# hku-mars/loam_livox

Hardware: NVIDIA H100
Metric: scans_per_sec (higher is better)
Workload: dtype f32 kNN / f64 solve

## Files before the change

include/loamlivox_b200.h:

```cpp
#ifndef LOAMLIVOX_B200_H
#define LOAMLIVOX_B200_H
#include <stddef.h>
#include <stdint.h>

#ifdef __cplusplus
extern "C" {
#endif

typedef struct { float x, y, z, intensity; } ll_point;
typedef struct { float x, y, z, _pad0, intensity, _pad1, _pad2, _pad3; } ll_pcl_xyzi;
enum { LL_FMT_XYZI16 = 0, LL_FMT_PCL32 = 1, LL_FMT_STRIDED = 2  };
enum { LL_HOST = 0, LL_DEVICE = 1 };

enum {
  LL_OK = 0,
  LL_ERR_INVALID = -1,
  LL_ERR_CUDA = -2,
  LL_ERR_CAPACITY = -3,
  LL_ERR_NO_BLOCKS = -4,
  LL_ERR_CAP_BINDS = -5
};

enum { LL_PT_NORMAL = 0, LL_PT_000 = 1, LL_PT_TOO_NEAR = 2, LL_PT_REFLECTIVITY_LOW = 4, LL_PT_REFLECTIVITY_HIGH = 8,
       LL_PT_CIRCLE_EDGE = 16, LL_PT_NAN = 32, LL_PT_SMALL_VIEW_ANGLE = 64 };
enum { LL_LABEL_INVALID = -1, LL_LABEL_UNLABELED = 0, LL_LABEL_CORNER = 1, LL_LABEL_SURFACE = 2, LL_LABEL_NEAR_NAN = 4,
       LL_LABEL_NEAR_ZERO = 8 };

typedef struct ll_ctx ll_ctx;
typedef struct ll_map ll_map;

typedef struct {
  float corner_curvature;
  float surface_curvature;
  float minimum_view_angle;
  float livox_min_dis;
  float livox_min_sigma;
  float max_fov_deg;
  float time_interval_pts;
  int   max_scan_points;
  int   max_features;
} ll_config;
void ll_config_default(ll_config* cfg);

int  ll_ctx_create(const ll_config* cfg, int device, ll_ctx** out);
void ll_ctx_destroy(ll_ctx* ctx);
int  ll_ctx_warmup(ll_ctx* ctx);
const char* ll_last_error(const ll_ctx* ctx);
void* ll_ctx_stream(ll_ctx* ctx);
int  ll_ctx_sync(ll_ctx* ctx);

int ll_extract(ll_ctx* ctx, const void* raw, size_t n, int fmt, int where, double stamp, int* n_scans);
int ll_extract_reset(ll_ctx* ctx);
int ll_piece_bounds(ll_ctx* ctx, int pieces, float* start, float* end);
int ll_get_features(ll_ctx* ctx, float minimum_blur, float maximum_blur, ll_point* corners, size_t* n_corners,
                    ll_point* surface, size_t* n_surface, ll_point* full, size_t* n_full);
int ll_extract_point_info(ll_ctx* ctx, int32_t* pt_type, int32_t* pt_label, float* curvature, float* view_angle,
                          float* depth_sq2, float* time_stamp, float* polar_dis_sq2, int32_t* polar_direction);
int ll_extract_split_idx(ll_ctx* ctx, int32_t* out, int cap, int* n_out);

int ll_voxel_downsample(ll_ctx* ctx, const void* in, size_t n, int fmt, int where, float leaf, ll_point* out, size_t* n_out);

int  ll_map_build(ll_ctx* ctx, const void* corner, size_t n_corner, const void* surf, size_t n_surf, int fmt, int where, ll_map** out);
int  ll_map_rebuild(ll_ctx* ctx, ll_map* map, const void* corner, size_t nc, const void* surf, size_t ns, int fmt, int where);
void ll_map_release(ll_map* map);
size_t ll_map_size(const ll_map* map, int which );
int  ll_map_build_sharded(ll_ctx* ctx, const void* corner, size_t n_corner, const void* surf, size_t n_surf, int fmt, int where,
                          int rank, int world, float cell_size, float halo_corner, float halo_surf, ll_map** out);
typedef struct { int rank, world; float cell_size, halo_corner, halo_surf; float origin[3]; int dims[3]; long long kept_corner, kept_surf, total_corner, total_surf; } ll_shard_info;
int  ll_map_shard_info(const ll_map* map, ll_shard_info* info, int* owner_out, size_t owner_cap);
int  ll_shard_plan(const int* cell_counts, const int dims[3], int world, int* owner_out);

int ll_knn(ll_ctx* ctx, const ll_map* map, int which, const ll_point* queries, size_t nq, int32_t* idx5, float* sqdist5);

typedef struct {
  int    if_motion_deblur;
  int    current_frame_index;
  int    mapping_init_accumulate_frames;
  int    icp_max_iterations;
  int    cere_max_iterations;
  int    cere_prerun_times;
  int    icp_plane, icp_line;
  int    maximum_allow_residual_block;
  int    rng_seed;
  double para_max_angular_rate;
  double para_max_speed;
  double max_final_cost;
  double minimum_pt_time_stamp, maximum_pt_time_stamp;
  double minimum_icp_R_diff, minimum_icp_T_diff;
  double inliner_dis, inlier_ratio;
  double maximum_dis_plane_for_match;
  double maximum_dis_line_for_match;
  double huber_a;
  double q_w_last[4], t_w_last[3];
  double q_w_curr[4], t_w_curr[3];
  double para_buffer_incremental[7];
} ll_reg_state;
void ll_reg_state_default(ll_reg_state* s);
void ll_reg_state_yaml(ll_reg_state* s, int realtime);
float ll_cap_uniform(int seed, int icp_iteration, int stream, int index);

typedef struct {
  int    status;
  int    registered;
  int    num_residual_blocks;
  int    icp_iterations, corner_used, surf_used;
  int    total_lm_iterations, total_evaluations;
  double q_w_curr[4], t_w_curr[3];
  double q_w_incre[4], t_w_incre[3];
  double inlier_threshold;
  double final_cost, initial_cost;
  double angular_diff, t_diff;
  float  gpu_ms_total, gpu_ms_knn;
  float  gpu_ms_knn_all, gpu_ms_solve_all, gpu_ms_select_all, gpu_ms_sort;
} ll_reg_result;

int ll_register(ll_ctx* ctx, const ll_map* map, const void* scan_corner, size_t n_corner, const void* scan_surf, size_t n_surf,
                int fmt, int where, const ll_reg_state* in, ll_reg_result* out);

int ll_build_blocks(ll_ctx* ctx, const ll_map* map, const void* scan_corner, size_t n_corner, const void* scan_surf, size_t n_surf,
                    int fmt, int where, const ll_reg_state* in, int32_t* type, double* a3, double* v3, int* corner_avail, int* surf_avail);
int ll_normal_equations(ll_ctx* ctx, const double x[7], double out28[28]);
int ll_solve(ll_ctx* ctx, int max_iterations, double x_io[7], double* initial_cost, double* final_cost, int* iterations);
int ll_inlier_select(ll_ctx* ctx, const double* l1, size_t n, double ratio, double* value, int* n_distinct);
int ll_set_blocks(ll_ctx* ctx, const ll_reg_state* in, size_t n, const int32_t* type, const ll_point* p, const float* a3, const double* v3);
int ll_solve_fused(ll_ctx* ctx, int prerun, int max_iterations, double x_io[7], double* threshold, int* n_distinct, int* n_kept, double* l1_out,
                   int iterations[2]);

typedef struct {
  float  line_res, plane_res;
  int    maximum_icp_iteration;
  int    maximum_residual_block;
  float  accepted_threshold;
  int    rng_seed;
  double t_init[3];
} ll_align_cfg;
void ll_align_cfg_default(ll_align_cfg* cfg);
int  ll_scene_align(ll_ctx* ctx, const void* source_line, size_t n_sl, const void* source_plane, size_t n_sp, const void* target_line, size_t n_tl,
                    const void* target_plane, size_t n_tp, int fmt, int where, const ll_align_cfg* cfg, ll_reg_result* out, int* scales_run);

int ll_transform(ll_ctx* ctx, const double q_wxyz[4], const double t[3], const void* in, size_t n, int fmt, int where, ll_point* out);

typedef struct {
  int   pieces;
  int   use_piece;
  float extractor_leaf_corner;
  float extractor_leaf_surf;
  float mapping_leaf_corner;
  float mapping_leaf_surf;
  int   whole_frame;
} ll_pipeline_cfg;
int ll_scan_to_pose(ll_ctx* ctx, const ll_map* map, const void* raw, size_t n, int fmt, int where, double stamp,
                    const ll_pipeline_cfg* pc, const ll_reg_state* in, ll_reg_result* out, int* n_corner_used, int* n_surf_used);

int ll_frame_to_pose(ll_ctx* ctx, const ll_map* map, int n_heads, const void* const* raws, const size_t* ns, int fmt, int where, const double* stamps,
                     const ll_pipeline_cfg* pc, const ll_reg_state* in, ll_reg_result* out, int* n_corner_used, int* n_surf_used);

typedef struct ll_cellmap ll_cellmap;
int  ll_cellmap_create(ll_ctx* ctx, float resolution, int revisit_threshold, int max_cells, ll_cellmap** out);
void ll_cellmap_release(ll_cellmap* map);
int  ll_cellmap_append(ll_ctx* ctx, ll_cellmap* map, const void* pts, size_t n, int fmt, int where);
int  ll_cellmap_assemble(ll_ctx* ctx, ll_cellmap* map, const double q_w_curr[4], const double t_w_curr[3], float search_range, float fov_deg, float leaf,
                         int down_sample_replace, ll_point* out_host, size_t cap, size_t* n_out, int* cells_in_fov, const ll_point** out_dev);
int  ll_cellmap_reserve(ll_ctx* ctx, ll_cellmap* map, size_t store_points, size_t scan_points);
int  ll_cellmap_stats(ll_ctx* ctx, ll_cellmap* map, int* cells, int* stored_points, int* frame_idx);

typedef struct {
  float line_resolution, plane_resolution;
  float cell_resolution;
  int   threshold_cell_revisit;
  float maximum_search_range_corner, maximum_search_range_surface, maximum_in_fov_angle;
  int   down_sample_replace;
  int   max_cells;
  int   matching_mode;
  int   maximum_history_size;
  int   reserve_map_points;
  int   reserve_store_points;
  ll_pipeline_cfg pipeline;
  ll_reg_state reg;
} ll_mapper_config;
typedef struct { int n_corner, n_surf, map_corner, map_surf, cells_in_fov_corner, cells_in_fov_surf, appended_corner, appended_surf;
                 float ms_front_end, ms_refresh, ms_register, ms_append;  } ll_mapper_stats;
typedef struct ll_mapper ll_mapper;
void ll_mapper_config_default(ll_mapper_config* cfg);
int  ll_mapper_create(ll_ctx* ctx, const ll_mapper_config* cfg, ll_mapper** out);
void ll_mapper_release(ll_mapper* mapper);
int  ll_mapper_process_scan(ll_mapper* mapper, const void* raw, size_t n, int fmt, int where, double stamp, ll_reg_result* out, ll_mapper_stats* stats);
int  ll_mapper_pose(const ll_mapper* mapper, double q_wxyz[4], double t[3], int* frame_index);

enum { LL_I_NONE = 0, LL_I_FLOAT32 = 7, LL_I_UINT8 = 2, LL_I_UINT16 = 4 };
typedef struct { int point_step, offset_x, offset_y, offset_z, offset_intensity, intensity_datatype; } ll_point_layout;
int  ll_set_point_layout(ll_ctx* ctx, const ll_point_layout* layout);
int  ll_features_to_pointcloud2(ll_ctx* ctx, int which, void* out_host, size_t cap_bytes, size_t* n_points);
int  ll_format_pose_log(const ll_reg_result* r, char* buf, size_t cap);

int  ll_state_snapshot_bytes(void);
int  ll_debug_solver_cycles(ll_ctx* ctx, long long out16[16]);

int ll_voxel_downsample_dev(ll_ctx* ctx, const ll_point* in_dev, size_t n, float leaf, ll_point* out_dev, size_t* n_out);
int ll_transform_dev(ll_ctx* ctx, const double q_wxyz[4], const double t[3], const ll_point* in_dev, size_t n, ll_point* out_dev);
int ll_last_features_dev(ll_ctx* ctx, const ll_point** corner_dev, size_t* n_corner, const ll_point** surf_dev, size_t* n_surf);

#define LL_IPC_HANDLE_BYTES 64
int ll_comm_local_handle(ll_ctx* ctx, unsigned char handle[LL_IPC_HANDLE_BYTES]);
int ll_comm_connect(ll_ctx* ctx, int rank, int world, const unsigned char* all_handles );

uint64_t ll_launch_count(const ll_ctx* ctx);

#ifdef __cplusplus
}
#endif
#endif
```

loam_livox_b200/capi.py:

```python
from __future__ import annotations

import ctypes as C
import os

import numpy as np

_HERE = os.path.dirname(os.path.abspath(__file__))
LIB_PATH = os.path.join(_HERE, "libloamlivox_b200.so")

LL_FMT_XYZI16, LL_FMT_PCL32, LL_FMT_STRIDED = 0, 1, 2
LL_I_NONE, LL_I_UINT8, LL_I_UINT16, LL_I_FLOAT32 = 0, 2, 4, 7
LL_HOST, LL_DEVICE = 0, 1
LL_OK, LL_ERR_INVALID, LL_ERR_CUDA, LL_ERR_CAPACITY, LL_ERR_NO_BLOCKS, LL_ERR_CAP_BINDS = 0, -1, -2, -3, -4, -5
LL_IPC_HANDLE_BYTES = 64

EXPORTS = [
    "ll_config_default", "ll_ctx_create", "ll_ctx_destroy", "ll_ctx_warmup", "ll_last_error", "ll_ctx_stream", "ll_ctx_sync", "ll_extract", "ll_extract_reset", "ll_piece_bounds",
    "ll_get_features", "ll_extract_point_info", "ll_extract_split_idx", "ll_voxel_downsample", "ll_map_build", "ll_map_release", "ll_map_size",
    "ll_map_build_sharded", "ll_knn", "ll_reg_state_default", "ll_register", "ll_build_blocks", "ll_normal_equations", "ll_solve", "ll_inlier_select", "ll_set_blocks", "ll_solve_fused", "ll_transform",
    "ll_scan_to_pose", "ll_comm_local_handle", "ll_comm_connect", "ll_launch_count", "ll_cellmap_create", "ll_cellmap_release", "ll_cellmap_append",
    "ll_cellmap_assemble", "ll_cellmap_reserve", "ll_cellmap_stats", "ll_voxel_downsample_dev", "ll_transform_dev", "ll_last_features_dev", "ll_mapper_config_default", "ll_mapper_create", "ll_mapper_release",
    "ll_mapper_process_scan", "ll_mapper_pose", "ll_map_rebuild", "ll_debug_solver_cycles", "ll_state_snapshot_bytes", "ll_set_point_layout", "ll_format_pose_log", "ll_reg_state_yaml", "ll_cap_uniform", "ll_map_shard_info", "ll_shard_plan", "ll_align_cfg_default", "ll_scene_align", "ll_frame_to_pose", "ll_features_to_pointcloud2",
]


class Config(C.Structure):
    _fields_ = [("corner_curvature", C.c_float), ("surface_curvature", C.c_float), ("minimum_view_angle", C.c_float), ("livox_min_dis", C.c_float),
                ("livox_min_sigma", C.c_float), ("max_fov_deg", C.c_float), ("time_interval_pts", C.c_float), ("max_scan_points", C.c_int), ("max_features", C.c_int)]


class RegState(C.Structure):
    _fields_ = [(n, C.c_int) for n in ("if_motion_deblur", "current_frame_index", "mapping_init_accumulate_frames", "icp_max_iterations", "cere_max_iterations",
                                       "cere_prerun_times", "icp_plane", "icp_line", "maximum_allow_residual_block", "rng_seed")] + \
               [(n, C.c_double) for n in ("para_max_angular_rate", "para_max_speed", "max_final_cost", "minimum_pt_time_stamp", "maximum_pt_time_stamp",
                                          "minimum_icp_R_diff", "minimum_icp_T_diff", "inliner_dis", "inlier_ratio", "maximum_dis_plane_for_match",
                                          "maximum_dis_line_for_match", "huber_a")] + \
               [("q_w_last", C.c_double * 4), ("t_w_last", C.c_double * 3), ("q_w_curr", C.c_double * 4), ("t_w_curr", C.c_double * 3),
                ("para_buffer_incremental", C.c_double * 7)]


class RegResult(C.Structure):
    _fields_ = [(n, C.c_int) for n in ("status", "registered", "num_residual_blocks", "icp_iterations", "corner_used", "surf_used", "total_lm_iterations",
                                       "total_evaluations")] + \
               [("q_w_curr", C.c_double * 4), ("t_w_curr", C.c_double * 3), ("q_w_incre", C.c_double * 4), ("t_w_incre", C.c_double * 3)] + \
               [(n, C.c_double) for n in ("inlier_threshold", "final_cost", "initial_cost", "angular_diff", "t_diff")] + \
               [("gpu_ms_total", C.c_float), ("gpu_ms_knn", C.c_float), ("gpu_ms_knn_all", C.c_float), ("gpu_ms_solve_all", C.c_float),
                ("gpu_ms_select_all", C.c_float), ("gpu_ms_sort", C.c_float)]


class PipelineCfg(C.Structure):
    _fields_ = [("pieces", C.c_int), ("use_piece", C.c_int), ("extractor_leaf_corner", C.c_float), ("extractor_leaf_surf", C.c_float),
                ("mapping_leaf_corner", C.c_float), ("mapping_leaf_surf", C.c_float), ("whole_frame", C.c_int)]


class PointLayout(C.Structure):
    _fields_ = [(n, C.c_int) for n in ("point_step", "offset_x", "offset_y", "offset_z", "offset_intensity", "intensity_datatype")]


class MapperConfig(C.Structure):
    _fields_ = [("line_resolution", C.c_float), ("plane_resolution", C.c_float), ("cell_resolution", C.c_float), ("threshold_cell_revisit", C.c_int),
                ("maximum_search_range_corner", C.c_float), ("maximum_search_range_surface", C.c_float), ("maximum_in_fov_angle", C.c_float),
                ("down_sample_replace", C.c_int), ("max_cells", C.c_int), ("matching_mode", C.c_int), ("maximum_history_size", C.c_int),
                ("reserve_map_points", C.c_int), ("reserve_store_points", C.c_int),
                ("pipeline", PipelineCfg), ("reg", RegState)]


class MapperStats(C.Structure):
    _fields_ = [(n, C.c_int) for n in ("n_corner", "n_surf", "map_corner", "map_surf", "cells_in_fov_corner", "cells_in_fov_surf", "appended_corner", "appended_surf")] + \
               [(n, C.c_float) for n in ("ms_front_end", "ms_refresh", "ms_register", "ms_append")]


class ShardInfo(C.Structure):
    _fields_ = [("rank", C.c_int), ("world", C.c_int), ("cell_size", C.c_float), ("halo_corner", C.c_float), ("halo_surf", C.c_float), ("origin", C.c_float * 3),
                ("dims", C.c_int * 3), ("kept_corner", C.c_longlong), ("kept_surf", C.c_longlong), ("total_corner", C.c_longlong), ("total_surf", C.c_longlong)]


class AlignCfg(C.Structure):
    _fields_ = [("line_res", C.c_float), ("plane_res", C.c_float), ("maximum_icp_iteration", C.c_int), ("maximum_residual_block", C.c_int),
                ("accepted_threshold", C.c_float), ("rng_seed", C.c_int), ("t_init", C.c_double * 3)]


class LoamLivoxError(RuntimeError):
    pass


_LIB = None


def lib():
    global _LIB
    if _LIB is not None:
        return _LIB
    if not os.path.exists(LIB_PATH):
        raise LoamLivoxError(f"{LIB_PATH} is missing: build it with `python -c 'import __graft_entry__ as g; g.build()'` (nvcc, sm_90a). "
                             "There is no CPU fallback.")
    L = C.CDLL(LIB_PATH)
    vp, sz, ci, cf, cd = C.c_void_p, C.c_size_t, C.c_int, C.c_float, C.c_double
    L.ll_config_default.argtypes = [C.POINTER(Config)]
    L.ll_ctx_create.argtypes = [C.POINTER(Config), ci, C.POINTER(vp)]
    L.ll_ctx_destroy.argtypes = [vp]
    L.ll_last_error.argtypes = [vp]
    L.ll_last_error.restype = C.c_char_p
    L.ll_ctx_stream.argtypes = [vp]
    L.ll_ctx_stream.restype = vp
    L.ll_ctx_sync.argtypes = [vp]
    L.ll_extract.argtypes = [vp, vp, sz, ci, ci, cd, C.POINTER(ci)]
    L.ll_extract_reset.argtypes = [vp]
    L.ll_piece_bounds.argtypes = [vp, ci, vp, vp]
    L.ll_get_features.argtypes = [vp, cf, cf, vp, C.POINTER(sz), vp, C.POINTER(sz), vp, C.POINTER(sz)]
    L.ll_extract_point_info.argtypes = [vp] + [vp] * 8
    L.ll_extract_split_idx.argtypes = [vp, vp, ci, C.POINTER(ci)]
    L.ll_voxel_downsample.argtypes = [vp, vp, sz, ci, ci, cf, vp, C.POINTER(sz)]
    L.ll_map_build.argtypes = [vp, vp, sz, vp, sz, ci, ci, C.POINTER(vp)]
    L.ll_map_build_sharded.argtypes = [vp, vp, sz, vp, sz, ci, ci, ci, ci, cf, cf, cf, C.POINTER(vp)]
    L.ll_map_shard_info.argtypes = [vp, C.POINTER(ShardInfo), vp, sz]
    L.ll_shard_plan.argtypes = [vp, vp, ci, vp]
    L.ll_align_cfg_default.argtypes = [C.POINTER(AlignCfg)]
    L.ll_scene_align.argtypes = [vp, vp, sz, vp, sz, vp, sz, vp, sz, ci, ci, C.POINTER(AlignCfg), C.POINTER(RegResult), C.POINTER(ci)]
    L.ll_map_release.argtypes = [vp]
    L.ll_map_size.argtypes = [vp, ci]
    L.ll_map_size.restype = sz
    L.ll_knn.argtypes = [vp, vp, ci, vp, sz, vp, vp]
    L.ll_reg_state_default.argtypes = [C.POINTER(RegState)]
    L.ll_reg_state_yaml.argtypes = [C.POINTER(RegState), ci]
    L.ll_cap_uniform.argtypes = [ci, ci, ci, ci]
    L.ll_cap_uniform.restype = cf
    L.ll_register.argtypes = [vp, vp, vp, sz, vp, sz, ci, ci, C.POINTER(RegState), C.POINTER(RegResult)]
    L.ll_build_blocks.argtypes = [vp, vp, vp, sz, vp, sz, ci, ci, C.POINTER(RegState), vp, vp, vp, C.POINTER(ci), C.POINTER(ci)]
    L.ll_normal_equations.argtypes = [vp, vp, vp]
    L.ll_solve.argtypes = [vp, ci, vp, C.POINTER(cd), C.POINTER(cd), C.POINTER(ci)]
    L.ll_inlier_select.argtypes = [vp, vp, sz, cd, C.POINTER(cd), C.POINTER(ci)]
    L.ll_set_blocks.argtypes = [vp, C.POINTER(RegState), sz, vp, vp, vp, vp]
    L.ll_solve_fused.argtypes = [vp, ci, ci, vp, C.POINTER(cd), C.POINTER(ci), C.POINTER(ci), vp, vp]
    L.ll_transform.argtypes = [vp, vp, vp, vp, sz, ci, ci, vp]
    L.ll_scan_to_pose.argtypes = [vp, vp, vp, sz, ci, ci, cd, C.POINTER(PipelineCfg), C.POINTER(RegState), C.POINTER(RegResult), C.POINTER(ci), C.POINTER(ci)]
    L.ll_frame_to_pose.argtypes = [vp, vp, ci, vp, vp, ci, ci, vp, C.POINTER(PipelineCfg), C.POINTER(RegState), C.POINTER(RegResult), C.POINTER(ci), C.POINTER(ci)]
    L.ll_features_to_pointcloud2.argtypes = [vp, ci, vp, sz, C.POINTER(sz)]
    L.ll_comm_local_handle.argtypes = [vp, vp]
    L.ll_comm_connect.argtypes = [vp, ci, ci, vp]
    L.ll_cellmap_create.argtypes = [vp, cf, ci, ci, C.POINTER(vp)]
    L.ll_cellmap_release.argtypes = [vp]
    L.ll_cellmap_append.argtypes = [vp, vp, vp, sz, ci, ci]
    L.ll_cellmap_assemble.argtypes = [vp, vp, vp, vp, cf, cf, cf, ci, vp, sz, C.POINTER(sz), C.POINTER(ci), C.POINTER(vp)]
    L.ll_ctx_warmup.argtypes = [vp]
    L.ll_cellmap_reserve.argtypes = [vp, vp, C.c_size_t, C.c_size_t]
    L.ll_cellmap_stats.argtypes = [vp, vp, C.POINTER(ci), C.POINTER(ci), C.POINTER(ci)]
    L.ll_voxel_downsample_dev.argtypes = [vp, vp, sz, cf, vp, C.POINTER(sz)]
    L.ll_transform_dev.argtypes = [vp, vp, vp, vp, sz, vp]
    L.ll_last_features_dev.argtypes = [vp, C.POINTER(vp), C.POINTER(sz), C.POINTER(vp), C.POINTER(sz)]
    L.ll_debug_solver_cycles.argtypes = [vp, vp]
    L.ll_state_snapshot_bytes.argtypes = []
    L.ll_set_point_layout.argtypes = [vp, C.POINTER(PointLayout)]
    L.ll_format_pose_log.argtypes = [C.POINTER(RegResult), C.c_char_p, sz]
    L.ll_map_rebuild.argtypes = [vp, vp, vp, sz, vp, sz, ci, ci]
    L.ll_mapper_config_default.argtypes = [C.POINTER(MapperConfig)]
    L.ll_mapper_create.argtypes = [vp, C.POINTER(MapperConfig), C.POINTER(vp)]
    L.ll_mapper_release.argtypes = [vp]
    L.ll_mapper_process_scan.argtypes = [vp, vp, sz, ci, ci, cd, C.POINTER(RegResult), C.POINTER(MapperStats)]
    L.ll_mapper_pose.argtypes = [vp, vp, vp, C.POINTER(ci)]
    L.ll_launch_count.argtypes = [vp]
    L.ll_launch_count.restype = C.c_uint64
    _LIB = L
    return L


def default_config(**kw) -> Config:
    c = Config()
    lib().ll_config_default(C.byref(c))
    for k, v in kw.items():
        setattr(c, k, v)
    return c


def default_reg_state(**kw) -> RegState:
    s = RegState()
    lib().ll_reg_state_default(C.byref(s))
    for k, v in kw.items():
        if isinstance(getattr(s, k), C.Array):
            getattr(s, k)[:] = list(v)
        else:
            setattr(s, k, v)
    return s


def yaml_reg_state(realtime: bool = False, **kw) -> RegState:
    s = RegState()
    lib().ll_reg_state_yaml(C.byref(s), int(bool(realtime)))
    for k, v in kw.items():
        if isinstance(getattr(s, k), C.Array):
            getattr(s, k)[:] = list(v)
        else:
            setattr(s, k, v)
    return s


def _ptr(a):
    if isinstance(a, (int, np.integer)):
        return C.c_void_p(int(a))
    return C.c_void_p(a.ctypes.data)


def _pts(a):
    a = np.ascontiguousarray(a, dtype=np.float32)
    assert a.ndim == 2 and a.shape[1] in (4, 8), "points must be [n,4] (XYZI16) or [n,8] (pcl::PointXYZI)"
    return a, (LL_FMT_XYZI16 if a.shape[1] == 4 else LL_FMT_PCL32)
```

loam_livox_b200/csrc/api.cu:

```cuda
#include <algorithm>
#include <cmath>
#include <cstring>
#include <cstdlib>
#include <cstdio>
#include "common.cuh"
#include "kernels.cuh"

static int ctx_alloc(ll_ctx* ctx) {
  const size_t cap = (size_t)ctx->cfg.max_features, scap = ctx->cfg.max_scan_points > ctx->cfg.max_features ? (size_t)ctx->cfg.max_scan_points : cap;
  RegArrays& A = ctx->A;
  LL_CUDA(ctx, ctx->reg_buf.carve([&](Carve& c) {
    A.feat = c.take<float4>(cap); A.blk_a = c.take<float4>(cap); A.blk_v = c.take<double>(cap * 3);
    A.l1 = c.take<double>(cap); A.k10_value = c.take<double>(1);
    A.k10_n_distinct = c.take<int>(1); A.counts = c.take<int>(16); A.bounds = c.take<float>(32);
    A.knn_idx = c.take<int>(cap * LL_KNN); A.knn_d = c.take<float>(cap * LL_KNN); A.perm = c.take<int>(cap);
    A.tmp_a = c.take<float4>(scap); A.tmp_b = c.take<float4>(scap); A.tmp_c = c.take<float4>(scap); A.tmp_d = c.take<float4>(scap);
  }));
  LL_TRY(extract_alloc(ctx));
  const int n = ctx->cfg.max_scan_points;
  const size_t vg = voxel_grid_bytes(n), pet = petals_bytes(n), gf = get_features_bytes(n);
  LL_CUDA(ctx, ctx->fe_main.reserve(std::max(vg, std::max(pet, gf))));
  LL_CUDA(ctx, ctx->fe_corner.reserve(vg));
  LL_CUDA(ctx, ctx->fe_petals.reserve(pet));
  return LL_OK;
}

extern "C" {

void ll_config_default(ll_config* c) {
  c->corner_curvature = 0.1f; c->surface_curvature = 0.005f; c->minimum_view_angle = 5.0f; c->livox_min_dis = 0.1f; c->livox_min_sigma = 7e-4f;
  c->max_fov_deg = 17.0f; c->time_interval_pts = 1.0e-5f; c->max_scan_points = 400000; c->max_features = 400000;
}
void ll_reg_state_default(ll_reg_state* s) {
  memset(s, 0, sizeof(*s));
  s->if_motion_deblur = 0; s->current_frame_index = 1000; s->mapping_init_accumulate_frames = 50; s->icp_max_iterations = 15; s->cere_max_iterations = 50; s->cere_prerun_times = 2;
  s->icp_plane = 1; s->icp_line = 1; s->maximum_allow_residual_block = 1000000;
  s->para_max_angular_rate = 20.0; s->para_max_speed = 0.3; s->max_final_cost = 1.0e9; s->minimum_pt_time_stamp = 0.0; s->maximum_pt_time_stamp = 0.1;
  s->minimum_icp_R_diff = 0.01; s->minimum_icp_T_diff = 0.01; s->inliner_dis = 0.02; s->inlier_ratio = 0.80; s->maximum_dis_plane_for_match = 50.0; s->maximum_dis_line_for_match = 2.0; s->huber_a = 0.1;
  s->q_w_last[0] = 1; s->q_w_curr[0] = 1; s->para_buffer_incremental[3] = 1;
}

void ll_reg_state_yaml(ll_reg_state* s, int realtime) {
  ll_reg_state_default(s);
  s->maximum_allow_residual_block = realtime ? 150 : 200;
  s->max_final_cost = 2.0;
}
float ll_cap_uniform(int seed, int icp_iteration, int stream, int index) { return ll_cap_uniform_f(seed, icp_iteration, stream, index); }

int ll_ctx_create(const ll_config* cfg, int device, ll_ctx** out) {
  if (!out) return LL_ERR_INVALID;
  *out = nullptr;
  int ndev = 0;
  if (cudaGetDeviceCount(&ndev) != cudaSuccess || ndev == 0) return LL_ERR_CUDA;
  if (device < 0 || device >= ndev) return LL_ERR_INVALID;
  if (cfg && (cfg->max_scan_points < 1 || cfg->max_scan_points >= (1 << 21) || cfg->max_features < 1)) return LL_ERR_INVALID;
  ll_ctx* ctx = new ll_ctx();
  ctx->device = device;
  if (cfg) ctx->cfg = *cfg; else ll_config_default(&ctx->cfg);
  cudaError_t e = cudaSetDevice(device);
  auto ok = [&](cudaError_t r) { if (e == cudaSuccess && r != cudaSuccess) e = r; };
  cudaDeviceProp prop; ok(cudaGetDeviceProperties(&prop, device)); ctx->num_sms = prop.multiProcessorCount;
  ok(cudaStreamCreateWithFlags(&ctx->stream, cudaStreamNonBlocking));
  ok(cudaStreamCreateWithFlags(&ctx->stream2, cudaStreamNonBlocking));
  ok(cudaStreamCreateWithFlags(&ctx->stream3, cudaStreamNonBlocking));
  ctx->sev.each([&](cudaEvent_t& ev) { ok(cudaEventCreateWithFlags(&ev, cudaEventDisableTiming)); });
  ctx->ev.each([&](cudaEvent_t& ev) { ok(cudaEventCreate(&ev)); });
  ok(cudaHostAlloc((void**)&ctx->pin, sizeof(PinnedStage), cudaHostAllocDefault));
  void* dreg = nullptr; ok(cudaMalloc(&dreg, sizeof(RegDevState))); if (dreg) ok(cudaMemset(dreg, 0, sizeof(RegDevState))); ctx->d_reg = (RegDevState*)dreg;
  if (e == cudaSuccess && solve_prepare(ctx) != LL_OK) e = cudaErrorUnknown;
  if (e == cudaSuccess && ctx_alloc(ctx) != LL_OK) e = cudaErrorMemoryAllocation;
  if (e != cudaSuccess) { cudaGetLastError(); ll_ctx_destroy(ctx); return LL_ERR_CUDA; }
  *out = ctx; return LL_OK;
}
void ll_ctx_destroy(ll_ctx* ctx) {
  if (!ctx) return;
  cudaSetDevice(ctx->device);
  for (cudaStream_t s : {ctx->stream, ctx->stream2, ctx->stream3}) if (s) cudaStreamSynchronize(s);
  if (ctx->fg.exec) cudaGraphExecDestroy(ctx->fg.exec);
  for (DevBuf* b : {&ctx->scratch, &ctx->scratch2, &ctx->fe_main, &ctx->fe_corner, &ctx->fe_petals, &ctx->stage_in, &ctx->extract_buf, &ctx->feat_buf, &ctx->reg_buf}) b->release();
  if (ctx->pin) cudaFreeHost(ctx->pin);
  if (ctx->d_reg) cudaFree(ctx->d_reg);
  if (ctx->d_sync) cudaFree(ctx->d_sync);
  if (ctx->comm_local) cudaFree(ctx->comm_local);
  for (int i = 0; i < 8; i++) if (ctx->comm_peers[i] && i != ctx->rank) cudaIpcCloseMemHandle(ctx->comm_peers[i]);
  ctx->sev.each([](cudaEvent_t& ev) { if (ev) cudaEventDestroy(ev); });
  ctx->ev.each([](cudaEvent_t& ev) { if (ev) cudaEventDestroy(ev); });
  for (cudaStream_t s : {ctx->stream3, ctx->stream2, ctx->stream}) if (s) cudaStreamDestroy(s);
  delete ctx;
}
const char* ll_last_error(const ll_ctx* ctx) { return ctx ? ctx->err.c_str() : "null context"; }
void* ll_ctx_stream(ll_ctx* ctx) { return (void*)ctx->stream; }
int ll_ctx_sync(ll_ctx* ctx) { cudaSetDevice(ctx->device); LL_CUDA(ctx, cudaStreamSynchronize(ctx->stream)); return LL_OK; }
uint64_t ll_launch_count(const ll_ctx* ctx) { return ctx->launches; }

static int extract_prepare(ll_ctx* ctx, const void* raw, size_t n, int fmt, int where, double stamp) {
  if ((int)n > ctx->cfg.max_scan_points) { ctx->set_error("scan larger than max_scan_points"); return LL_ERR_CAPACITY; }
  ExtractState& e = ctx->ex;
  if (stamp <= 0.0000001 || (stamp < e.last_maximum_time_stamp)) e.current_time = e.last_maximum_time_stamp; else e.current_time = stamp - e.first_receive_time;
  if (e.first_receive_time <= 0) e.first_receive_time = stamp;
  e.n = (int)n;
  if (n > 0) e.last_maximum_time_stamp = (double)(float)(e.current_time + (double)(((float)(n - 1)) * ctx->cfg.time_interval_pts));
  LL_TRY(upload_cloud(ctx, raw, n, fmt, where, e.raw));
  ctx->pin->extract_time = e.current_time;
  LL_CUDA(ctx, cudaMemcpyAsync(e.d_time, &ctx->pin->extract_time, sizeof(double), cudaMemcpyHostToDevice, ctx->stream));
  return LL_OK;
}
static int extract_enqueue(ll_ctx* ctx, DevBuf& scratch) {
  ExtractState& e = ctx->ex;
  if (e.n >= 5) { LL_TRY(launch_extract_points(ctx, e.n)); LL_TRY(launch_extract_petals(ctx, e.n, ctx->stream, scratch)); }
  else LL_CUDA(ctx, cudaMemsetAsync(e.d_meta, 0, 16, ctx->stream));
  return LL_OK;
}
int ll_extract(ll_ctx* ctx, const void* raw, size_t n, int fmt, int where, double stamp, int* n_scans) {
  if (!ctx || (!raw && n)) return LL_ERR_INVALID;
  cudaSetDevice(ctx->device);
  ExtractState& e = ctx->ex;
  LL_TRY(extract_prepare(ctx, raw, n, fmt, where, stamp));
  LL_TRY(extract_enqueue(ctx, ctx->scratch));
  if (n_scans) {
    int* h = ctx->pin->counts;
    LL_CUDA(ctx, cudaMemcpyAsync(h, e.d_meta, 3 * sizeof(int), cudaMemcpyDeviceToHost, ctx->stream));
    LL_CUDA(ctx, cudaStreamSynchronize(ctx->stream));
    *n_scans = h[1];
  }
  return LL_OK;
}
int ll_extract_reset(ll_ctx* ctx) {
  if (!ctx) return LL_ERR_INVALID;
  ctx->ex.first_receive_time = -1; ctx->ex.current_time = 0; ctx->ex.last_maximum_time_stamp = 0; ctx->ex.n = 0;
  return LL_OK;
}
int ll_piece_bounds(ll_ctx* ctx, int pieces, float* start, float* end) {
  if (!ctx || pieces < 1 || pieces > 16) return LL_ERR_INVALID;
  cudaSetDevice(ctx->device);
  const RegArrays& A = ctx->A;
  LL_TRY(launch_piece_bounds(ctx, pieces, A.bounds));
  float* h = ctx->pin->bounds;
  LL_CUDA(ctx, cudaMemcpyAsync(h, A.bounds, 2 * pieces * sizeof(float), cudaMemcpyDeviceToHost, ctx->stream));
  LL_CUDA(ctx, cudaStreamSynchronize(ctx->stream));
  for (int i = 0; i < pieces; i++) { start[i] = h[2 * i]; end[i] = h[2 * i + 1]; }
  return LL_OK;
}
int ll_get_features(ll_ctx* ctx, float minimum_blur, float maximum_blur, ll_point* corners, size_t* n_corners, ll_point* surface, size_t* n_surface, ll_point* full, size_t* n_full) {
  if (!ctx) return LL_ERR_INVALID;
  cudaSetDevice(ctx->device);
  const RegArrays& A = ctx->A;
  LL_TRY(launch_get_features(ctx, ctx->stream, ctx->scratch, nullptr, minimum_blur, maximum_blur, A.tmp_a, A.tmp_b, A.tmp_c, A.counts));
  int* h = ctx->pin->counts;
  LL_CUDA(ctx, cudaMemcpyAsync(h, A.counts, 3 * sizeof(int), cudaMemcpyDeviceToHost, ctx->stream));
  LL_CUDA(ctx, cudaStreamSynchronize(ctx->stream));
  int nc = ctx->ex.n ? h[0] : 0, ns = ctx->ex.n ? h[1] : 0, nf = ctx->ex.n ? h[2] : 0;
  if (corners && nc) LL_CUDA(ctx, cudaMemcpyAsync(corners, A.tmp_a, (size_t)nc * 16, cudaMemcpyDeviceToHost, ctx->stream));
  if (surface && ns) LL_CUDA(ctx, cudaMemcpyAsync(surface, A.tmp_b, (size_t)ns * 16, cudaMemcpyDeviceToHost, ctx->stream));
  if (full && nf) LL_CUDA(ctx, cudaMemcpyAsync(full, A.tmp_c, (size_t)nf * 16, cudaMemcpyDeviceToHost, ctx->stream));
  LL_CUDA(ctx, cudaStreamSynchronize(ctx->stream));
  if (n_corners) *n_corners = nc; if (n_surface) *n_surface = ns; if (n_full) *n_full = nf;
  return LL_OK;
}
int ll_extract_point_info(ll_ctx* ctx, int32_t* pt_type, int32_t* pt_label, float* curvature, float* view_angle, float* depth_sq2, float* time_stamp, float* polar_dis_sq2, int32_t* polar_direction) {
  if (!ctx) return LL_ERR_INVALID;
  cudaSetDevice(ctx->device);
  ExtractState& e = ctx->ex; size_t n = e.n; cudaStream_t s = ctx->stream;
  if (pt_type) LL_CUDA(ctx, cudaMemcpyAsync(pt_type, e.pt_type, n * 4, cudaMemcpyDeviceToHost, s));
  if (pt_label) LL_CUDA(ctx, cudaMemcpyAsync(pt_label, e.pt_label, n * 4, cudaMemcpyDeviceToHost, s));
  if (curvature) LL_CUDA(ctx, cudaMemcpyAsync(curvature, e.curvature, n * 4, cudaMemcpyDeviceToHost, s));
  if (view_angle) LL_CUDA(ctx, cudaMemcpyAsync(view_angle, e.view_angle, n * 4, cudaMemcpyDeviceToHost, s));
  if (depth_sq2) LL_CUDA(ctx, cudaMemcpyAsync(depth_sq2, e.depth_sq2, n * 4, cudaMemcpyDeviceToHost, s));
  if (time_stamp) LL_CUDA(ctx, cudaMemcpyAsync(time_stamp, e.time_stamp, n * 4, cudaMemcpyDeviceToHost, s));
  if (polar_dis_sq2) LL_CUDA(ctx, cudaMemcpyAsync(polar_dis_sq2, e.polar_dis_sq2, n * 4, cudaMemcpyDeviceToHost, s));
  LL_CUDA(ctx, cudaStreamSynchronize(s));
  if (polar_direction) {
    std::vector<int8_t> tmp(n);
    LL_CUDA(ctx, cudaMemcpy(tmp.data(), e.polar_dir, n, cudaMemcpyDeviceToHost));
    for (size_t i = 0; i < n; i++) polar_direction[i] = tmp[i];
  }
  return LL_OK;
}
int ll_extract_split_idx(ll_ctx* ctx, int32_t* out, int cap, int* n_out) {
  if (!ctx) return LL_ERR_INVALID;
  cudaSetDevice(ctx->device);
  int meta[3] = {0, 0, 0};
  LL_CUDA(ctx, cudaStreamSynchronize(ctx->stream));
  LL_CUDA(ctx, cudaMemcpy(meta, ctx->ex.d_meta, sizeof(meta), cudaMemcpyDeviceToHost));
  int m = meta[0] < cap ? meta[0] : cap;
  if (m > 0) LL_CUDA(ctx, cudaMemcpy(out, ctx->ex.split_idx, (size_t)m * 4, cudaMemcpyDeviceToHost));
  if (n_out) *n_out = meta[0];
  return LL_OK;
}

int ll_voxel_downsample(ll_ctx* ctx, const void* in, size_t n, int fmt, int where, float leaf, ll_point* out, size_t* n_out) {
  if (!ctx || !n_out || !(leaf > 0.f)) return LL_ERR_INVALID;
  cudaSetDevice(ctx->device);
  *n_out = 0; if (n == 0) return LL_OK;
  float4* d_in; float4* d_out; int* d_n;
  LL_CUDA(ctx, ctx->feat_buf.carve([&](Carve& c) { d_in = c.take<float4>(n); d_out = c.take<float4>(n); d_n = c.take<int>(1); }));
  LL_TRY(upload_cloud(ctx, in, n, fmt, where, d_in));
  LL_TRY(launch_voxel_grid(ctx, ctx->stream, ctx->scratch, d_in, (int)n, nullptr, leaf, d_out, d_n));
  int* h = ctx->pin->counts;
  LL_CUDA(ctx, cudaMemcpyAsync(h, d_n, sizeof(int), cudaMemcpyDeviceToHost, ctx->stream));
  LL_CUDA(ctx, cudaStreamSynchronize(ctx->stream));
  *n_out = (size_t)h[0];
  if (out && h[0] > 0) { LL_CUDA(ctx, cudaMemcpyAsync(out, d_out, (size_t)h[0] * 16, cudaMemcpyDeviceToHost, ctx->stream)); LL_CUDA(ctx, cudaStreamSynchronize(ctx->stream)); }
  return LL_OK;
}
int ll_transform(ll_ctx* ctx, const double q[4], const double t[3], const void* in, size_t n, int fmt, int where, ll_point* out) {
  if (!ctx || !q || !t) return LL_ERR_INVALID;
  cudaSetDevice(ctx->device);
  if (n == 0) return LL_OK;
  float4* d_in; float4* d_out; double* d_pose;
  LL_CUDA(ctx, ctx->feat_buf.carve([&](Carve& c) { d_in = c.take<float4>(n); d_out = c.take<float4>(n); d_pose = c.take<double>(7); }));
  double* h = ctx->pin->pose; for (int k = 0; k < 4; k++) h[k] = q[k]; for (int k = 0; k < 3; k++) h[4 + k] = t[k];
  LL_CUDA(ctx, cudaMemcpyAsync(d_pose, h, 7 * sizeof(double), cudaMemcpyHostToDevice, ctx->stream));
  LL_TRY(upload_cloud(ctx, in, n, fmt, where, d_in));
  LL_TRY(launch_transform(ctx, ctx->stream, d_pose, d_in, (int)n, d_out));
  LL_CUDA(ctx, cudaMemcpyAsync(out, d_out, n * 16, cudaMemcpyDeviceToHost, ctx->stream));
  LL_CUDA(ctx, cudaStreamSynchronize(ctx->stream));
  return LL_OK;
}

int ll_voxel_downsample_dev(ll_ctx* ctx, const ll_point* in_dev, size_t n, float leaf, ll_point* out_dev, size_t* n_out) {
  if (!ctx || !n_out || !(leaf > 0.f)) return LL_ERR_INVALID;
  cudaSetDevice(ctx->device);
  *n_out = 0; if (n == 0) return LL_OK;
  int* d_n;
  LL_CUDA(ctx, ctx->feat_buf.carve([&](Carve& c) { d_n = c.take<int>(1); }));
  LL_TRY(launch_voxel_grid(ctx, ctx->stream, ctx->scratch, (const float4*)in_dev, (int)n, nullptr, leaf, (float4*)out_dev, d_n));
  int* h = ctx->pin->counts;
  LL_CUDA(ctx, cudaMemcpyAsync(h, d_n, sizeof(int), cudaMemcpyDeviceToHost, ctx->stream));
  LL_CUDA(ctx, cudaStreamSynchronize(ctx->stream));
  *n_out = (size_t)h[0];
  return LL_OK;
}
int ll_transform_dev(ll_ctx* ctx, const double q[4], const double t[3], const ll_point* in_dev, size_t n, ll_point* out_dev) {
  if (!ctx || !q || !t) return LL_ERR_INVALID;
  cudaSetDevice(ctx->device);
  if (n == 0) return LL_OK;
  double* d_pose;
  LL_CUDA(ctx, ctx->feat_buf.carve([&](Carve& c) { d_pose = c.take<double>(7); }));
  double* h = ctx->pin->pose; for (int k = 0; k < 4; k++) h[k] = q[k]; for (int k = 0; k < 3; k++) h[4 + k] = t[k];
  LL_CUDA(ctx, cudaMemcpyAsync(d_pose, h, 7 * sizeof(double), cudaMemcpyHostToDevice, ctx->stream));
  LL_TRY(launch_transform(ctx, ctx->stream, d_pose, (const float4*)in_dev, (int)n, (float4*)out_dev));
  LL_CUDA(ctx, cudaStreamSynchronize(ctx->stream));
  return LL_OK;
}
int ll_last_features_dev(ll_ctx* ctx, const ll_point** corner_dev, size_t* n_corner, const ll_point** surf_dev, size_t* n_surf) {
  if (!ctx) return LL_ERR_INVALID;
  const RegArrays& A = ctx->A;
  if (corner_dev) *corner_dev = (const ll_point*)A.feat; if (n_corner) *n_corner = (size_t)ctx->last_nc;
  if (surf_dev) *surf_dev = (const ll_point*)(A.feat + ctx->last_nc); if (n_surf) *n_surf = (size_t)ctx->last_ns;
  return LL_OK;
}

static int map_index(ll_ctx* ctx, ll_map* m, const void* corner, size_t nc, const void* surf, size_t ns, int fmt, int where) {
  const bool in_place = where == LL_DEVICE && fmt == LL_FMT_XYZI16;
  const float4* d_c = (const float4*)corner; const float4* d_s = (const float4*)surf;
  int st = LL_OK;
  if (!in_place) {
    float4* b_c; float4* b_s;
    LL_CUDA(ctx, ctx->feat_buf.carve([&](Carve& c) { b_c = c.take<float4>(nc); b_s = c.take<float4>(ns); }));
    d_c = b_c; d_s = b_s;
    st = upload_cloud(ctx, corner, nc, fmt, where, b_c);
    if (st == LL_OK) st = upload_cloud(ctx, surf, ns, fmt, where, b_s);
    if (st != LL_OK) return st;
  }
  cudaStream_t s = ctx->stream;
  LL_CUDA(ctx, cudaEventRecord(ctx->sev.fork, s));
  LL_CUDA(ctx, cudaStreamWaitEvent(ctx->stream2, ctx->sev.fork, 0));
  st = build_bucket_tree(ctx, ctx->stream2, ctx->scratch2, d_c, (int)nc, &m->corner);
  const int st2 = build_bucket_tree(ctx, s, ctx->scratch, d_s, (int)ns, &m->surf);
  LL_CUDA(ctx, cudaEventRecord(ctx->sev.join, ctx->stream2));
  LL_CUDA(ctx, cudaStreamWaitEvent(s, ctx->sev.join, 0));
  if (st == LL_OK) st = st2;
  if (st == LL_OK && where == LL_HOST && cudaStreamSynchronize(s) != cudaSuccess) st = LL_ERR_CUDA;
  return st;
}
static int map_build_common(ll_ctx* ctx, const void* corner, size_t nc, const void* surf, size_t ns, int fmt, int where, ll_map** out) {
  if (!ctx || !out) return LL_ERR_INVALID;
  cudaSetDevice(ctx->device);
  ll_map* m = new ll_map(); m->device = ctx->device;
  int st = map_index(ctx, m, corner, nc, surf, ns, fmt, where);
  if (st != LL_OK) { m->corner.storage.release(); m->surf.storage.release(); delete m; return st; }
  *out = m; return LL_OK;
}
int ll_map_rebuild(ll_ctx* ctx, ll_map* map, const void* corner, size_t nc, const void* surf, size_t ns, int fmt, int where) {
  if (!ctx || !map) return LL_ERR_INVALID;
  cudaSetDevice(ctx->device);
  return map_index(ctx, map, corner, nc, surf, ns, fmt, where);
}
int ll_map_build(ll_ctx* ctx, const void* corner, size_t nc, const void* surf, size_t ns, int fmt, int where, ll_map** out) {
  return map_build_common(ctx, corner, nc, surf, ns, fmt, where, out);
}
void ll_map_release(ll_map* map) {
  if (!map) return;
  cudaSetDevice(map->device);
  map->corner.storage.release(); map->surf.storage.release(); map->shard_owner.release(); delete map;
}
size_t ll_map_size(const ll_map* map, int which) { return map ? (size_t)(which == 0 ? map->corner.n : map->surf.n) : 0; }

int ll_knn(ll_ctx* ctx, const ll_map* map, int which, const ll_point* queries, size_t nq, int32_t* idx5, float* sqdist5) {
  if (!ctx || !map) return LL_ERR_INVALID;
  cudaSetDevice(ctx->device);
  if (nq == 0) return LL_OK;
  float4* d_q; int* d_idx; float* d_d;
  LL_CUDA(ctx, ctx->feat_buf.carve([&](Carve& c) { d_q = c.take<float4>(nq); d_idx = c.take<int>(nq * LL_KNN); d_d = c.take<float>(nq * LL_KNN); }));
  LL_CUDA(ctx, cudaMemcpyAsync(d_q, queries, nq * 16, cudaMemcpyHostToDevice, ctx->stream));
  LL_TRY(launch_knn_query(ctx, which == 0 ? map->corner : map->surf, d_q, (int)nq, d_idx, d_d));
  LL_CUDA(ctx, cudaMemcpyAsync(idx5, d_idx, nq * 20, cudaMemcpyDeviceToHost, ctx->stream));
  LL_CUDA(ctx, cudaMemcpyAsync(sqdist5, d_d, nq * 20, cudaMemcpyDeviceToHost, ctx->stream));
  LL_CUDA(ctx, cudaStreamSynchronize(ctx->stream));
  return LL_OK;
}

static void fill_state(RegDevState* h, const ll_reg_state* in) {
  memset(h, 0, sizeof(RegDevState));
  for (int k = 0; k < 4; k++) { h->pose_curr[k] = in->q_w_curr[k]; h->pose_last[k] = in->q_w_last[k]; }
  for (int k = 0; k < 3; k++) { h->pose_curr[4 + k] = in->t_w_curr[k]; h->pose_last[4 + k] = in->t_w_last[k]; }
  for (int k = 0; k < 7; k++) h->x[k] = in->para_buffer_incremental[k];
  h->q_last_opt[0] = 1.0;
  h->bound = (double)(float)in->para_max_speed; h->huber_a = in->huber_a; h->inliner_dis = in->inliner_dis; h->inlier_ratio = in->inlier_ratio;
  h->min_icp_R = in->minimum_icp_R_diff; h->min_icp_T = in->minimum_icp_T_diff;
  h->cap = in->maximum_allow_residual_block; h->rng_seed = in->rng_seed;
  h->if_motion_deblur = in->if_motion_deblur ? 1 : 0; h->min_ts = in->minimum_pt_time_stamp; h->max_ts = in->maximum_pt_time_stamp;
}
static KnnBlocksArgs knn_args(ll_ctx* ctx, const ll_map* map, int nc, int ns, const ll_reg_state* in, bool debug) {
  const RegArrays& A = ctx->A;
  KnnBlocksArgs a; a.corner = make_view(map->corner); a.surf = make_view(map->surf); a.feat = A.feat; a.n_corner = nc; a.n_surf = ns;
  a.pose = ctx->d_reg->pose_curr; a.max_dis_line = in->maximum_dis_line_for_match; a.max_dis_plane = in->maximum_dis_plane_for_match;
  a.icp_line = in->icp_line; a.icp_plane = in->icp_plane; a.blk_a = A.blk_a; a.blk_v = A.blk_v;
  a.corner_avail = &ctx->d_reg->corner_avail; a.surf_avail = &ctx->d_reg->surf_avail; a.n_blocks = &ctx->d_reg->n_blocks;
  a.cap = in->maximum_allow_residual_block; a.rng_seed = in->rng_seed;
  a.seed_ids = A.knn_idx; a.knn_d = debug ? A.knn_d : nullptr; a.perm = A.perm;
  ctx->solve_world = (map->world > 1 && ctx->world > 1) ? ctx->world : 1;
  a.st = ctx->d_reg; a.deblur = in->if_motion_deblur ? 1 : 0; ctx->reg_deblur = a.deblur;
  a.rank = map->rank; a.world = map->world; a.grid = map->grid; a.shard_owner = (const int*)map->shard_owner.p;
  return a;
}
static SolveArgs solve_args(ll_ctx* ctx, int M, SolveMode mode, int max_iter) {
  const RegArrays& A = ctx->A;
  SolveArgs s; s.st = ctx->d_reg; s.sync = ctx->d_sync; s.feat = A.feat; s.blk_a = A.blk_a; s.blk_v = A.blk_v; s.l1 = A.l1; s.k10_value = A.k10_value; s.k10_n_distinct = A.k10_n_distinct;
  s.M = M; s.max_iterations = max_iter; s.mode = mode; s.rank = ctx->rank; s.world = ctx->solve_world; s.comm_local = (double*)ctx->comm_local;
  for (int i = 0; i < 8; i++) s.comm_peer[i] = (double*)ctx->comm_peers[i];
  s.cap_check = 0; s.deblur = ctx->reg_deblur; s.prerun_iterations = 0; s.table = nullptr; s.table_mask = 0;
  return s;
}

}

int register_device(ll_ctx* ctx, const ll_map* map, int nc, int ns, const ll_reg_state* in, ll_reg_result* out) {
  cudaStream_t s = ctx->stream;
  const RegArrays& A = ctx->A;
  RegEvents& ev = ctx->ev;
  memset(out, 0, sizeof(*out));
  out->status = 1;
  for (int k = 0; k < 4; k++) { out->q_w_curr[k] = in->q_w_curr[k]; out->q_w_incre[k] = k == 0 ? in->para_buffer_incremental[3] : in->para_buffer_incremental[k - 1]; }
  for (int k = 0; k < 3; k++) { out->t_w_curr[k] = in->t_w_curr[k]; out->t_w_incre[k] = in->para_buffer_incremental[4 + k]; }
  if (!(map->corner.n_src > 0 && map->surf.n_src > 50 && in->current_frame_index > in->mapping_init_accumulate_frames)) return LL_OK;
  const int M = nc + ns;
  ctx->last_nc = nc; ctx->last_ns = ns;
  const int cap_check = M > in->maximum_allow_residual_block ? 1 : 0;
  if (M == 0) { ctx->set_error("no features"); return LL_ERR_NO_BLOCKS; }
  LL_TRY(solve_capacity(ctx, M, in->if_motion_deblur ? 1 : 0));
  RegDevState* h = &ctx->pin->state_in;
  fill_state(h, in);
  LL_CUDA(ctx, cudaMemcpyAsync(ctx->d_reg, h, sizeof(RegDevState), cudaMemcpyHostToDevice, s));
  LL_CUDA(ctx, cudaEventRecord(ev.total[0], s));
  out->registered = 1;
  KnnBlocksArgs ka = knn_args(ctx, map, nc, ns, in, false);
  LL_CUDA(ctx, cudaMemsetAsync(A.knn_idx, 0xff, (size_t)M * LL_KNN * 4, s));
  LL_CUDA(ctx, cudaEventRecord(ev.sort[0], s));
  LL_TRY(launch_query_sort(ctx, s, ctx->scratch, ka, A.perm));
  LL_CUDA(ctx, cudaEventRecord(ev.sort[1], s));
  int iter = 0; RegDevState* hs = &ctx->pin->snap[0];
  const bool sharded = ctx->world > 1 && map->world > 1;
  if (sharded && (map->world != ctx->world || map->rank != ctx->rank)) { ctx->set_error("map shard and context disagree on rank/world"); return LL_ERR_INVALID; }
  if (map->world > 1 && (std::sqrt(in->maximum_dis_line_for_match) > (double)map->halo[0] * 1.0001 + 1e-3 || std::sqrt(in->maximum_dis_plane_for_match) > (double)map->halo[1] * 1.0001 + 1e-3)) {
    ctx->set_error("match gates wider than the halo this shard was built with: owner + halo search would no longer be exact"); return LL_ERR_INVALID;
  }
  if (map->world > 1 && ctx->world != map->world) { ctx->set_error("a sharded map needs a context connected to the same number of ranks (ll_comm_connect)"); return LL_ERR_INVALID; }
  if (sharded && M > ctx->cfg.max_features) { ctx->set_error("more features than max_features (exchange buffer)"); return LL_ERR_CAPACITY; }
  double* x_l1 = sharded ? (double*)((char*)ctx->comm_local + LL_COMM_X_OFF) : nullptr;
  unsigned long long* set_table = nullptr;
  LL_CUDA(ctx, ctx->scratch.carve([&](Carve& c) { set_table = l1_set_layout(c, M); }));
  RegDevState* slots = ctx->pin->snap;
  auto enqueue_iteration = [&](int it) -> int {
    cudaEvent_t* e = it < LL_TIMED_ITERS ? ev.phase[it] : nullptr;
    LL_CUDA(ctx, cudaMemsetAsync(&ctx->d_reg->corner_avail, 0, 3 * sizeof(int), s));
    if (sharded) LL_CUDA(ctx, cudaMemsetAsync(x_l1, 0xff, (size_t)M * sizeof(double), s));
    if (it == 0) LL_CUDA(ctx, cudaEventRecord(ev.knn_first[0], s));
    if (e) LL_CUDA(ctx, cudaEventRecord(e[0], s));
    LL_TRY(launch_knn_blocks(ctx, ka));
    if (e) LL_CUDA(ctx, cudaEventRecord(e[1], s));
    if (it == 0) LL_CUDA(ctx, cudaEventRecord(ev.knn_first[1], s));
    if (!sharded) {
      SolveArgs sa = solve_args(ctx, M, SOLVE_FUSED, in->cere_max_iterations);
      sa.prerun_iterations = in->cere_prerun_times; sa.table = set_table; sa.table_mask = l1_set_capacity(M) - 1;
      sa.cap_check = cap_check;
      if (e) { LL_CUDA(ctx, cudaEventRecord(e[2], s)); LL_CUDA(ctx, cudaEventRecord(e[3], s)); }
      LL_TRY(launch_solve(ctx, sa));
    } else {
      if (cap_check) LL_TRY(launch_count_exchange(ctx));
      { SolveArgs sa = solve_args(ctx, M, SOLVE_FIRST, in->cere_prerun_times); sa.cap_check = cap_check; LL_TRY(launch_solve(ctx, sa)); }
      if (e) LL_CUDA(ctx, cudaEventRecord(e[2], s));
      LL_TRY(launch_l1_exchange(ctx, A.l1, M));
      LL_TRY(launch_k10_select(ctx, x_l1, M, &ctx->d_reg->inlier_ratio, set_table, l1_set_capacity(M) - 1, A.k10_value, A.k10_n_distinct));
      if (e) LL_CUDA(ctx, cudaEventRecord(e[3], s));
      { SolveArgs sa = solve_args(ctx, M, SOLVE_SECOND, in->cere_max_iterations); sa.cap_check = cap_check; LL_TRY(launch_solve(ctx, sa)); }
    }
    if (e) LL_CUDA(ctx, cudaEventRecord(e[4], s));
    LL_CUDA(ctx, cudaMemcpyAsync(&slots[it & 1], ctx->d_reg, sizeof(RegDevState), cudaMemcpyDeviceToHost, s));
    LL_CUDA(ctx, cudaEventRecord(ctx->sev.it[it & 1], s));
    return LL_OK;
  };
  const bool speculate = !sharded;
  LL_TRY(enqueue_iteration(0));
  for (iter = 0; iter < in->icp_max_iterations; iter++) {
    if (speculate && iter + 1 < in->icp_max_iterations) LL_TRY(enqueue_iteration(iter + 1));
    LL_CUDA(ctx, cudaEventSynchronize(ctx->sev.it[iter & 1]));
    hs = &slots[iter & 1];
    if (hs->lm.termination == -1) {
      cudaStreamSynchronize(s); ctx->set_error("no residual block survived the gates / cap / inlier selection"); return LL_ERR_NO_BLOCKS;
    }
    if (hs->icp_done) break;
    if (!speculate && iter + 1 < in->icp_max_iterations) LL_TRY(enqueue_iteration(iter + 1));
  }
  LL_CUDA(ctx, cudaEventRecord(ev.total[1], s));
  LL_CUDA(ctx, cudaEventSynchronize(ev.total[1]));
  cudaEventElapsedTime(&out->gpu_ms_total, ev.total[0], ev.total[1]); cudaEventElapsedTime(&out->gpu_ms_knn, ev.knn_first[0], ev.knn_first[1]);
  cudaEventElapsedTime(&out->gpu_ms_sort, ev.sort[0], ev.sort[1]);
  { const int done_iters = (iter < in->icp_max_iterations ? iter + 1 : in->icp_max_iterations);
    for (int i = 0; i < done_iters && i < LL_TIMED_ITERS; i++) { float a = 0, b = 0, c = 0, d = 0; cudaEvent_t* e = ev.phase[i];
      cudaEventElapsedTime(&a, e[0], e[1]); cudaEventElapsedTime(&b, e[1], e[2]); cudaEventElapsedTime(&c, e[2], e[3]); cudaEventElapsedTime(&d, e[3], e[4]);
      out->gpu_ms_knn_all += a; out->gpu_ms_solve_all += b + d; out->gpu_ms_select_all += c; } }
  out->icp_iterations = (iter + 1 < in->icp_max_iterations) ? iter + 1 : in->icp_max_iterations;
  out->corner_used = hs->corner_avail; out->surf_used = hs->surf_avail; out->num_residual_blocks = hs->num_residual_blocks;
  out->total_lm_iterations = hs->total_lm_iterations; out->total_evaluations = hs->total_evaluations;
  for (int k = 0; k < 4; k++) out->q_w_curr[k] = hs->pose_curr[k];
  for (int k = 0; k < 3; k++) out->t_w_curr[k] = hs->pose_curr[4 + k];
  out->q_w_incre[0] = hs->x[3]; out->q_w_incre[1] = hs->x[0]; out->q_w_incre[2] = hs->x[1]; out->q_w_incre[3] = hs->x[2];
  for (int k = 0; k < 3; k++) out->t_w_incre[k] = hs->x[4 + k];
  out->final_cost = hs->final_cost; out->initial_cost = hs->initial_cost; out->angular_diff = hs->angular_diff; out->t_diff = hs->t_diff;
  out->inlier_threshold = hs->inlier_threshold * hs->final_cost / hs->initial_cost;
  const float minimize_cost = (float)hs->final_cost;
  if (hs->angular_diff > (double)(float)in->para_max_angular_rate || minimize_cost > (float)in->max_final_cost) {
    out->status = 0;
    for (int k = 0; k < 4; k++) out->q_w_curr[k] = in->q_w_last[k];
    for (int k = 0; k < 3; k++) out->t_w_curr[k] = in->t_w_last[k];
  }
  return LL_OK;
}

extern "C" {

int ll_register(ll_ctx* ctx, const ll_map* map, const void* scan_corner, size_t nc, const void* scan_surf, size_t ns, int fmt, int where, const ll_reg_state* in, ll_reg_result* out) {
  if (!ctx || !map || !in || !out) return LL_ERR_INVALID;
  cudaSetDevice(ctx->device);
  if ((int)(nc + ns) > ctx->cfg.max_features) { ctx->set_error("more features than max_features"); return LL_ERR_CAPACITY; }
  LL_TRY(upload_cloud(ctx, scan_corner, nc, fmt, where, ctx->A.feat));
  LL_TRY(upload_cloud(ctx, scan_surf, ns, fmt, where, ctx->A.feat + nc));
  return register_device(ctx, map, (int)nc, (int)ns, in, out);
}

int ll_ctx_warmup(ll_ctx* ctx) {
  if (!ctx) return LL_ERR_INVALID;
  cudaSetDevice(ctx->device);
  std::vector<ll_point> surf, corner, fs, fc;
  auto add = [](std::vector<ll_point>& v, float x, float y, float z) { ll_point p; p.x = x; p.y = y; p.z = z; p.intensity = 0.f; v.push_back(p); };
  for (int i = 0; i < 20; i++) for (int j = 0; j < 20; j++) {
    const float u = 0.1f * i + 0.013f * (j % 3), v = 0.1f * j + 0.007f * (i % 5);
    add(surf, 1.f + u, -1.f + v, 0.f); add(surf, 1.f + u, 1.2f, 0.05f + v); add(surf, 3.2f, -1.f + u, 0.05f + v);
    if ((i * 20 + j) % 4 == 0) { add(fs, 1.f + u + 0.004f, -1.f + v - 0.003f, 0.006f); add(fs, 1.f + u, 1.195f, 0.05f + v); add(fs, 3.194f, -1.f + u, 0.05f + v); }
  }
  for (int k = 0; k < 20; k++) { add(corner, 3.2f, 1.2f, 0.1f * k); add(corner, 1.f + 0.1f * k, 1.2f, 0.f); if (k % 4 == 0) { add(fc, 3.195f, 1.197f, 0.1f * k + 0.02f); add(fc, 1.02f + 0.1f * k, 1.196f, 0.004f); } }
  if ((int)(fc.size() + fs.size()) > ctx->cfg.max_features) return LL_OK;
  ll_map* m = nullptr;
  int st = ll_map_build(ctx, corner.data(), corner.size(), surf.data(), surf.size(), LL_FMT_XYZI16, LL_HOST, &m);
  if (st == LL_OK) {
    ll_reg_state rs; ll_reg_state_default(&rs); rs.current_frame_index = rs.mapping_init_accumulate_frames + 1;
    ll_reg_result r;
    st = ll_register(ctx, m, fc.data(), fc.size(), fs.data(), fs.size(), LL_FMT_XYZI16, LL_HOST, &rs, &r);
    if (st == LL_ERR_NO_BLOCKS) st = LL_OK;
  }
  if (m) ll_map_release(m);
  if (cudaStreamSynchronize(ctx->stream) != cudaSuccess) return LL_ERR_CUDA;
  return st;
}

int ll_build_blocks(ll_ctx* ctx, const ll_map* map, const void* scan_corner, size_t nc, const void* scan_surf, size_t ns, int fmt, int where, const ll_reg_state* in,
                    int32_t* type, double* a3, double* v3, int* corner_avail, int* surf_avail) {
  if (!ctx || !map || !in) return LL_ERR_INVALID;
  cudaSetDevice(ctx->device);
  const int M = (int)(nc + ns);
  if (M > ctx->cfg.max_features) return LL_ERR_CAPACITY;
  const RegArrays& A = ctx->A;
  cudaStream_t s = ctx->stream;
  LL_TRY(upload_cloud(ctx, scan_corner, nc, fmt, where, A.feat));
  LL_TRY(upload_cloud(ctx, scan_surf, ns, fmt, where, A.feat + nc));
  RegDevState* h = &ctx->pin->state_in; fill_state(h, in);
  LL_CUDA(ctx, cudaMemcpyAsync(ctx->d_reg, h, sizeof(RegDevState), cudaMemcpyHostToDevice, s));
  { KnnBlocksArgs ka = knn_args(ctx, map, (int)nc, (int)ns, in, true); LL_CUDA(ctx, cudaMemsetAsync(A.knn_idx, 0xff, (size_t)M * LL_KNN * 4, s)); LL_TRY(launch_query_sort(ctx, s, ctx->scratch, ka, A.perm)); LL_TRY(launch_knn_blocks(ctx, ka)); }
  std::vector<float4> ba(M); std::vector<double> bv((size_t)M * 3);
  int cnt[2];
  LL_CUDA(ctx, cudaMemcpyAsync(ba.data(), A.blk_a, (size_t)M * 16, cudaMemcpyDeviceToHost, s));
  LL_CUDA(ctx, cudaMemcpyAsync(bv.data(), A.blk_v, (size_t)M * 24, cudaMemcpyDeviceToHost, s));
  LL_CUDA(ctx, cudaMemcpyAsync(cnt, &ctx->d_reg->corner_avail, 8, cudaMemcpyDeviceToHost, s));
  LL_CUDA(ctx, cudaStreamSynchronize(s));
  for (int i = 0; i < M; i++) {
    int t; memcpy(&t, &ba[i].w, 4);
    if (type) type[i] = t;
    if (a3) { a3[3 * i] = ba[i].x; a3[3 * i + 1] = ba[i].y; a3[3 * i + 2] = ba[i].z; }
    if (v3) { v3[3 * i] = bv[3 * i]; v3[3 * i + 1] = bv[3 * i + 1]; v3[3 * i + 2] = bv[3 * i + 2]; }
  }
  if (corner_avail) *corner_avail = cnt[0]; if (surf_avail) *surf_avail = cnt[1];
  ctx->hook_slots = M;
  return LL_OK;
}
}

static int hook_solve(ll_ctx* ctx, const double x[7], const SolveArgs& sa, double* l1_out = nullptr) {
  cudaStream_t s = ctx->stream;
  PinnedStage* pin = ctx->pin;
  for (int k = 0; k < 7; k++) pin->x[k] = x[k];
  LL_CUDA(ctx, cudaMemcpyAsync(ctx->d_reg->x, pin->x, 7 * sizeof(double), cudaMemcpyHostToDevice, s));
  LL_TRY(launch_solve(ctx, sa));
  LL_CUDA(ctx, cudaMemcpyAsync(&pin->snap[0], ctx->d_reg, sizeof(RegDevState), cudaMemcpyDeviceToHost, s));
  if (l1_out && sa.M > 0) LL_CUDA(ctx, cudaMemcpyAsync(l1_out, ctx->A.l1, (size_t)sa.M * sizeof(double), cudaMemcpyDeviceToHost, s));
  LL_CUDA(ctx, cudaStreamSynchronize(s));
  return LL_OK;
}

extern "C" {

int ll_normal_equations(ll_ctx* ctx, const double x[7], double out28[28]) {
  if (!ctx || !x || !out28) return LL_ERR_INVALID;
  cudaSetDevice(ctx->device);
  LL_TRY(hook_solve(ctx, x, solve_args(ctx, ctx->hook_slots, SOLVE_EVALUATE, 0)));
  const RegDevState* hs = &ctx->pin->snap[0];
  for (int i = 0; i < 21; i++) out28[i] = hs->lm.H[i];
  for (int i = 0; i < 6; i++) out28[21 + i] = hs->lm.g[i];
  out28[27] = hs->lm.x_cost;
  return LL_OK;
}
int ll_solve(ll_ctx* ctx, int max_iterations, double x_io[7], double* initial_cost, double* final_cost, int* iterations) {
  if (!ctx || !x_io) return LL_ERR_INVALID;
  cudaSetDevice(ctx->device);
  LL_TRY(hook_solve(ctx, x_io, solve_args(ctx, ctx->hook_slots, SOLVE_PLAIN, max_iterations)));
  const RegDevState* hs = &ctx->pin->snap[0];
  for (int k = 0; k < 7; k++) x_io[k] = hs->x[k];
  if (initial_cost) *initial_cost = hs->lm.initial_cost; if (final_cost) *final_cost = hs->lm.final_cost; if (iterations) *iterations = hs->lm.iteration;
  return LL_OK;
}
int ll_set_blocks(ll_ctx* ctx, const ll_reg_state* in, size_t n, const int32_t* type, const ll_point* p, const float* a3, const double* v3) {
  if (!ctx || !in || (n > 0 && (!type || !p || !a3 || !v3))) return LL_ERR_INVALID;
  if (n > (size_t)ctx->cfg.max_features) { ctx->set_error("more blocks than max_features"); return LL_ERR_CAPACITY; }
  const int M = (int)n;
  LL_TRY(solve_capacity(ctx, M, in->if_motion_deblur ? 1 : 0));
  for (int i = 0; i < M; i++) if (type[i] < 0 || type[i] > 2) { ctx->set_error("block type must be 0, 1 (line) or 2 (plane)"); return LL_ERR_INVALID; }
  cudaSetDevice(ctx->device);
  const RegArrays& A = ctx->A;
  cudaStream_t s = ctx->stream;
  std::vector<float4> ba(M);
  for (int i = 0; i < M; i++) { ba[i].x = a3[3 * i]; ba[i].y = a3[3 * i + 1]; ba[i].z = a3[3 * i + 2]; memcpy(&ba[i].w, &type[i], 4); }
  if (M > 0) {
    LL_CUDA(ctx, cudaMemcpyAsync(A.feat, p, (size_t)M * 16, cudaMemcpyHostToDevice, s));
    LL_CUDA(ctx, cudaMemcpyAsync(A.blk_a, ba.data(), (size_t)M * 16, cudaMemcpyHostToDevice, s));
    LL_CUDA(ctx, cudaMemcpyAsync(A.blk_v, v3, (size_t)M * 24, cudaMemcpyHostToDevice, s));
  }
  RegDevState* h = &ctx->pin->state_in; fill_state(h, in);
  for (int i = 0; i < M; i++) h->n_blocks += type[i] != 0 ? 1 : 0;
  LL_CUDA(ctx, cudaMemcpyAsync(ctx->d_reg, h, sizeof(RegDevState), cudaMemcpyHostToDevice, s));
  LL_CUDA(ctx, cudaStreamSynchronize(s));
  ctx->hook_slots = M; ctx->hook_cap_check = M > in->maximum_allow_residual_block ? 1 : 0;
  ctx->reg_deblur = in->if_motion_deblur ? 1 : 0; ctx->solve_world = 1;
  return LL_OK;
}
int ll_solve_fused(ll_ctx* ctx, int prerun, int max_iterations, double x_io[7], double* threshold, int* n_distinct, int* n_kept, double* l1_out, int iterations[2]) {
  if (!ctx || !x_io) return LL_ERR_INVALID;
  cudaSetDevice(ctx->device);
  const int M = ctx->hook_slots;
  cudaStream_t s = ctx->stream;
  SolveArgs sa = solve_args(ctx, M, SOLVE_FUSED, max_iterations);
  LL_CUDA(ctx, ctx->scratch.carve([&](Carve& c) { sa.table = l1_set_layout(c, M); }));
  sa.prerun_iterations = prerun; sa.table_mask = l1_set_capacity(M) - 1;
  sa.cap_check = ctx->hook_cap_check;
  LL_CUDA(ctx, cudaMemsetAsync(&ctx->d_reg->icp_done, 0, sizeof(int), s));
  LL_CUDA(ctx, cudaMemsetAsync(&ctx->d_reg->total_lm_iterations, 0, 2 * sizeof(int), s));
  LL_TRY(hook_solve(ctx, x_io, sa, l1_out));
  const RegDevState* hs = &ctx->pin->snap[0];
  for (int k = 0; k < 7; k++) x_io[k] = hs->x[k];
  if (threshold) *threshold = hs->inlier_threshold; if (n_distinct) *n_distinct = hs->n_unique; if (n_kept) *n_kept = hs->num_residual_blocks;
  if (iterations) { iterations[1] = hs->lm.iteration; iterations[0] = hs->total_lm_iterations - hs->lm.iteration; }
  return LL_OK;
}
int ll_inlier_select(ll_ctx* ctx, const double* l1, size_t n, double ratio, double* value, int* n_distinct) {
  if (!ctx || (n > 0 && !l1) || !value || !n_distinct || !(ratio >= 0.0)) return LL_ERR_INVALID;
  for (size_t i = 0; i < n; i++) if (l1[i] < 0.0) { ctx->set_error("L1 norms are never negative"); return LL_ERR_INVALID; }
  if (n > (size_t)ctx->cfg.max_features) { ctx->set_error("more values than max_features"); return LL_ERR_CAPACITY; }
  cudaSetDevice(ctx->device);
  const int M = (int)n;
  const RegArrays& A = ctx->A;
  cudaStream_t s = ctx->stream;
  if (M > 0) LL_CUDA(ctx, cudaMemcpyAsync(A.l1, l1, n * sizeof(double), cudaMemcpyHostToDevice, s));
  double* d_ratio = &ctx->d_reg->inlier_ratio;
  LL_CUDA(ctx, cudaMemcpyAsync(d_ratio, &ratio, sizeof(double), cudaMemcpyHostToDevice, s));
  unsigned long long* table = nullptr;
  LL_CUDA(ctx, ctx->scratch.carve([&](Carve& c) { table = l1_set_layout(c, M); }));
  LL_TRY(launch_k10_select(ctx, A.l1, M, d_ratio, table, l1_set_capacity(M) - 1, A.k10_value, A.k10_n_distinct));
  LL_CUDA(ctx, cudaMemcpyAsync(value, A.k10_value, sizeof(double), cudaMemcpyDeviceToHost, s));
  LL_CUDA(ctx, cudaMemcpyAsync(n_distinct, A.k10_n_distinct, sizeof(int), cudaMemcpyDeviceToHost, s));
  LL_CUDA(ctx, cudaStreamSynchronize(s));
  return LL_OK;
}

int ll_set_point_layout(ll_ctx* ctx, const ll_point_layout* L) {
  if (!ctx || !L) return LL_ERR_INVALID;
  const int isz = L->intensity_datatype == LL_I_FLOAT32 ? 4 : L->intensity_datatype == LL_I_UINT16 ? 2 : L->intensity_datatype == LL_I_UINT8 ? 1 : 0;
  if (L->intensity_datatype != LL_I_NONE && isz == 0) { ctx->set_error("unsupported intensity datatype"); return LL_ERR_INVALID; }
  const int offs[3] = {L->offset_x, L->offset_y, L->offset_z};
  for (int k = 0; k < 3; k++) if (offs[k] < 0 || offs[k] + 4 > L->point_step) { ctx->set_error("field outside the point record"); return LL_ERR_INVALID; }
  if (isz && (L->offset_intensity < 0 || L->offset_intensity + isz > L->point_step)) { ctx->set_error("intensity outside the point record"); return LL_ERR_INVALID; }
  ctx->layout = *L;
  return LL_OK;
}
int ll_features_to_pointcloud2(ll_ctx* ctx, int which, void* out_host, size_t cap_bytes, size_t* n_points) {
  if (!ctx || !n_points || (which != 0 && which != 1)) return LL_ERR_INVALID;
  cudaSetDevice(ctx->device);
  const RegArrays& A = ctx->A;
  const int n = which == 0 ? ctx->last_nc : ctx->last_ns;
  const float4* src = which == 0 ? A.feat : A.feat + ctx->last_nc;
  *n_points = (size_t)n;
  const size_t bytes = (size_t)n * (size_t)ctx->layout.point_step;
  if (!out_host || n == 0) return LL_OK;
  if (cap_bytes < bytes) { ctx->set_error("output buffer smaller than n * point_step"); return LL_ERR_CAPACITY; }
  LL_CUDA(ctx, ctx->stage_in.reserve(bytes));
  LL_TRY(launch_pack_strided(ctx, src, n, ctx->stage_in.as<unsigned char>()));
  LL_CUDA(ctx, cudaMemcpyAsync(out_host, ctx->stage_in.p, bytes, cudaMemcpyDeviceToHost, ctx->stream));
  LL_CUDA(ctx, cudaStreamSynchronize(ctx->stream));
  return LL_OK;
}
int ll_format_pose_log(const ll_reg_result* r, char* buf, size_t cap) {
  if (!r || !buf) return -1;
  const int n = snprintf(buf, cap, "--------------------\nCurr_Q = %f,%f,%f,%f\r\nCurr_T = %f,%f,%f\r\nIncre_Q = %f,%f,%f,%f\r\nIncre_T = %f,%f,%f\r\nCost=%f,blk_size = %d \r\n",
                         r->q_w_curr[0], r->q_w_curr[1], r->q_w_curr[2], r->q_w_curr[3], r->t_w_curr[0], r->t_w_curr[1], r->t_w_curr[2],
                         r->q_w_incre[0], r->q_w_incre[1], r->q_w_incre[2], r->q_w_incre[3], r->t_w_incre[0], r->t_w_incre[1], r->t_w_incre[2],
                         r->final_cost, r->num_residual_blocks);
  return (n < 0 || (size_t)n >= cap) ? -1 : n;
}
int ll_state_snapshot_bytes(void) { return (int)sizeof(RegDevState); }
int ll_debug_solver_cycles(ll_ctx* ctx, long long out8[16]) {
  if (!ctx || !out8) return LL_ERR_INVALID;
  cudaSetDevice(ctx->device);
  LL_CUDA(ctx, cudaMemcpyAsync(out8, ctx->d_reg->prof, 16 * sizeof(long long), cudaMemcpyDeviceToHost, ctx->stream));
  LL_CUDA(ctx, cudaStreamSynchronize(ctx->stream));
  return LL_OK;
}

}

static int voxel_chains(ll_ctx* ctx, const ll_pipeline_cfg* pc, int nc_cap, const int* d_nc, int ns_cap, const int* d_ns) {
  cudaStream_t s = ctx->stream, s2 = ctx->stream2;
  const RegArrays& A = ctx->A; int* cnt = A.counts;
  LL_CUDA(ctx, cudaEventRecord(ctx->sev.fork, s));
  LL_CUDA(ctx, cudaStreamWaitEvent(s2, ctx->sev.fork, 0));
  LL_TRY(launch_voxel_grid(ctx, s2, ctx->fe_corner, A.tmp_a, nc_cap, d_nc, pc->extractor_leaf_corner, A.tmp_d, cnt + 4));
  LL_TRY(launch_voxel_grid(ctx, s2, ctx->fe_corner, A.tmp_d, nc_cap, cnt + 4, pc->mapping_leaf_corner, A.tmp_a, cnt + 5));
  LL_CUDA(ctx, cudaEventRecord(ctx->sev.join, s2));
  LL_TRY(launch_voxel_grid(ctx, s, ctx->fe_main, A.tmp_b, ns_cap, d_ns, pc->extractor_leaf_surf, A.tmp_c, cnt + 6));
  LL_TRY(launch_voxel_grid(ctx, s, ctx->fe_main, A.tmp_c, ns_cap, cnt + 6, pc->mapping_leaf_surf, A.tmp_b, cnt + 7));
  LL_CUDA(ctx, cudaStreamWaitEvent(s, ctx->sev.join, 0));
  return LL_OK;
}

static int front_end_enqueue(ll_ctx* ctx, const ll_pipeline_cfg* pc, int ncap) {
  cudaStream_t s = ctx->stream;
  const RegArrays& A = ctx->A;
  const bool petals_aside = pc->whole_frame && ctx->ex.n >= 5;
  if (petals_aside) {
    LL_TRY(launch_extract_points(ctx, ctx->ex.n));
    LL_CUDA(ctx, cudaEventRecord(ctx->sev.fork3, s));
    LL_CUDA(ctx, cudaStreamWaitEvent(ctx->stream3, ctx->sev.fork3, 0));
    LL_TRY(launch_extract_petals(ctx, ctx->ex.n, ctx->stream3, ctx->fe_petals));
    LL_CUDA(ctx, cudaEventRecord(ctx->sev.join3, ctx->stream3));
  } else LL_TRY(extract_enqueue(ctx, ctx->fe_main));
  const float* d_bounds = nullptr;
  if (!pc->whole_frame) { LL_TRY(launch_piece_bounds(ctx, pc->pieces, A.bounds)); d_bounds = A.bounds + 2 * pc->use_piece; }
  LL_TRY(launch_get_features(ctx, s, ctx->fe_main, d_bounds, 0.f, 1.f, A.tmp_a, A.tmp_b, nullptr, A.counts));
  LL_TRY(voxel_chains(ctx, pc, ncap, A.counts + 0, ncap, A.counts + 1));
  if (petals_aside) LL_CUDA(ctx, cudaStreamWaitEvent(s, ctx->sev.join3, 0));
  LL_CUDA(ctx, cudaMemcpyAsync(ctx->pin->fe_counts, A.counts, sizeof(ctx->pin->fe_counts), cudaMemcpyDeviceToHost, s));
  LL_CUDA(ctx, cudaMemcpyAsync(ctx->pin->fe_meta, ctx->ex.d_meta, sizeof(ctx->pin->fe_meta), cudaMemcpyDeviceToHost, s));
  return LL_OK;
}

int scan_front_end(ll_ctx* ctx, const void* raw, size_t n, int fmt, int where, double stamp, const ll_pipeline_cfg* pc, int* nc_out, int* ns_out, int* dropped) {
  cudaStream_t s = ctx->stream;
  const RegArrays& A = ctx->A;
  LL_TRY(extract_prepare(ctx, raw, n, fmt, where, stamp));
  const int ncap = (int)n;
  ll_ctx::FrontGraph& g = ctx->fg;
  const bool same = g.n == n && memcmp(&g.pc, pc, sizeof(*pc)) == 0;
  if (same && g.exec) {
    LL_CUDA(ctx, cudaGraphLaunch(g.exec, s));
    ctx->launches += g.launches;
  } else if (same && g.warm && n >= 5) {
    if (g.exec) { cudaGraphExecDestroy(g.exec); g.exec = nullptr; }
    const uint64_t l0 = ctx->launches;
    cudaGraph_t graph = nullptr;
    LL_CUDA(ctx, cudaStreamBeginCapture(s, cudaStreamCaptureModeRelaxed));
    const int st = front_end_enqueue(ctx, pc, ncap);
    const cudaError_t ce = cudaStreamEndCapture(s, &graph);
    if (st != LL_OK || ce != cudaSuccess) {
      if (graph) cudaGraphDestroy(graph);
      cudaGetLastError(); g.warm = false; g.n = 0;
      LL_TRY(front_end_enqueue(ctx, pc, ncap));
    } else {
      g.launches = ctx->launches - l0;
      LL_CUDA(ctx, cudaGraphInstantiate(&g.exec, graph, 0));
      cudaGraphDestroy(graph);
      LL_CUDA(ctx, cudaGraphLaunch(g.exec, s));
    }
  } else {
    if (g.exec) { cudaGraphExecDestroy(g.exec); g.exec = nullptr; }
    LL_TRY(front_end_enqueue(ctx, pc, ncap));
    g.n = n; g.pc = *pc; g.warm = true;
  }
  LL_CUDA(ctx, cudaStreamSynchronize(s));
  const int* h = ctx->pin->fe_counts;
  const int nc = h[5], ns = h[7], meta_scans = ctx->pin->fe_meta[1];
  ctx->last_full_min_t = ll_ord2f(h[10]); ctx->last_full_max_t = ll_ord2f(h[11]);
  *nc_out = nc; *ns_out = ns;
  *dropped = (meta_scans <= 5 && !pc->whole_frame) ? 1 : 0;
  if (*dropped) return LL_OK;
  if (nc + ns > ctx->cfg.max_features) { ctx->set_error("more features than max_features"); return LL_ERR_CAPACITY; }
  LL_CUDA(ctx, cudaMemcpyAsync(A.feat, A.tmp_a, (size_t)nc * 16, cudaMemcpyDeviceToDevice, s));
  LL_CUDA(ctx, cudaMemcpyAsync(A.feat + nc, A.tmp_b, (size_t)ns * 16, cudaMemcpyDeviceToDevice, s));
  return LL_OK;
}

extern "C" int ll_scan_to_pose(ll_ctx* ctx, const ll_map* map, const void* raw, size_t n, int fmt, int where, double stamp, const ll_pipeline_cfg* pc, const ll_reg_state* in,
                    ll_reg_result* out, int* n_corner_used, int* n_surf_used) {
  if (!ctx || !map || !pc || !in || !out) return LL_ERR_INVALID;
  cudaSetDevice(ctx->device);
  int nc = 0, ns = 0, dropped = 0;
  LL_TRY(scan_front_end(ctx, raw, n, fmt, where, stamp, pc, &nc, &ns, &dropped));
  if (n_corner_used) *n_corner_used = nc; if (n_surf_used) *n_surf_used = ns;
  if (dropped) { memset(out, 0, sizeof(*out)); out->status = 1; ctx->set_error("frame dropped: <= 5 petals"); return LL_OK; }
  return register_device(ctx, map, nc, ns, in, out);
}

extern "C" int ll_frame_to_pose(ll_ctx* ctx, const ll_map* map, int n_heads, const void* const* raws, const size_t* ns, int fmt, int where, const double* stamps,
                     const ll_pipeline_cfg* pc, const ll_reg_state* in, ll_reg_result* out, int* n_corner_used, int* n_surf_used) {
  if (!ctx || !map || !pc || !in || !out || !raws || !ns || !stamps || n_heads < 1 || n_heads > 8) return LL_ERR_INVALID;
  cudaSetDevice(ctx->device);
  cudaStream_t s = ctx->stream;
  size_t total = 0; for (int h = 0; h < n_heads; h++) total += ns[h];
  if ((int)total > ctx->cfg.max_scan_points) { ctx->set_error("frame (all heads) larger than max_scan_points"); return LL_ERR_CAPACITY; }
  const RegArrays& A = ctx->A;
  int acc_c = 0, acc_s = 0;
  int* hc = ctx->pin->fe_counts; const int* hm = ctx->pin->fe_meta;
  for (int h = 0; h < n_heads; h++) {
    LL_TRY(extract_prepare(ctx, raws[h], ns[h], fmt, where, stamps[h]));
    LL_TRY(extract_enqueue(ctx, ctx->fe_main));
    const float* d_bounds = nullptr;
    if (!pc->whole_frame) { LL_TRY(launch_piece_bounds(ctx, pc->pieces, A.bounds)); d_bounds = A.bounds + 2 * pc->use_piece; }
    LL_TRY(launch_get_features(ctx, s, ctx->fe_main, d_bounds, 0.f, 1.f, A.tmp_a + acc_c, A.tmp_b + acc_s, nullptr, A.counts));
    LL_CUDA(ctx, cudaMemcpyAsync(hc, A.counts, 3 * sizeof(int), cudaMemcpyDeviceToHost, s));
    LL_CUDA(ctx, cudaMemcpyAsync(ctx->pin->fe_meta, ctx->ex.d_meta, sizeof(ctx->pin->fe_meta), cudaMemcpyDeviceToHost, s));
    LL_CUDA(ctx, cudaStreamSynchronize(s));
    if (ns[h] >= 5 && (hm[1] > 5 || pc->whole_frame)) { acc_c += hc[0]; acc_s += hc[1]; }
  }
  LL_TRY(voxel_chains(ctx, pc, acc_c, nullptr, acc_s, nullptr));
  LL_CUDA(ctx, cudaMemcpyAsync(hc, A.counts, 8 * sizeof(int), cudaMemcpyDeviceToHost, s));
  LL_CUDA(ctx, cudaStreamSynchronize(s));
  const int nc = hc[5], nsf = hc[7];
  if (n_corner_used) *n_corner_used = nc; if (n_surf_used) *n_surf_used = nsf;
  if (nc + nsf > ctx->cfg.max_features) { ctx->set_error("more features than max_features"); return LL_ERR_CAPACITY; }
  LL_CUDA(ctx, cudaMemcpyAsync(A.feat, A.tmp_a, (size_t)nc * 16, cudaMemcpyDeviceToDevice, s));
  LL_CUDA(ctx, cudaMemcpyAsync(A.feat + nc, A.tmp_b, (size_t)nsf * 16, cudaMemcpyDeviceToDevice, s));
  return register_device(ctx, map, nc, nsf, in, out);
}

extern "C" {

int ll_comm_local_handle(ll_ctx* ctx, unsigned char handle[LL_IPC_HANDLE_BYTES]) {
  if (!ctx) return LL_ERR_INVALID;
  cudaSetDevice(ctx->device);
  const size_t comm_bytes = LL_COMM_X_OFF + (size_t)ctx->cfg.max_features * sizeof(double);
  if (!ctx->comm_local) { LL_CUDA(ctx, cudaMalloc(&ctx->comm_local, comm_bytes)); LL_CUDA(ctx, cudaMemset(ctx->comm_local, 0, comm_bytes)); }
  cudaIpcMemHandle_t h; LL_CUDA(ctx, cudaIpcGetMemHandle(&h, ctx->comm_local));
  static_assert(sizeof(cudaIpcMemHandle_t) <= LL_IPC_HANDLE_BYTES, "ipc handle size");
  memset(handle, 0, LL_IPC_HANDLE_BYTES); memcpy(handle, &h, sizeof(h));
  return LL_OK;
}
int ll_comm_connect(ll_ctx* ctx, int rank, int world, const unsigned char* all) {
  if (!ctx || world < 1 || world > 8 || rank < 0 || rank >= world) return LL_ERR_INVALID;
  cudaSetDevice(ctx->device);
  if (!ctx->comm_local) { ctx->set_error("call ll_comm_local_handle first"); return LL_ERR_INVALID; }
  ctx->rank = rank; ctx->world = world;
  for (int p = 0; p < world; p++) {
    if (p == rank) { ctx->comm_peers[p] = ctx->comm_local; continue; }
    cudaIpcMemHandle_t h; memcpy(&h, all + (size_t)p * LL_IPC_HANDLE_BYTES, sizeof(h));
    LL_CUDA(ctx, cudaIpcOpenMemHandle(&ctx->comm_peers[p], h, cudaIpcMemLazyEnablePeerAccess));
  }
  return LL_OK;
}
}
```

loam_livox_b200/csrc/kernels.cuh:

```cuda
#pragma once
#include "common.cuh"

struct TreeView {
  const float4* pts;
  const float4* src;
  const float4* nodes[LL_MAX_LEVELS];
  int n, n_levels;
  const float* bbox;
};
TreeView make_view(const BucketTree& t);
int build_bucket_tree(ll_ctx* ctx, cudaStream_t s, DevBuf& scratch, const float4* d_src, int n_src, BucketTree* t);
size_t tree_scratch_bytes(int n_src);
size_t tree_storage_bytes(int n_src);
__global__ void bbox_init_kernel(int* bbox);
__global__ void bbox_kernel(const float4* __restrict__ src, int n, int* __restrict__ bbox);

struct RegDevState;
struct KnnBlocksArgs {
  TreeView corner, surf;
  const float4* feat;
  int n_corner, n_surf;
  const double* pose;
  double max_dis_line, max_dis_plane;
  int icp_line, icp_plane;
  float4* blk_a; double* blk_v;
  int* corner_avail; int* surf_avail; int* n_blocks;
  int cap, rng_seed;
  int* seed_ids;
  float* knn_d;
  const int* perm;
  int rank, world; ShardGrid grid; const int* shard_owner;
  const RegDevState* st;
  int deblur;
};
int launch_knn_query(ll_ctx* ctx, const BucketTree& t, const float4* d_q, int nq, int* d_idx, float* d_d);
int launch_knn_blocks(ll_ctx* ctx, const KnnBlocksArgs& a);
int launch_query_sort(ll_ctx* ctx, cudaStream_t s, DevBuf& scratch, const KnnBlocksArgs& a, int* d_perm);
size_t query_sort_bytes(int M);

#include "lm_state.h"

struct RegDevState {
  double pose_curr[7];
  double pose_last[7];
  double x[7];
  double q_last_opt[4], t_last_opt[3];
  double bound, huber_a, inliner_dis, inlier_ratio, min_icp_R, min_icp_T;
  double inlier_threshold, angular_diff, t_diff, final_cost, initial_cost;
  int corner_avail, surf_avail, n_blocks, icp_done, icp_iter, num_residual_blocks, status, total_lm_iterations, total_evaluations;
  int n_unique; int if_motion_deblur;
  int cap, rng_seed, n_blocks_all;
  double min_ts, max_ts, interp_theta, interp_hat[9], interp_hat_sq[9];
  long long prof[16];
  LmState lm;
};

struct PinnedStage {
  RegDevState state_in;
  RegDevState snap[2];
  double x[7];
  double pose[7];
  double mapper_pose[7];
  double extract_time;
  int fe_counts[12];
  int fe_meta[3];
  int counts[3];
  float bounds[32];
};

#define LL_SYNC_ROWS 160
struct SolveSync {
  double rows[2][LL_SYNC_ROWS][32];
  double bcast[2][32];
  unsigned hist[6][2048]; unsigned list_cnt; unsigned _pad[63];
  double list[64];
  unsigned gen;
};

enum SolveMode : int {
  SOLVE_FIRST = 0,
  SOLVE_SECOND = 1,
  SOLVE_PLAIN = 2,
  SOLVE_EVALUATE = 3,
  SOLVE_FUSED = 4,
};
struct SolveArgs {
  RegDevState* st;
  SolveSync* sync;
  const float4* feat;
  const float4* blk_a;
  const double* blk_v;
  double* l1;
  const double* k10_value;
  const int* k10_n_distinct;
  int M;
  int max_iterations;
  SolveMode mode;
  int rank, world; double* comm_local; double* comm_peer[8];
  int prerun_iterations; unsigned long long* table; unsigned table_mask;
  int cap_check;
  int deblur;
};
#define LL_COMM_CTRL_OFF 8192
#define LL_COMM_X_OFF 16384
int launch_solve(ll_ctx* ctx, const SolveArgs& a);
int solve_capacity(ll_ctx* ctx, int M, int deblur);
int solve_prepare(ll_ctx* ctx);
int launch_k10_select(ll_ctx* ctx, const double* d_l1, int n, const double* d_ratio, unsigned long long* table, unsigned table_mask, double* d_value, int* d_n_distinct);
inline unsigned l1_set_capacity(int M) { unsigned cap = 1024; while (cap < (unsigned)(2 * M)) cap <<= 1; return cap; }
inline unsigned long long* l1_set_layout(Carve& c, int M) { return c.take<unsigned long long>(l1_set_capacity(M)); }
int launch_l1_exchange(ll_ctx* ctx, const double* d_l1, int M);
int launch_count_exchange(ll_ctx* ctx);

int upload_cloud(ll_ctx* ctx, const void* src, size_t n, int fmt, int where, float4* d_dst);
int launch_transform(ll_ctx* ctx, cudaStream_t s, const double* d_pose7, const float4* d_in, int n, float4* d_out);
int launch_pack_strided(ll_ctx* ctx, const float4* d_src, int n, unsigned char* d_dst);
int launch_voxel_grid(ll_ctx* ctx, cudaStream_t s, DevBuf& scratch, const float4* d_in, int n_cap, const int* d_n_in, float leaf, float4* d_out, int* d_n_out);
size_t voxel_grid_bytes(int n_cap);

int extract_alloc(ll_ctx* ctx);
int launch_extract_points(ll_ctx* ctx, int n);
int launch_extract_petals(ll_ctx* ctx, int n, cudaStream_t s, DevBuf& scratch);
int launch_get_features(ll_ctx* ctx, cudaStream_t s, DevBuf& scratch, const float* d_bounds , float min_blur, float max_blur,
                        float4* d_corners, float4* d_surf, float4* d_full, int* d_counts );
int launch_piece_bounds(ll_ctx* ctx, int pieces, float* d_start_end );
size_t petals_bytes(int n);
size_t get_features_bytes(int n);

int register_device(ll_ctx* ctx, const ll_map* map, int nc, int ns, const ll_reg_state* in, ll_reg_result* out);
int scan_front_end(ll_ctx* ctx, const void* raw, size_t n, int fmt, int where, double stamp, const ll_pipeline_cfg* pc, int* nc_out, int* ns_out, int* dropped);
```

loam_livox_b200/csrc/lm_core.cuh:

```cuda
#pragma once
#include <cfloat>
#include <cmath>
#ifdef __CUDACC__
#define LL_HD __device__
#define LL_INLINE __forceinline__
#define LL_NOINLINE __noinline__
#else
#define LL_HD
#define LL_INLINE inline
#define LL_NOINLINE
static inline double rsqrt(double x) { return 1.0 / std::sqrt(x); }
using std::isfinite;
#endif

#include "lm_state.h"

LL_HD void d_qmul(const double a[4], const double b[4], double o[4]) {
  o[0] = a[0] * b[0] - a[1] * b[1] - a[2] * b[2] - a[3] * b[3];
  o[1] = a[0] * b[1] + a[1] * b[0] + a[2] * b[3] - a[3] * b[2];
  o[2] = a[0] * b[2] + a[2] * b[0] + a[3] * b[1] - a[1] * b[3];
  o[3] = a[0] * b[3] + a[3] * b[0] + a[1] * b[2] - a[2] * b[1];
}
LL_HD void d_qrot(const double q[4], const double v[3], double o[3]) {
  double ux = q[1], uy = q[2], uz = q[3], w = q[0];
  double cx = uy * v[2] - uz * v[1], cy = uz * v[0] - ux * v[2], cz = ux * v[1] - uy * v[0];
  cx += cx; cy += cy; cz += cz;
  o[0] = v[0] + w * cx + (uy * cz - uz * cy); o[1] = v[1] + w * cy + (uz * cx - ux * cz); o[2] = v[2] + w * cz + (ux * cy - uy * cx);
}
LL_HD double d_angdist(const double a[4], const double b[4]) {
  double bc[4] = {b[0], -b[1], -b[2], -b[3]}, d[4]; d_qmul(a, bc, d);
  return 2.0 * atan2(sqrt(d[1] * d[1] + d[2] * d[2] + d[3] * d[3]), fabs(d[0]));
}
LL_HD void d_plus(const double x[7], const double delta[6], double bound, double out[7]) {
  double nd = sqrt(delta[0] * delta[0] + delta[1] * delta[1] + delta[2] * delta[2]);
  if (nd > 0.0) {
    double sn, cs; sincos(nd, &sn, &cs);
    const double sbd = sn / nd;
    double dq[4] = {cs, sbd * delta[0], sbd * delta[1], sbd * delta[2]}, q[4] = {x[3], x[0], x[1], x[2]}, r[4];
    d_qmul(dq, q, r); out[0] = r[1]; out[1] = r[2]; out[2] = r[3]; out[3] = r[0];
  } else { out[0] = x[0]; out[1] = x[1]; out[2] = x[2]; out[3] = x[3]; }
  for (int k = 0; k < 3; k++) { double v = x[4 + k] + delta[3 + k]; out[4 + k] = fmin(fmax(v, -bound), bound); }
}
LL_HD LL_INLINE bool d_chol6(const double A[6][6], const double b[6], double x[6]) {
  double L[6][6], inv[6];
#pragma unroll
  for (int i = 0; i < 6; i++)
#pragma unroll
    for (int j = 0; j < 6; j++) L[i][j] = 0;
  bool ok = true;
#pragma unroll
  for (int i = 0; i < 6; i++) {
#pragma unroll
    for (int j = 0; j <= i; j++) {
      double s = A[i][j];
#pragma unroll
      for (int k = 0; k < j; k++) s -= L[i][k] * L[j][k];
      if (i == j) { if (!(s > 0.0)) ok = false; inv[i] = rsqrt(s); L[i][i] = s * inv[i]; } else L[i][j] = s * inv[j];
    }
  }
  if (!ok) return false;
  double y[6];
#pragma unroll
  for (int i = 0; i < 6; i++) { double s = b[i];
#pragma unroll
    for (int k = 0; k < i; k++) s -= L[i][k] * y[k]; y[i] = s * inv[i]; }
#pragma unroll
  for (int i = 5; i >= 0; i--) { double s = y[i];
#pragma unroll
    for (int k = i + 1; k < 6; k++) s -= L[k][i] * x[k]; x[i] = s * inv[i]; }
#pragma unroll
  for (int i = 0; i < 6; i++) if (!isfinite(x[i])) ok = false;
  return ok;
}
LL_HD LL_INLINE int hidx(int i, int j) { return i * 6 - (i * (i - 1)) / 2 + (j - i); }

LL_HD double d_poly_eval(const double* p, int n, double x) { double v = 0; for (int i = 0; i < n; i++) v = v * x + p[i]; return v; }
LL_HD int d_fit_poly(const FnSample* s, int ns, double* coef) {
  int nc = 0; for (int i = 0; i < ns; i++) { if (s[i].value_valid) nc++; if (s[i].gradient_valid) nc++; }
  const int deg = nc - 1; double A[6][6], rhs[6]; int perm[6];
  int row = 0;
  for (int i = 0; i < ns; i++) {
    if (s[i].value_valid) { for (int j = 0; j <= deg; j++) A[row][j] = pow(s[i].x, (double)(deg - j)); rhs[row] = s[i].value; row++; }
    if (s[i].gradient_valid) { for (int j = 0; j <= deg; j++) A[row][j] = j < deg ? (deg - j) * pow(s[i].x, (double)(deg - j - 1)) : 0.0; rhs[row] = s[i].gradient; row++; }
  }
  for (int i = 0; i < nc; i++) perm[i] = i;
  for (int c = 0; c < nc; c++) {
    int pr = c, pc = c; double best = 0;
    for (int i = c; i < nc; i++) for (int j = c; j < nc; j++) if (fabs(A[i][j]) > best) { best = fabs(A[i][j]); pr = i; pc = j; }
    if (best == 0) break;
    for (int j = 0; j < nc; j++) { double t = A[c][j]; A[c][j] = A[pr][j]; A[pr][j] = t; }
    { double t = rhs[c]; rhs[c] = rhs[pr]; rhs[pr] = t; }
    for (int i = 0; i < nc; i++) { double t = A[i][c]; A[i][c] = A[i][pc]; A[i][pc] = t; }
    { int t = perm[c]; perm[c] = perm[pc]; perm[pc] = t; }
    for (int i = c + 1; i < nc; i++) { double f = A[i][c] / A[c][c]; for (int j = c; j < nc; j++) A[i][j] -= f * A[c][j]; rhs[i] -= f * rhs[c]; }
  }
  double y[6];
  for (int i = nc - 1; i >= 0; i--) { double sacc = rhs[i]; for (int j = i + 1; j < nc; j++) sacc -= A[i][j] * y[j]; y[i] = sacc / A[i][i]; }
  for (int i = 0; i < nc; i++) coef[perm[i]] = y[i];
  return nc;
}
LL_HD int d_root_real_parts(const double* pin, int n, double* out) {
  double p[6]; int m = 0; bool lead = true;
  for (int i = 0; i < n; i++) { if (lead && pin[i] == 0.0) continue; lead = false; p[m++] = pin[i]; }
  int deg = m - 1; if (deg < 1) return 0;
  if (deg == 1) { out[0] = -p[1] / p[0]; return 1; }
  if (deg == 2) {
    double a = p[0], b = p[1], c = p[2], D = b * b - 4 * a * c, sD = sqrt(fabs(D));
    if (D >= 0) { if (b >= 0) { out[0] = (-b - sD) / (2.0 * a); out[1] = (2.0 * c) / (-b - sD); } else { out[0] = (2.0 * c) / (-b + sD); out[1] = (-b + sD) / (2.0 * a); } }
    else { out[0] = -b / (2.0 * a); out[1] = out[0]; }
    return 2;
  }
  double zr[5], zi[5], cr[6]; for (int i = 0; i <= deg; i++) cr[i] = p[i] / p[0];
  double rad = 0; for (int i = 1; i <= deg; i++) rad = fmax(rad, fabs(cr[i])); rad = 1.0 + rad;
  for (int i = 0; i < deg; i++) { double ang = 2.0 * 3.14159265358979323846 * i / deg + 0.4; zr[i] = rad * 0.5 * cos(ang); zi[i] = rad * 0.5 * sin(ang); }
  for (int it = 0; it < 500; it++) {
    double change = 0;
    for (int i = 0; i < deg; i++) {
      double nr = 0, ni = 0; for (int k = 0; k <= deg; k++) { double tr = nr * zr[i] - ni * zi[i] + cr[k], ti = nr * zi[i] + ni * zr[i]; nr = tr; ni = ti; }
      double dr = 1, di = 0; for (int j = 0; j < deg; j++) if (j != i) { double ar = zr[i] - zr[j], ai = zi[i] - zi[j]; double tr = dr * ar - di * ai, ti = dr * ai + di * ar; dr = tr; di = ti; }
      double den = dr * dr + di * di; if (den == 0) { dr = 1e-300; di = 0; den = 1e-600 > 0 ? 1e-300 * 1e-300 : DBL_MIN; }
      double qr = (nr * dr + ni * di) / den, qi = (ni * dr - nr * di) / den;
      zr[i] -= qr; zi[i] -= qi; change = fmax(change, sqrt(qr * qr + qi * qi));
    }
    if (change < 1e-15 * rad) break;
  }
  for (int i = 0; i < deg; i++) out[i] = zr[i];
  return deg;
}
LL_HD double d_minimize_interp(const FnSample* s, int ns, double x_min, double x_max) {
  double coef[6]; int n = d_fit_poly(s, ns, coef);
  double ox = (x_min + x_max) / 2.0, ov = d_poly_eval(coef, n, ox);
  double v = d_poly_eval(coef, n, x_min); if (v < ov) { ov = v; ox = x_min; }
  v = d_poly_eval(coef, n, x_max); if (v < ov) { ov = v; ox = x_max; }
  if (n <= 2) return ox;
  double der[5]; int deg = n - 1; for (int i = 0; i < deg; i++) der[i] = (deg - i) * coef[i];
  double roots[5]; int nr = d_root_real_parts(der, deg, roots);
  for (int i = 0; i < nr; i++) { double r = roots[i]; if (!(r >= x_min && r <= x_max)) continue; v = d_poly_eval(coef, n, r); if (v < ov) { ov = v; ox = r; } }
  return ox;
}

#define LM_FTOL 1e-6
#define LM_GTOL 1e-10
#define LM_PTOL 1e-8

LL_HD double lm_gmax(const LmState& L, double bound) {
  double ng[6], pg[7]; for (int c = 0; c < 6; c++) ng[c] = -L.g[c];
  d_plus(L.x, ng, bound, pg); double m = 0; for (int k = 0; k < 7; k++) m = fmax(m, fabs(L.x[k] - pg[k])); return m;
}
LL_HD void lm_finish(LmState& L, int termination) {
  L.done = 1; L.termination = termination; L.final_cost = fmin(L.initial_cost, L.min_iter_cost);
}
struct StepIn { double H[21], g[6], x[7], scaling[6], diagonal[6], radius; int reuse_diagonal; };
struct StepOut { double delta[6], trial[7], diagonal[6], model_cost_change, gd, dmax; int valid; };
LL_HD LL_NOINLINE void compute_step(const StepIn& I, double bound, StepOut& O) {
  for (int c = 0; c < 6; c++) { if (I.reuse_diagonal) O.diagonal[c] = I.diagonal[c]; else { double d = I.H[hidx(c, c)] * I.scaling[c] * I.scaling[c]; O.diagonal[c] = fmin(fmax(d, 1e-6), 1e32); } }
  double A[6][6], rhs[6], Hs[6][6];
  for (int i = 0; i < 6; i++) { rhs[i] = I.g[i] * I.scaling[i]; for (int j = i; j < 6; j++) { double v = I.H[hidx(i, j)] * I.scaling[i] * I.scaling[j]; Hs[i][j] = v; Hs[j][i] = v; } }
  for (int i = 0; i < 6; i++) for (int j = 0; j < 6; j++) A[i][j] = Hs[i][j];
  { const double inv_radius = 1.0 / I.radius; for (int c = 0; c < 6; c++) A[c][c] += O.diagonal[c] * inv_radius; }
  double step[6]; const bool solved = d_chol6(A, rhs, step);
  O.valid = 0; O.model_cost_change = 0; O.gd = 0; O.dmax = 0;
  if (solved) {
    for (int c = 0; c < 6; c++) step[c] = -step[c];
    double sg = 0, shs = 0; for (int i = 0; i < 6; i++) { sg += step[i] * rhs[i]; double r = 0; for (int j = 0; j < 6; j++) r += Hs[i][j] * step[j]; shs += step[i] * r; }
    O.model_cost_change = -sg - 0.5 * shs; O.valid = O.model_cost_change > 0.0 ? 1 : 0;
  }
  if (!O.valid) return;
  for (int c = 0; c < 6; c++) { O.delta[c] = step[c] * I.scaling[c]; O.gd += I.g[c] * O.delta[c]; O.dmax = fmax(O.dmax, fabs(O.delta[c])); }
  d_plus(I.x, O.delta, bound, O.trial);
}
LL_HD LL_INLINE double radius_after_success(double radius, double rel) {
  const double c1 = 2.0 * rel - 1.0; radius = radius / fmax(1.0 / 3.0, 1.0 - c1 * c1 * c1); return fmin(1e16, radius);
}
LL_HD void lm_hypothesis(const LmState& L, const double* sums, int h, StepIn& I) {
  if (L.phase == 0 || h == 0) {
    for (int i = 0; i < 21; i++) I.H[i] = sums[i]; for (int i = 0; i < 6; i++) I.g[i] = sums[21 + i]; for (int k = 0; k < 7; k++) I.x[k] = L.trial[k];
    if (L.phase == 0) { for (int c = 0; c < 6; c++) I.scaling[c] = 1.0 / (1.0 + sqrt(I.H[hidx(c, c)])); I.radius = 1e4; }
    else { for (int c = 0; c < 6; c++) I.scaling[c] = L.scaling[c]; I.radius = radius_after_success(L.radius, (L.x_cost - sums[27]) / L.model_cost_change); }
    for (int c = 0; c < 6; c++) I.diagonal[c] = 0.0; I.reuse_diagonal = 0;
  } else {
    for (int i = 0; i < 21; i++) I.H[i] = L.H[i]; for (int i = 0; i < 6; i++) I.g[i] = L.g[i]; for (int k = 0; k < 7; k++) I.x[k] = L.x[k];
    for (int c = 0; c < 6; c++) { I.scaling[c] = L.scaling[c]; I.diagonal[c] = L.diagonal[c]; }
    I.radius = L.radius / L.decrease_factor; I.reuse_diagonal = 1;
  }
}
LL_HD void lm_next_iteration(LmState& L, double bound, const StepOut* pre) {
  for (;;) {
    if (L.iteration >= L.max_iterations) { lm_finish(L, 0); return; }
    if (L.last_successful && L.last_gmax <= LM_GTOL) { lm_finish(L, 1); return; }
    if (L.radius <= 1e-32) { lm_finish(L, 5); return; }
    L.iteration++; L.total_iterations++;
    StepOut tmp; const StepOut* so = pre; pre = nullptr;
    if (!so) {
      StepIn in; for (int i = 0; i < 21; i++) in.H[i] = L.H[i]; for (int i = 0; i < 6; i++) { in.g[i] = L.g[i]; in.scaling[i] = L.scaling[i]; in.diagonal[i] = L.diagonal[i]; }
      for (int k = 0; k < 7; k++) in.x[k] = L.x[k]; in.radius = L.radius; in.reuse_diagonal = L.reuse_diagonal;
      compute_step(in, bound, tmp); so = &tmp;
    }
    for (int c = 0; c < 6; c++) L.diagonal[c] = so->diagonal[c];
    L.reuse_diagonal = 1;
    if (!so->valid) {
      if (++L.num_invalid >= 5) { lm_finish(L, 4); return; }
      L.radius = L.radius / L.decrease_factor; L.decrease_factor *= 2.0; L.reuse_diagonal = 1; L.last_successful = 0; continue;
    }
    L.num_invalid = 0;
    L.model_cost_change = so->model_cost_change; L.gd = so->gd; L.dmax = so->dmax;
    for (int c = 0; c < 6; c++) L.delta[c] = so->delta[c];
    for (int k = 0; k < 7; k++) L.trial[k] = so->trial[k];
    L.ls_iters = 0; L.prev.value_valid = 0; L.prev.gradient_valid = 0; L.ls_alpha = 1.0;
    L.phase = 1; return;
  }
}
LL_HD void lm_accept_test(LmState& L, const double* sums, double bound, bool defer_gmax) {
  const double cand_cost = sums[27];
  double step_norm = 0; for (int k = 0; k < 7; k++) step_norm += (L.x[k] - L.trial[k]) * (L.x[k] - L.trial[k]); step_norm = sqrt(step_norm);
  if (step_norm <= LM_PTOL * (L.x_norm + LM_PTOL)) { lm_finish(L, 2); return; }
  const double cost_change = L.x_cost - cand_cost;
  if (fabs(cost_change) <= LM_FTOL * L.x_cost) { lm_finish(L, 3); return; }
  const double rel = (L.x_cost - cand_cost) / L.model_cost_change;
  if (rel > 1e-3) {
    for (int k = 0; k < 7; k++) L.x[k] = L.trial[k];
    double n = 0; for (int k = 0; k < 7; k++) n += L.x[k] * L.x[k]; L.x_norm = sqrt(n);
    L.x_cost = cand_cost; for (int i = 0; i < 21; i++) L.H[i] = sums[i]; for (int i = 0; i < 6; i++) L.g[i] = sums[21 + i];
    if (!defer_gmax) L.last_gmax = lm_gmax(L, bound);
    L.last_successful = 1;
    L.radius = radius_after_success(L.radius, rel);
    L.decrease_factor = 2.0; L.reuse_diagonal = 0;
    L.min_iter_cost = fmin(L.min_iter_cost, L.x_cost);
    if (L.x_cost < L.minimum_cost) { L.minimum_cost = L.x_cost; for (int k = 0; k < 7; k++) L.x_best[k] = L.x[k]; }
    L.pending = 0;
  } else {
    L.radius = L.radius / L.decrease_factor; L.decrease_factor *= 2.0; L.reuse_diagonal = 1; L.last_successful = 0;
    L.min_iter_cost = fmin(L.min_iter_cost, cand_cost);
    L.pending = 1;
  }
}
LL_HD LL_NOINLINE void lm_step(LmState& L, const double* sums, double bound, bool defer_gmax) {
  L.total_evaluations++; L.pending = -1;
  if (L.phase == 0) {
    for (int k = 0; k < 7; k++) { L.x[k] = L.trial[k]; L.x_best[k] = L.trial[k]; }
    double n = 0; for (int k = 0; k < 7; k++) n += L.x[k] * L.x[k]; L.x_norm = sqrt(n);
    L.x_cost = sums[27]; for (int i = 0; i < 21; i++) L.H[i] = sums[i]; for (int i = 0; i < 6; i++) L.g[i] = sums[21 + i];
    L.n_valid = (int)(sums[28] + 0.5);
    L.initial_cost = L.x_cost; L.min_iter_cost = L.x_cost; L.minimum_cost = L.x_cost; L.final_cost = L.x_cost;
    for (int c = 0; c < 6; c++) L.scaling[c] = 1.0 / (1.0 + sqrt(L.H[hidx(c, c)]));
    if (!defer_gmax) L.last_gmax = lm_gmax(L, bound);
    L.last_successful = 1; L.iteration = 0; L.radius = 1e4; L.decrease_factor = 2.0; L.reuse_diagonal = 0; L.num_invalid = 0;
    if (L.n_valid == 0) { lm_finish(L, -1); return; }
    if (!isfinite(L.x_cost)) { lm_finish(L, 4); return; }
    L.pending = 0; return;
  }
  if (L.phase == 1) {
    double gt = 0; for (int c = 0; c < 6; c++) gt += sums[21 + c] * L.delta[c];
    L.cur.x = L.ls_alpha; L.cur.value = sums[27]; L.cur.gradient = gt; L.cur.value_valid = isfinite(sums[27]) ? 1 : 0; L.cur.gradient_valid = (L.cur.value_valid && isfinite(gt)) ? 1 : 0;
    if (L.cur.value_valid && !(L.cur.value > L.x_cost + 1e-4 * L.gd * L.cur.x)) {
      for (int c = 0; c < 6; c++) L.delta[c] *= L.cur.x;
      lm_accept_test(L, sums, bound, defer_gmax); return;
    }
    bool failed = false; double step_size = 0;
    if (++L.ls_iters >= 20) failed = true;
    else {
      const double mn = 1e-3 * L.cur.x, mx = 0.6 * L.cur.x;
      if (!L.cur.value_valid) step_size = fmin(fmax(L.cur.x * 0.5, mn), mx);
      else {
        FnSample s[3]; int ns = 0;
        s[ns].x = 0; s[ns].value = L.x_cost; s[ns].gradient = L.gd; s[ns].value_valid = 1; s[ns].gradient_valid = 1; ns++;
        s[ns++] = L.cur; if (L.prev.value_valid) s[ns++] = L.prev;
        step_size = d_minimize_interp(s, ns, mn, mx);
      }
      if (step_size * L.dmax < 1e-9) failed = true;
    }
    if (!failed) { L.prev = L.cur; L.ls_alpha = step_size; double sd[6]; for (int c = 0; c < 6; c++) sd[c] = step_size * L.delta[c]; d_plus(L.x, sd, bound, L.trial); return; }
    if (L.cur.x == 1.0) { lm_accept_test(L, sums, bound, defer_gmax); return; }
    d_plus(L.x, L.delta, bound, L.trial); L.phase = 2; return;
  }
  lm_accept_test(L, sums, bound, defer_gmax);
}
```

loam_livox_b200/csrc/solve.cu:

```cuda
#include <cfloat>
#include <cstdlib>
#include "common.cuh"
#include "kernels.cuh"
#include "exact_math.cuh"

#define FULL 0xffffffffu
#define NSUM 29
#define SOLVE_THREADS 256

__device__ __forceinline__ unsigned ld_acquire_u32(const unsigned* p) { unsigned v; asm volatile("ld.acquire.gpu.global.u32 %0, [%1];" : "=r"(v) : "l"(p) : "memory"); return v; }
__device__ __forceinline__ void st_release_u32(unsigned* p, unsigned v) { asm volatile("st.release.gpu.global.u32 [%0], %1;" ::"l"(p), "r"(v) : "memory"); }
__device__ __forceinline__ unsigned ld_acquire_sys_u32(const unsigned* p) { unsigned v; asm volatile("ld.acquire.sys.global.u32 %0, [%1];" : "=r"(v) : "l"(p) : "memory"); return v; }
__device__ __forceinline__ void st_release_sys_u32(unsigned* p, unsigned v) { asm volatile("st.release.sys.global.u32 [%0], %1;" ::"l"(p), "r"(v) : "memory"); }

#include "lm_core.cuh"

struct Slot { double px, py, pz, ax, ay, az, vx, vy, vz; double s; int type; };

struct EvalConst {
  double x[7];
  double PJ[4][3];
  double Rl[3][3];
  double tl[3];
  double huber_a, huber_b;
  double sl_theta, sl_sin, sl_cos, sl_dth_dw; int sl_lerp;
};

__device__ __forceinline__ void cross3(double ax, double ay, double az, double bx, double by, double bz, double& ox, double& oy, double& oz) {
  ox = ay * bz - az * by; oy = az * bx - ax * bz; oz = ax * by - ay * bx;
}
template <bool MB>
__device__ __forceinline__ void eval_block(const Slot& s, const EvalConst& E, double r[3], double J[6][3], bool want_j) {
  double ux = E.x[0], uy = E.x[1], uz = E.x[2], w = E.x[3];
  double sc1 = 1.0, dsc0 = 0.0, dsc1 = 0.0, ts = 1.0;
  if (MB) {
    const double sb = s.s; double sc0;
    if (E.sl_lerp) { sc0 = 1.0 - sb; sc1 = sb; }
    else {
      double s0, c0, s1, c1; sincos((1.0 - sb) * E.sl_theta, &s0, &c0); sincos(sb * E.sl_theta, &s1, &c1);
      const double inv = 1.0 / E.sl_sin;
      sc0 = s0 * inv; sc1 = s1 * inv;
      dsc0 = ((1.0 - sb) * c0 * E.sl_sin - s0 * E.sl_cos) * inv * inv * E.sl_dth_dw;
      dsc1 = (sb * c1 * E.sl_sin - s1 * E.sl_cos) * inv * inv * E.sl_dth_dw;
    }
    if (E.x[3] < 0.0) { sc1 = -sc1; dsc1 = -dsc1; }
    ux *= sc1; uy *= sc1; uz *= sc1; w = sc0 + sc1 * E.x[3]; ts = sb;
  }
  double cx, cy, cz; cross3(ux, uy, uz, s.px, s.py, s.pz, cx, cy, cz); cx += cx; cy += cy; cz += cz;
  double ex, ey, ez; cross3(ux, uy, uz, cx, cy, cz, ex, ey, ez);
  const double yx = s.px + w * cx + ex + ts * E.x[4], yy = s.py + w * cy + ey + ts * E.x[5], yz = s.pz + w * cz + ez + ts * E.x[6];
  const double dx = E.Rl[0][0] * yx + E.Rl[0][1] * yy + E.Rl[0][2] * yz + E.tl[0] - s.ax;
  const double dy = E.Rl[1][0] * yx + E.Rl[1][1] * yy + E.Rl[1][2] * yz + E.tl[1] - s.ay;
  const double dz = E.Rl[2][0] * yx + E.Rl[2][1] * yy + E.Rl[2][2] * yz + E.tl[2] - s.az;
  const double dv = dx * s.vx + dy * s.vy + dz * s.vz;
  const bool line = s.type == 1;
  if (line) { r[0] = dx - dv * s.vx; r[1] = dy - dv * s.vy; r[2] = dz - dv * s.vz; }
  else { r[0] = dv * s.vx; r[1] = dv * s.vy; r[2] = dv * s.vz; }
  if (!want_j) return;
#pragma unroll
  for (int c = 0; c < 6; c++) {
    double gx, gy, gz;
    if (c < 3) {
      double dux = E.PJ[0][c], duy = E.PJ[1][c], duz = E.PJ[2][c], dw = E.PJ[3][c];
      if (MB) {
        const double k1 = dsc1 * dw;
        dux = k1 * E.x[0] + sc1 * dux; duy = k1 * E.x[1] + sc1 * duy; duz = k1 * E.x[2] + sc1 * duz;
        dw = dsc0 * dw + k1 * E.x[3] + sc1 * dw;
      }
      double ax, ay, az; cross3(dux, duy, duz, s.px, s.py, s.pz, ax, ay, az); ax += ax; ay += ay; az += az;
      double bx, by, bz; cross3(dux, duy, duz, cx, cy, cz, bx, by, bz);
      double fx, fy, fz; cross3(ux, uy, uz, ax, ay, az, fx, fy, fz);
      gx = dw * cx + w * ax + bx + fx; gy = dw * cy + w * ay + by + fy; gz = dw * cz + w * az + bz + fz;
    } else { gx = c == 3 ? ts : 0.0; gy = c == 4 ? ts : 0.0; gz = c == 5 ? ts : 0.0; }
    const double e0 = E.Rl[0][0] * gx + E.Rl[0][1] * gy + E.Rl[0][2] * gz;
    const double e1 = E.Rl[1][0] * gx + E.Rl[1][1] * gy + E.Rl[1][2] * gz;
    const double e2 = E.Rl[2][0] * gx + E.Rl[2][1] * gy + E.Rl[2][2] * gz;
    const double ev = e0 * s.vx + e1 * s.vy + e2 * s.vz;
    if (line) { J[c][0] = e0 - ev * s.vx; J[c][1] = e1 - ev * s.vy; J[c][2] = e2 - ev * s.vz; }
    else { J[c][0] = ev * s.vx; J[c][1] = ev * s.vy; J[c][2] = ev * s.vz; }
  }
}
__device__ __forceinline__ double huber_weight(double sq, double a, double b, double& rho0) {
  if (sq > b) { double r = sqrt(sq); rho0 = 2.0 * a * r - b; return fmax(DBL_MIN, a / r); }
  rho0 = sq; return 1.0;
}

__device__ void setup_static(EvalConst& E, const RegDevState* st) {
  const double* ql = st->pose_last;
  for (int k = 0; k < 3; k++) { double e[3] = {k == 0 ? 1.0 : 0.0, k == 1 ? 1.0 : 0.0, k == 2 ? 1.0 : 0.0}, o[3]; d_qrot(ql, e, o); E.Rl[0][k] = o[0]; E.Rl[1][k] = o[1]; E.Rl[2][k] = o[2]; }
  E.tl[0] = st->pose_last[4]; E.tl[1] = st->pose_last[5]; E.tl[2] = st->pose_last[6];
  E.huber_a = st->huber_a; E.huber_b = st->huber_a * st->huber_a;
}
template <bool MB>
__device__ __forceinline__ void setup_trial(EvalConst& E, const double* x) {
  for (int k = 0; k < 7; k++) E.x[k] = x[k];
  E.PJ[0][0] = x[3];  E.PJ[0][1] = x[2];  E.PJ[0][2] = -x[1];
  E.PJ[1][0] = -x[2]; E.PJ[1][1] = x[3];  E.PJ[1][2] = x[0];
  E.PJ[2][0] = x[1];  E.PJ[2][1] = -x[0]; E.PJ[2][2] = x[3];
  E.PJ[3][0] = -x[0]; E.PJ[3][1] = -x[1]; E.PJ[3][2] = -x[2];
  if (MB) { const double d = x[3], ad = fabs(d);
    if (ad >= 1.0 - 2.220446049250313e-16) { E.sl_lerp = 1; E.sl_theta = 0; E.sl_sin = 1; E.sl_cos = 1; E.sl_dth_dw = 0; }
    else { E.sl_lerp = 0; E.sl_theta = acos(ad); E.sl_sin = sin(E.sl_theta); E.sl_cos = cos(E.sl_theta); E.sl_dth_dw = -(d < 0.0 ? -1.0 : 1.0) / sqrt(1.0 - ad * ad); } }
}

struct FastSlot { double px, py, pz, ax, ay, az, wx, wy, wz; int type; };
__device__ __forceinline__ void fast_residual(const FastSlot& s, const EvalConst& E, double y[3], double r[3], double& alpha) {
  const double ux = E.x[0], uy = E.x[1], uz = E.x[2], w = E.x[3];
  double cx, cy, cz; cross3(ux, uy, uz, s.px, s.py, s.pz, cx, cy, cz); cx += cx; cy += cy; cz += cz;
  double ex, ey, ez; cross3(ux, uy, uz, cx, cy, cz, ex, ey, ez);
  y[0] = s.px + w * cx + ex; y[1] = s.py + w * cy + ey; y[2] = s.pz + w * cz + ez;
  const double dx = y[0] + E.x[4] - s.ax, dy = y[1] + E.x[5] - s.ay, dz = y[2] + E.x[6] - s.az;
  alpha = dx * s.wx + dy * s.wy + dz * s.wz;
  if (s.type == 1) { r[0] = dx - alpha * s.wx; r[1] = dy - alpha * s.wy; r[2] = dz - alpha * s.wz; }
  else { r[0] = alpha * s.wx; r[1] = alpha * s.wy; r[2] = alpha * s.wz; }
}
__device__ __forceinline__ void fast_accumulate(const FastSlot& s, const EvalConst& E, double acc[NSUM]) {
  double y[3], r[3], alpha; fast_residual(s, E, y, r, alpha);
  double rho0; const double wgt = huber_weight(r[0] * r[0] + r[1] * r[1] + r[2] * r[2], E.huber_a, E.huber_b, rho0);
  acc[27] += 0.5 * rho0; acc[28] += 1.0;
  const bool line = s.type == 1;
  const double wn2 = s.wx * s.wx + s.wy * s.wy + s.wz * s.wz;
  double b[6]; cross3(y[0], y[1], y[2], s.wx, s.wy, s.wz, b[0], b[1], b[2]); b[0] += b[0]; b[1] += b[1]; b[2] += b[2]; b[3] = s.wx; b[4] = s.wy; b[5] = s.wz;
  double rr[3], cg;
  if (line) { const double wr = s.wx * r[0] + s.wy * r[1] + s.wz * r[2]; rr[0] = r[0] - wr * s.wx; rr[1] = r[1] - wr * s.wy; rr[2] = r[2] - wr * s.wz; cg = wgt; }
  else { rr[0] = r[0]; rr[1] = r[1]; rr[2] = r[2]; cg = wgt * wn2; }
  double g0, g1, g2; cross3(y[0], y[1], y[2], rr[0], rr[1], rr[2], g0, g1, g2);
  acc[21] += cg * (g0 + g0); acc[22] += cg * (g1 + g1); acc[23] += cg * (g2 + g2); acc[24] += cg * rr[0]; acc[25] += cg * rr[1]; acc[26] += cg * rr[2];
  const double cb = line ? -wgt * (2.0 - wn2) : wgt * wn2;
  int h = 0;
#pragma unroll
  for (int i = 0; i < 6; i++) {
#pragma unroll
    for (int j = i; j < 6; j++) { acc[h] += cb * b[i] * b[j]; h++; }
  }
  if (line) {
    const double yy = y[0] * y[0] + y[1] * y[1] + y[2] * y[2], w4 = 4.0 * wgt, w2 = 2.0 * wgt;
    acc[0] += w4 * (yy - y[0] * y[0]); acc[1] -= w4 * y[0] * y[1]; acc[2] -= w4 * y[0] * y[2];
    acc[4] -= w2 * y[2]; acc[5] += w2 * y[1];
    acc[6] += w4 * (yy - y[1] * y[1]); acc[7] -= w4 * y[1] * y[2];
    acc[8] += w2 * y[2]; acc[10] -= w2 * y[0];
    acc[11] += w4 * (yy - y[2] * y[2]);
    acc[12] -= w2 * y[1]; acc[13] += w2 * y[0];
    acc[15] += wgt; acc[18] += wgt; acc[20] += wgt;
  }
}

template <int OFF>
__device__ __forceinline__ void butterfly_level(double (&w)[32], int lane) {
  const bool upper = (lane & OFF) != 0;
#pragma unroll
  for (int i = 0; i < OFF; i++) {
    const double send = upper ? w[i] : w[i + OFF];
    const double keep = upper ? w[i + OFF] : w[i];
    w[i] = keep + __shfl_xor_sync(FULL, send, OFF);
  }
}

struct SmemSlots { float* p[3]; float* a[3]; double* v[3]; double* ap[3]; int* type; float* s; };
__device__ __forceinline__ SmemSlots carve(unsigned char* base, int cap, bool mb) {
  SmemSlots s; double* d = (double*)base;
  s.v[0] = d; s.v[1] = d + cap; s.v[2] = d + 2 * cap; d += 3 * (size_t)cap;
  if (!mb) { s.ap[0] = d; s.ap[1] = d + cap; s.ap[2] = d + 2 * cap; d += 3 * (size_t)cap; } else { s.ap[0] = s.ap[1] = s.ap[2] = nullptr; }
  float* f = (float*)d;
  s.p[0] = f; s.p[1] = f + cap; s.p[2] = f + 2 * cap; f += 3 * (size_t)cap;
  if (mb) { s.a[0] = f; s.a[1] = f + cap; s.a[2] = f + 2 * cap; f += 3 * (size_t)cap; s.s = f; f += cap; } else { s.a[0] = s.a[1] = s.a[2] = nullptr; s.s = nullptr; }
  s.type = (int*)f;
  return s;
}
#define SLOT_BYTES 64
#define SLOT_BYTES_MB 56

__device__ __forceinline__ double* sync_row(SolveSync* Y, unsigned gen, int cta) { return Y->rows[gen & 1u][cta]; }
__device__ __forceinline__ void sync_arrive(SolveSync* Y, unsigned gen) {
  st_release_u32((unsigned*)(sync_row(Y, gen, blockIdx.x) + 31), gen);
}
__device__ __forceinline__ void sync_wait_all(SolveSync* Y, unsigned gen) {
  if (threadIdx.x < gridDim.x) { const unsigned* f = (const unsigned*)(sync_row(Y, gen, threadIdx.x) + 31); while (ld_acquire_u32(f) != gen) {} }
  __syncthreads();
}
__device__ __forceinline__ void grid_sync(SolveSync* Y, unsigned& gen) {
  gen++;
  __syncthreads();
  if (threadIdx.x == 0) sync_arrive(Y, gen);
  sync_wait_all(Y, gen);
}

#define K10_PASSES 6
#define L1_EMPTY 0xffffffffffffffffull

__device__ __forceinline__ unsigned long long l1_key(double v) { return (unsigned long long)__double_as_longlong(v == 0.0 ? 0.0 : v); }
__device__ __forceinline__ bool l1_set_insert_flag(unsigned long long* __restrict__ table, unsigned table_mask, double v, bool valid) {
  if (!(valid && v < INFINITY)) return false;
  const unsigned long long key = l1_key(v);
  unsigned h = (unsigned)((key * 0x9E3779B97F4A7C15ull) >> 40) & table_mask;
  for (;;) {
    const unsigned long long prev = atomicCAS(&table[h], L1_EMPTY, key);
    if (prev == L1_EMPTY) return true;
    if (prev == key) return false;
    h = (h + 1) & table_mask;
  }
}
__device__ __forceinline__ double k10_threshold(double inliner_dis, double value, int n_distinct) { return fmax(inliner_dis, n_distinct > 0 ? value : 0.0); }
struct K10Smem { unsigned hist[2048]; unsigned warp_sum[SOLVE_THREADS / 32 + 1]; unsigned long long prefix, mask; int k, cnt_bin, n_distinct, done; int scratch[40]; double result; };

__device__ __forceinline__ void k10_clear(unsigned long long* table, unsigned table_mask, SolveSync* Y) {
  for (unsigned idx = blockIdx.x * SOLVE_THREADS + threadIdx.x; idx <= table_mask; idx += gridDim.x * SOLVE_THREADS) table[idx] = L1_EMPTY;
  for (unsigned idx = blockIdx.x * SOLVE_THREADS + threadIdx.x; idx < K10_PASSES * 2048u + 64u; idx += gridDim.x * SOLVE_THREADS) ((unsigned*)Y->hist)[idx] = 0u;
}

__device__ __forceinline__ void k10_select(K10Smem& s_k10, SolveSync* Y, unsigned& gen, const int* type, const double* l1, int M, int tiles_per_cta, int tile, const double* ratio) {
  const int tid = threadIdx.x, lane = tid & 31, warp = tid >> 5;
  if (tid == 0) { s_k10.prefix = 0ull; s_k10.mask = 0ull; s_k10.k = -1; s_k10.done = 0; s_k10.result = 0.0; }
  __syncthreads();
  for (int pass = 0; pass < K10_PASSES && !s_k10.done; pass++) {
    const int shift = pass < 5 ? 52 - 11 * pass : 0; const unsigned dmask = pass < 5 ? 2047u : 255u;
    for (int b = tid; b < 2048; b += SOLVE_THREADS) s_k10.hist[b] = 0u;
    __syncthreads();
    const unsigned long long prefix = s_k10.prefix, himask = s_k10.mask;
    for (int k = 0; k < tiles_per_cta; k++) {
      const int i = (blockIdx.x + gridDim.x * k) * tile + tid, li = k * SOLVE_THREADS + tid;
      if (i < M && tid < tile && (type[li] & 0x100)) {
        const unsigned long long key = l1_key(l1[i]);
        if ((key & himask) == prefix) atomicAdd(&s_k10.hist[(unsigned)(key >> shift) & dmask], 1u);
      }
    }
    __syncthreads();
    unsigned* gh = Y->hist[pass];
    for (int b = tid; b < 2048; b += SOLVE_THREADS) { const unsigned c = s_k10.hist[b]; if (c) atomicAdd(&gh[b], c); }
    grid_sync(Y, gen);
    constexpr int BPT = 2048 / SOLVE_THREADS;
    unsigned h[BPT], run = 0;
#pragma unroll
    for (int b = 0; b < BPT; b++) { h[b] = __ldcg(&gh[tid * BPT + b]); run += h[b]; }
    unsigned incl = run;
#pragma unroll
    for (int o = 1; o < 32; o <<= 1) { const unsigned v = __shfl_up_sync(FULL, incl, o); if (lane >= o) incl += v; }
    if (lane == 31) s_k10.warp_sum[warp] = incl;
    __syncthreads();
    if (tid == 0) { unsigned t = 0; for (int w = 0; w < SOLVE_THREADS / 32; w++) { const unsigned c = s_k10.warp_sum[w]; s_k10.warp_sum[w] = t; t += c; } s_k10.warp_sum[SOLVE_THREADS / 32] = t; }
    __syncthreads();
    if (pass == 0 && tid == 0) {
      const int n = (int)s_k10.warp_sum[SOLVE_THREADS / 32]; s_k10.n_distinct = n;
      int k = (int)(*ratio * (double)n); if (k > n - 1) k = n - 1; s_k10.k = k;
      if (n == 0) s_k10.done = 1;
    }
    __syncthreads();
    if (!s_k10.done) {
      const unsigned excl = s_k10.warp_sum[warp] + incl - run; const unsigned k = (unsigned)s_k10.k;
      __syncthreads();
      if (k >= excl && k < excl + run) {
        unsigned below = excl; int j = 0;
#pragma unroll
        for (int b = 0; b < BPT; b++) { if (k >= below + h[b] && j == b) { below += h[b]; j = b + 1; } }
        const int jj = j < BPT ? j : BPT - 1;
        s_k10.k = (int)(k - below); s_k10.cnt_bin = (int)h[jj];
        s_k10.prefix = prefix | ((unsigned long long)(tid * BPT + jj) << shift);
        s_k10.mask = himask | ((unsigned long long)dmask << shift);
      }
      __syncthreads();
      if (s_k10.cnt_bin <= 64 || pass == K10_PASSES - 1) {
        const unsigned long long pf = s_k10.prefix, hm = s_k10.mask;
        for (int kk = 0; kk < tiles_per_cta; kk++) {
          const int i = (blockIdx.x + gridDim.x * kk) * tile + tid, li = kk * SOLVE_THREADS + tid;
          if (i < M && tid < tile && (type[li] & 0x100)) {
            const double v = l1[i];
            if ((l1_key(v) & hm) == pf) { const unsigned slot = atomicAdd(&Y->list_cnt, 1u); if (slot < 64u) Y->list[slot] = v; }
          }
        }
        grid_sync(Y, gen);
        {
          double* cand = (double*)s_k10.hist;
          const int m = min((int)*((volatile unsigned*)&Y->list_cnt), 64);
          if (tid < m) cand[tid] = __ldcg(&Y->list[tid]);
          __syncthreads();
          if (tid < m) { const double mine = cand[tid]; int rank = 0; for (int q = 0; q < m; q++) rank += (cand[q] < mine) ? 1 : 0; if (rank == s_k10.k) s_k10.result = mine; }
          if (tid == 0) s_k10.done = 1;
        }
        __syncthreads();
      }
    }
  }
}

template <bool MB>
__global__ void __launch_bounds__(SOLVE_THREADS, 2) lm_solve_kernel(SolveArgs a, int tiles_per_cta, int tile) {
  extern __shared__ __align__(16) unsigned char s_dyn[];
  __shared__ EvalConst E;
  __shared__ double s_red[SOLVE_THREADS / 32][NSUM + 1];
  __shared__ double s_sum[32];
  __shared__ LmState s_lm;
  __shared__ double s_gmax;
  __shared__ StepOut s_pre[2];
  __shared__ K10Smem s_k10;
  __shared__ long long s_prof[16];
  RegDevState* st = a.st;
  SolveSync* Y = a.sync;
  if ((a.mode == SOLVE_FUSED || a.mode <= SOLVE_SECOND) && *((volatile int*)&st->icp_done)) return;
  const int tid = threadIdx.x, lane = tid & 31, warp = tid >> 5;
  const int cap = tiles_per_cta * SOLVE_THREADS;
  const SmemSlots S = carve(s_dyn, cap, MB);
  const bool master = blockIdx.x == 0;
  unsigned gen = *((volatile unsigned*)&Y->gen);
  if (tid < 16) s_prof[tid] = 0;

  const long long t_k0 = clock64();
  const bool fused = a.mode == SOLVE_FUSED;
  SolveMode cur_mode = fused ? SOLVE_FIRST : a.mode;
  if (fused) k10_clear(a.table, a.table_mask, Y);
  double thr = 0;
  if (a.mode == SOLVE_SECOND) {
    thr = k10_threshold(st->inliner_dis, *a.k10_value, *a.k10_n_distinct);
    if (master && tid == 0) st->inlier_threshold = thr;
  }
  float cap_keep = 2.0f; int cap_iter = 0, cap_seed = 0;
  if (a.cap_check) {
    const int nb = a.world > 1 ? st->n_blocks_all : st->n_blocks;
    if (nb > st->cap) cap_keep = (float)st->cap / (float)nb;
    cap_iter = st->icp_iter; cap_seed = st->rng_seed;
  }
  for (int k = 0; k < tiles_per_cta; k++) {
    const int i = (blockIdx.x + gridDim.x * k) * tile + tid, li = k * SOLVE_THREADS + tid;
    int type = 0;
    if (i < a.M && tid < tile) {
      const float4 ba = a.blk_a[i]; type = __float_as_int(ba.w);
      if (type != 0 && cap_keep <= 1.0f && ll_cap_uniform_f(cap_seed, cap_iter, 2, i) > cap_keep) type = 0;
      if (type != 0 && a.mode == SOLVE_SECOND && (a.l1[i] > thr)) type = 0;
      if (type != 0) {
        const float4 f = a.feat[i];
        S.p[0][li] = f.x; S.p[1][li] = f.y; S.p[2][li] = f.z;
        const double v0 = a.blk_v[(size_t)i * 3], v1 = a.blk_v[(size_t)i * 3 + 1], v2 = a.blk_v[(size_t)i * 3 + 2];
        if (MB) {
          S.a[0][li] = ba.x; S.a[1][li] = ba.y; S.a[2][li] = ba.z; S.v[0][li] = v0; S.v[1][li] = v1; S.v[2][li] = v2;
          S.s[li] = refine_blur_f(f.w, (float)st->min_ts, (float)st->max_ts);
        } else {
          const double qc[4] = {st->pose_last[0], -st->pose_last[1], -st->pose_last[2], -st->pose_last[3]};
          double vin[3] = {v0, v1, v2}, o[3]; d_qrot(qc, vin, o); S.v[0][li] = o[0]; S.v[1][li] = o[1]; S.v[2][li] = o[2];
          double ain[3] = {(double)ba.x - st->pose_last[4], (double)ba.y - st->pose_last[5], (double)ba.z - st->pose_last[6]}; d_qrot(qc, ain, o);
          S.ap[0][li] = o[0]; S.ap[1][li] = o[1]; S.ap[2][li] = o[2];
        }
      }
    }
    S.type[li] = type;
  }
  const double bound = st->bound;
  double x_start[7]; for (int k = 0; k < 7; k++) x_start[k] = st->x[k];
  for (int ph = 0; ph < (fused ? 2 : 1); ph++) {
  if (tid == 0) {
    double z[6] = {0, 0, 0, 0, 0, 0}, tr[7];
    if (ph == 1) for (int k = 0; k < 7; k++) x_start[k] = s_lm.x_best[k];
    d_plus(x_start, z, bound, tr);
    if (ph == 0) setup_static(E, st);
    setup_trial<MB>(E, tr);
    LmState& L = s_lm;
    L.phase = 0; L.iteration = 0; L.max_iterations = (fused && ph == 0) ? a.prerun_iterations : a.max_iterations; L.num_invalid = 0; L.done = 0; L.termination = 0; L.last_successful = 1; L.reuse_diagonal = 0;
    L.ls_iters = 0; L.n_valid = 0; L.total_iterations = 0; L.total_evaluations = 0; L.pending = -1;
    for (int k = 0; k < 7; k++) { L.trial[k] = tr[k]; L.x_best[k] = tr[k]; }
  }
  __syncthreads();

  if (master && tid == 0 && ph == 0) s_prof[6] += clock64() - t_k0;
  for (;;) {
    const long long t_e0 = clock64();
    double acc[NSUM];
#pragma unroll
    for (int i = 0; i < NSUM; i++) acc[i] = 0.0;
    for (int k = 0; k < tiles_per_cta; k++) {
      const int li = k * SOLVE_THREADS + tid;
      const int type = S.type[li];
      if (!MB) {
        if (type != 0) {
          FastSlot fs; fs.type = type; fs.px = S.p[0][li]; fs.py = S.p[1][li]; fs.pz = S.p[2][li]; fs.ax = S.ap[0][li]; fs.ay = S.ap[1][li]; fs.az = S.ap[2][li];
          fs.wx = S.v[0][li]; fs.wy = S.v[1][li]; fs.wz = S.v[2][li];
          fast_accumulate(fs, E, acc);
        }
        continue;
      }
      Slot s; s.type = type;
      if (s.type != 0) {
        s.px = S.p[0][li]; s.py = S.p[1][li]; s.pz = S.p[2][li]; s.ax = S.a[0][li]; s.ay = S.a[1][li]; s.az = S.a[2][li];
        s.vx = S.v[0][li]; s.vy = S.v[1][li]; s.vz = S.v[2][li];
        s.s = (double)S.s[li];
        double r[3], J[6][3]; eval_block<true>(s, E, r, J, true);
        double rho0; const double wgt = huber_weight(r[0] * r[0] + r[1] * r[1] + r[2] * r[2], E.huber_a, E.huber_b, rho0);
        acc[27] += 0.5 * rho0; acc[28] += 1.0;
        int h = 0;
#pragma unroll
        for (int i = 0; i < 6; i++) {
          acc[21 + i] += wgt * (J[i][0] * r[0] + J[i][1] * r[1] + J[i][2] * r[2]);
#pragma unroll
          for (int j = i; j < 6; j++) { acc[h] += wgt * (J[i][0] * J[j][0] + J[i][1] * J[j][1] + J[i][2] * J[j][2]); h++; }
        }
      }
    }
    if (__any_sync(FULL, acc[28] != 0.0)) {
      double w[32];
#pragma unroll
      for (int i = 0; i < 32; i++) w[i] = i < NSUM ? acc[i] : 0.0;
      butterfly_level<16>(w, lane); butterfly_level<8>(w, lane); butterfly_level<4>(w, lane); butterfly_level<2>(w, lane); butterfly_level<1>(w, lane);
      if (lane < NSUM) s_red[warp][lane] = w[0];
    } else if (lane < NSUM) s_red[warp][lane] = 0.0;
    __syncthreads();
    gen++;
    if (warp == 0) {
      if (lane < NSUM) { double v = 0; for (int wq = 0; wq < SOLVE_THREADS / 32; wq++) v += s_red[wq][lane]; sync_row(Y, gen, blockIdx.x)[lane] = v; }
      __syncwarp();
      if (lane == 0) sync_arrive(Y, gen);
    }
    const long long t_e1 = clock64();
    sync_wait_all(Y, gen);
    const long long t_e2 = clock64();
    {
      constexpr int G = SOLVE_THREADS / 32, RMAX = (LL_SYNC_ROWS + G - 1) / G;
      static_assert(RMAX % 4 == 0, "the row loop below runs whole groups of four");
      const int val = tid & 31, grp = tid >> 5, nb = (int)gridDim.x;
      const int n = grp < nb ? (nb - grp + G - 1) / G : 0;
      if (val < NSUM) {
        double r[RMAX];
#pragma unroll
        for (int j = 0; j < RMAX; j++) r[j] = j < n ? __ldcg(&sync_row(Y, gen, grp + j * G)[val]) : 0.0;
        double v0 = 0, v1 = 0, v2 = 0, v3 = 0;
        const int whole = n & ~3;
#pragma unroll
        for (int j = 0; j < RMAX; j += 4) if (j < whole) { v0 += r[j]; v1 += r[j + 1]; v2 += r[j + 2]; v3 += r[j + 3]; }
#pragma unroll
        for (int j = 0; j < RMAX; j++) if (j >= whole && j < n) v0 += r[j];
        s_red[grp][val] = (v0 + v1) + (v2 + v3);
      }
      __syncthreads();
      if (tid < NSUM) { double t = 0; for (int g = 0; g < G; g++) t += s_red[g][tid]; s_sum[tid] = t; }
      __syncthreads();
    }
    if (a.world > 1) {
      if (master && warp == 0) {
        unsigned* cgen = (unsigned*)((char*)a.comm_local + LL_COMM_CTRL_OFF);
        const unsigned g1 = *cgen + 1; const int par = g1 & 1;
        for (int p = 0; p < a.world; p++) {
          double* dst = a.comm_peer[p] + ((size_t)par * 8 + a.rank) * 64;
          if (lane < NSUM) dst[lane] = s_sum[lane];
        }
        __threadfence_system();
        __syncwarp();
        if (lane < a.world) st_release_sys_u32((unsigned*)(a.comm_peer[lane] + ((size_t)par * 8 + a.rank) * 64 + 32), g1);
        if (lane < a.world) { const unsigned* f = (const unsigned*)(a.comm_local + ((size_t)par * 8 + lane) * 64 + 32); while (ld_acquire_sys_u32(f) != g1) {} }
        __syncwarp();
        double t = 0;
        if (lane < NSUM) for (int p = 0; p < a.world; p++) t += *((volatile double*)(a.comm_local + ((size_t)par * 8 + p) * 64 + lane));
        if (lane < NSUM) Y->bcast[gen & 1u][lane] = t;
        if (lane == 0) *cgen = g1;
        __syncwarp();
        if (lane == 0) { __threadfence(); st_release_u32((unsigned*)&Y->bcast[gen & 1u][31], gen); }
      }
      if (tid == 0) { const unsigned* f = (const unsigned*)&Y->bcast[gen & 1u][31]; while (ld_acquire_u32(f) != gen) {} }
      __syncthreads();
      if (tid < NSUM) s_sum[tid] = __ldcg(&Y->bcast[gen & 1u][tid]);
      __syncthreads();
    }
    const long long t_e3 = clock64();
    if (cur_mode == SOLVE_EVALUATE) {
      if (tid == 0) { LmState& L = s_lm; for (int i = 0; i < 21; i++) L.H[i] = s_sum[i]; for (int i = 0; i < 6; i++) L.g[i] = s_sum[21 + i]; L.x_cost = s_sum[27]; L.n_valid = (int)(s_sum[28] + 0.5); L.done = 1; }
    } else {
      StepIn in; double gx[7], gg[6];
      if (warp == 1 && lane < 2) lm_hypothesis(s_lm, s_sum, lane, in);
      if (tid == 64) { for (int k = 0; k < 7; k++) gx[k] = s_lm.trial[k]; for (int c = 0; c < 6; c++) gg[c] = -s_sum[21 + c]; }
      __syncthreads();
      const long long t_h0 = clock64();
      if (warp == 1 && lane < 2) { compute_step(in, bound, s_pre[lane]); if (master && lane == 0) s_prof[13] += clock64() - t_h0; }
      else if (tid == 0) { lm_step(s_lm, s_sum, bound, true); if (master) s_prof[14] += clock64() - t_h0; }
      else if (tid == 64) {
        double pg[7]; d_plus(gx, gg, bound, pg); double mx = 0; for (int k = 0; k < 7; k++) mx = fmax(mx, fabs(gx[k] - pg[k])); s_gmax = mx;
      }
      __syncthreads();
      if (tid == 0 && s_lm.pending == 0) s_lm.last_gmax = s_gmax;
      if (master && tid == 0) s_prof[15] += clock64() - t_h0;
      if (tid == 0 && s_lm.pending >= 0) lm_next_iteration(s_lm, bound, &s_pre[s_lm.pending]);
    }
    if (tid == 0) { if (!*(volatile int*)&s_lm.done) setup_trial<MB>(E, s_lm.trial); }
    __syncthreads();
    if (master && tid == 0) { const long long t_e4 = clock64(); s_prof[0] += t_e1 - t_e0; s_prof[1] += t_e2 - t_e1; s_prof[2] += t_e3 - t_e2; s_prof[3] += t_e4 - t_e3; s_prof[5] += 1; }
    if (s_lm.done) break;
  }
  if (tid == 0) {
    LmState& L = s_lm;
    setup_trial<MB>(E, L.x_best);
    if (master) {
      st->lm = L;
      if (cur_mode != SOLVE_EVALUATE) {
        for (int k = 0; k < 7; k++) st->x[k] = L.x_best[k];
        st->total_lm_iterations += L.iteration; st->total_evaluations += L.total_evaluations;
      }
      if (cur_mode == SOLVE_SECOND) {
        double qi[4] = {L.x_best[3], L.x_best[0], L.x_best[1], L.x_best[2]}, ti[3] = {L.x_best[4], L.x_best[5], L.x_best[6]};
        const double* ql = st->pose_last; double tcur[3], qcur[4];
        d_qrot(ql, ti, tcur); for (int k = 0; k < 3; k++) tcur[k] += st->pose_last[4 + k];
        d_qmul(ql, qi, qcur);
        for (int k = 0; k < 4; k++) st->pose_curr[k] = qcur[k]; for (int k = 0; k < 3; k++) st->pose_curr[4 + k] = tcur[k];
        st->angular_diff = (double)((float)d_angdist(qcur, ql)) * 57.3;
        double td = 0; for (int k = 0; k < 3; k++) td += (tcur[k] - st->pose_last[4 + k]) * (tcur[k] - st->pose_last[4 + k]); st->t_diff = sqrt(td);
        if (MB) {
          double n = sqrt(qi[1] * qi[1] + qi[2] * qi[2] + qi[3] * qi[3]), ax[3], ang;
          if (n != 0.0) { ang = 2.0 * atan2(n, fabs(qi[0])); if (qi[0] < 0) n = -n; ax[0] = qi[1] / n; ax[1] = qi[2] / n; ax[2] = qi[3] / n; }
          else { ang = 0; ax[0] = 1; ax[1] = 0; ax[2] = 0; }
          const double an = sqrt(ax[0] * ax[0] + ax[1] * ax[1] + ax[2] * ax[2]); for (int k = 0; k < 3; k++) ax[k] /= an;
          double* H = st->interp_hat; for (int k = 0; k < 9; k++) H[k] = 0;
          H[1] = -ax[2]; H[3] = ax[2]; H[2] = ax[1]; H[6] = -ax[1]; H[5] = -ax[0]; H[7] = ax[0];
          for (int i = 0; i < 3; i++) for (int j = 0; j < 3; j++) { double t = 0; for (int k = 0; k < 3; k++) t += H[i * 3 + k] * H[k * 3 + j]; st->interp_hat_sq[i * 3 + j] = t; }
          st->interp_theta = ang;
        }
        if (L.termination == -1) st->icp_done = 1;
        st->final_cost = L.final_cost; st->initial_cost = L.initial_cost; st->num_residual_blocks = L.n_valid;
        double dt = 0; for (int k = 0; k < 3; k++) dt += (st->t_last_opt[k] - ti[k]) * (st->t_last_opt[k] - ti[k]);
        if (d_angdist(st->q_last_opt, qi) < 57.3 * st->min_icp_R && sqrt(dt) < st->min_icp_T) st->icp_done = 1;
        else { for (int k = 0; k < 4; k++) st->q_last_opt[k] = qi[k]; for (int k = 0; k < 3; k++) st->t_last_opt[k] = ti[k]; }
        st->icp_iter++;
      }
    }
  }
  __syncthreads();
  const long long t_p0 = clock64();
  if (cur_mode == SOLVE_FIRST) {
    for (int k = 0; k < tiles_per_cta; k++) {
      const int i = (blockIdx.x + gridDim.x * k) * tile + tid, li = k * SOLVE_THREADS + tid;
      double my_l1 = INFINITY;
      if (i < a.M && tid < tile) {
        double l1 = INFINITY;
        Slot s; s.type = S.type[li] & 0xff;
        if (s.type != 0) {
          double r[3];
          if (MB) {
            s.px = S.p[0][li]; s.py = S.p[1][li]; s.pz = S.p[2][li]; s.ax = S.a[0][li]; s.ay = S.a[1][li]; s.az = S.a[2][li];
            s.vx = S.v[0][li]; s.vy = S.v[1][li]; s.vz = S.v[2][li];
            s.s = (double)S.s[li];
            double J[6][3]; eval_block<true>(s, E, r, J, false);
          } else {
            FastSlot fs; fs.type = s.type; fs.px = S.p[0][li]; fs.py = S.p[1][li]; fs.pz = S.p[2][li]; fs.ax = S.ap[0][li]; fs.ay = S.ap[1][li]; fs.az = S.ap[2][li];
            fs.wx = S.v[0][li]; fs.wy = S.v[1][li]; fs.wz = S.v[2][li];
            double y[3], rp[3], alpha; fast_residual(fs, E, y, rp, alpha);
            r[0] = E.Rl[0][0] * rp[0] + E.Rl[0][1] * rp[1] + E.Rl[0][2] * rp[2];
            r[1] = E.Rl[1][0] * rp[0] + E.Rl[1][1] * rp[1] + E.Rl[1][2] * rp[2];
            r[2] = E.Rl[2][0] * rp[0] + E.Rl[2][1] * rp[1] + E.Rl[2][2] * rp[2];
          }
          double rho0; const double wgt = huber_weight(r[0] * r[0] + r[1] * r[1] + r[2] * r[2], E.huber_a, E.huber_b, rho0);
          const double sc = sqrt(wgt);
          l1 = fabs(sc * r[0]) + fabs(sc * r[1]) + fabs(sc * r[2]);
        }
        a.l1[i] = l1;
        my_l1 = l1;
      }
      if (fused && l1_set_insert_flag(a.table, a.table_mask, my_l1, my_l1 < INFINITY)) S.type[li] |= 0x100;
    }
  }
  if (fused && ph == 0) {
    const long long q0 = clock64();
    k10_select(s_k10, Y, gen, S.type, a.l1, a.M, tiles_per_cta, tile, &st->inlier_ratio);
    const double thr2 = k10_threshold(st->inliner_dis, s_k10.result, s_k10.n_distinct);
    if (master && tid == 0) { st->inlier_threshold = thr2; st->n_unique = s_k10.n_distinct; }
    const long long q3 = clock64();
    for (int k = 0; k < tiles_per_cta; k++) {
      const int i = (blockIdx.x + gridDim.x * k) * tile + tid, li = k * SOLVE_THREADS + tid;
      if (i < a.M && tid < tile) { const int t = S.type[li] & 0xff; S.type[li] = (t != 0 && a.l1[i] > thr2) ? 0 : t; }
    }
    cur_mode = SOLVE_SECOND;
    __syncthreads();
    if (master && tid == 0) { const long long q4 = clock64(); s_prof[8] += q0 - t_p0; s_prof[10] += q3 - q0; s_prof[12] += q4 - q3; }
  }
  if (master && tid == 0) s_prof[7] += clock64() - t_p0;
  }
  if (master && tid == 0) {
    *((volatile unsigned*)&Y->gen) = gen;
    for (int k = 0; k < 16; k++) st->prof[k] += s_prof[k];
  }
}

#define SOLVE_MAX_SMEM (200 * 1024)

int solve_prepare(ll_ctx* ctx) {
  LL_CUDA(ctx, cudaFuncSetAttribute((void*)lm_solve_kernel<true>, cudaFuncAttributeMaxDynamicSharedMemorySize, SOLVE_MAX_SMEM));
  LL_CUDA(ctx, cudaFuncSetAttribute((void*)lm_solve_kernel<false>, cudaFuncAttributeMaxDynamicSharedMemorySize, SOLVE_MAX_SMEM));
  if (!ctx->d_sync) {
    void* p = nullptr; LL_CUDA(ctx, cudaMalloc(&p, sizeof(SolveSync))); LL_CUDA(ctx, cudaMemset(p, 0, sizeof(SolveSync))); ctx->d_sync = (SolveSync*)p;
  }
  return LL_OK;
}
struct SolveGrid { int tile, tiles_per_cta, grid; };
static SolveGrid solve_grid(const ll_ctx* ctx, int M) {
  const int M1 = M > 0 ? M : 1;
  SolveGrid g;
  g.tile = ((ll_div_up(M1, ctx->num_sms) + 31) / 32) * 32; if (g.tile > SOLVE_THREADS) g.tile = SOLVE_THREADS;
  const int tiles = ll_div_up(M1, g.tile);
  g.grid = tiles < ctx->num_sms ? tiles : ctx->num_sms; if (g.grid > LL_SYNC_ROWS) g.grid = LL_SYNC_ROWS;
  g.tiles_per_cta = ll_div_up(tiles, g.grid);
  return g;
}
static size_t solve_smem_bytes(const SolveGrid& sg, int deblur) { return (size_t)sg.tiles_per_cta * SOLVE_THREADS * (deblur ? SLOT_BYTES_MB : SLOT_BYTES); }
int solve_capacity(ll_ctx* ctx, int M, int deblur) {
  if (solve_smem_bytes(solve_grid(ctx, M), deblur) > SOLVE_MAX_SMEM) { ctx->set_error("too many residual-block slots for the shared-memory-resident solver"); return LL_ERR_CAPACITY; }
  return LL_OK;
}
int launch_solve(ll_ctx* ctx, const SolveArgs& a) {
  const SolveGrid sg = solve_grid(ctx, a.M);
  int tile = sg.tile, tiles_per_cta = sg.tiles_per_cta; const int grid = sg.grid;
  const int mb = a.deblur ? 1 : 0;
  LL_TRY(solve_capacity(ctx, a.M, mb));
  const size_t smem = solve_smem_bytes(sg, mb);
  void* fn = mb ? (void*)lm_solve_kernel<true> : (void*)lm_solve_kernel<false>;
  SolveArgs args = a; args.sync = ctx->d_sync; void* kargs[] = {&args, &tiles_per_cta, &tile};
  LL_CUDA(ctx, cudaLaunchCooperativeKernel(fn, dim3(grid), dim3(SOLVE_THREADS), kargs, smem, ctx->stream));
  ctx->launches++;
  return LL_OK;
}

__global__ void __launch_bounds__(SOLVE_THREADS) k10_select_kernel(SolveSync* Y, const double* l1, int n, const double* ratio, unsigned long long* table, unsigned table_mask,
                                                                   int tiles_per_cta, int tile, double* value, int* n_distinct) {
  extern __shared__ int s_flag[];
  __shared__ K10Smem s_k10;
  const int tid = threadIdx.x;
  unsigned gen = *((volatile unsigned*)&Y->gen);
  k10_clear(table, table_mask, Y);
  grid_sync(Y, gen);
  for (int k = 0; k < tiles_per_cta; k++) {
    const int i = (blockIdx.x + gridDim.x * k) * tile + tid, li = k * SOLVE_THREADS + tid;
    const double v = (i < n && tid < tile) ? l1[i] : INFINITY;
    s_flag[li] = l1_set_insert_flag(table, table_mask, v, v < INFINITY) ? 0x100 : 0;
  }
  k10_select(s_k10, Y, gen, s_flag, l1, n, tiles_per_cta, tile, ratio);
  if (blockIdx.x == 0 && tid == 0) {
    *value = s_k10.n_distinct > 0 ? s_k10.result : 0.0; *n_distinct = s_k10.n_distinct;
    *((volatile unsigned*)&Y->gen) = gen;
  }
}
int launch_k10_select(ll_ctx* ctx, const double* d_l1, int n, const double* d_ratio, unsigned long long* table, unsigned table_mask, double* d_value, int* d_n_distinct) {
  const SolveGrid sg = solve_grid(ctx, n);
  int tile = sg.tile, tiles_per_cta = sg.tiles_per_cta;
  SolveSync* Y = ctx->d_sync;
  const size_t smem = (size_t)tiles_per_cta * SOLVE_THREADS * sizeof(int);
  if (smem > 48 * 1024) LL_CUDA(ctx, cudaFuncSetAttribute((void*)k10_select_kernel, cudaFuncAttributeMaxDynamicSharedMemorySize, (int)smem));
  void* kargs[] = {&Y, &d_l1, &n, &d_ratio, &table, &table_mask, &tiles_per_cta, &tile, &d_value, &d_n_distinct};
  LL_CUDA(ctx, cudaLaunchCooperativeKernel((void*)k10_select_kernel, dim3(sg.grid), dim3(SOLVE_THREADS), kargs, smem, ctx->stream));
  ctx->launches++;
  return LL_OK;
}


struct L1ExchangeArgs { const double* l1; int M; int rank, world; char* comm_local; char* comm_peer[8]; };
__global__ void __launch_bounds__(256) l1_exchange_kernel(L1ExchangeArgs a) {
  const int i = blockIdx.x * blockDim.x + threadIdx.x;
  if (i < a.M) {
    const double v = a.l1[i];
    if (v < INFINITY) for (int p = 0; p < a.world; p++) ((double*)(a.comm_peer[p] + LL_COMM_X_OFF))[i] = v;
  }
  __threadfence_system();
  __syncthreads();
  if (threadIdx.x != 0) return;
  unsigned* ctrl = (unsigned*)(a.comm_local + LL_COMM_CTRL_OFF);
  if (atomicAdd(&ctrl[2], 1u) != gridDim.x - 1) return;
  ctrl[2] = 0u;
  const unsigned g = ctrl[1] + 1u; ctrl[1] = g;
  __threadfence_system();
  for (int p = 0; p < a.world; p++) st_release_sys_u32((unsigned*)(a.comm_peer[p] + LL_COMM_CTRL_OFF) + 16 + a.rank, g);
  for (int p = 0; p < a.world; p++) { const unsigned* f = ctrl + 16 + p; while (ld_acquire_sys_u32(f) != g) {} }
}
struct CountExchangeArgs { RegDevState* st; int rank, world; char* comm_local; char* comm_peer[8]; };
__global__ void count_exchange_kernel(CountExchangeArgs a) {
  const int lane = threadIdx.x;
  unsigned* ctrl = (unsigned*)(a.comm_local + LL_COMM_CTRL_OFF);
  const unsigned g = ctrl[3] + 1u; const int par = g & 1u;
  if (lane < a.world) {
    unsigned* pc = (unsigned*)(a.comm_peer[lane] + LL_COMM_CTRL_OFF);
    pc[64 + par * 8 + a.rank] = (unsigned)a.st->n_blocks;
    __threadfence_system();
    st_release_sys_u32(pc + 80 + a.rank, g);
    while (ld_acquire_sys_u32(ctrl + 80 + lane) != g) {}
  }
  __syncwarp();
  if (lane == 0) {
    int tot = 0; for (int p = 0; p < a.world; p++) tot += (int)*((volatile unsigned*)(ctrl + 64 + par * 8 + p));
    a.st->n_blocks_all = tot; ctrl[3] = g;
  }
}
int launch_count_exchange(ll_ctx* ctx) {
  if (ctx->world <= 1) return LL_OK;
  CountExchangeArgs a; a.st = ctx->d_reg; a.rank = ctx->rank; a.world = ctx->world; a.comm_local = (char*)ctx->comm_local;
  for (int i = 0; i < 8; i++) a.comm_peer[i] = (char*)ctx->comm_peers[i];
  count_exchange_kernel<<<1, 32, 0, ctx->stream>>>(a); ctx->launches++;
  LL_CUDA(ctx, cudaGetLastError());
  return LL_OK;
}
int launch_l1_exchange(ll_ctx* ctx, const double* d_l1, int M) {
  if (ctx->world <= 1 || M == 0) return LL_OK;
  L1ExchangeArgs a; a.l1 = d_l1; a.M = M; a.rank = ctx->rank; a.world = ctx->world; a.comm_local = (char*)ctx->comm_local;
  for (int i = 0; i < 8; i++) a.comm_peer[i] = (char*)ctx->comm_peers[i];
  l1_exchange_kernel<<<ll_div_up(M, 256), 256, 0, ctx->stream>>>(a); ctx->launches++;
  LL_CUDA(ctx, cudaGetLastError());
  return LL_OK;
}
```

Measured before the change: 865.8.

## Warp-parallelize LM step Cholesky, iteration bookkeeping, and refine k10 select histogram

Replaces the single-thread LM step computation, which did a 6x6 Cholesky solve per hypothesis, with a warp-cooperative version that distributes the lower-triangle entries across lanes via shuffles. The LM iteration loop and trial setup also run cooperatively across a warp. In the k10 inlier-select kernel, a fine-grained per-exponent histogram is built during the first pass so the target bin can be narrowed without extra passes. The change adds shared memory, global atomics on the fine table, and a parity-test entry point comparing the serial and warp step results. It risks small floating-point differences because of FMA use and a different operation order.

```diff
diff --git a/include/loamlivox_b200.h b/include/loamlivox_b200.h
--- a/include/loamlivox_b200.h
+++ b/include/loamlivox_b200.h
@@ -125,6 +125,7 @@
 int ll_set_blocks(ll_ctx* ctx, const ll_reg_state* in, size_t n, const int32_t* type, const ll_point* p, const float* a3, const double* v3);
 int ll_solve_fused(ll_ctx* ctx, int prerun, int max_iterations, double x_io[7], double* threshold, int* n_distinct, int* n_kept, double* l1_out,
                    int iterations[2]);
+int ll_lm_step_parity(ll_ctx* ctx, const double* in, size_t n, double bound, double* out_serial, double* out_warp);
 
 typedef struct {
   float  line_res, plane_res;
diff --git a/loam_livox_b200/capi.py b/loam_livox_b200/capi.py
--- a/loam_livox_b200/capi.py
+++ b/loam_livox_b200/capi.py
@@ -17,7 +17,7 @@
 EXPORTS = [
     "ll_config_default", "ll_ctx_create", "ll_ctx_destroy", "ll_ctx_warmup", "ll_last_error", "ll_ctx_stream", "ll_ctx_sync", "ll_extract", "ll_extract_reset", "ll_piece_bounds",
     "ll_get_features", "ll_extract_point_info", "ll_extract_split_idx", "ll_voxel_downsample", "ll_map_build", "ll_map_release", "ll_map_size",
-    "ll_map_build_sharded", "ll_knn", "ll_reg_state_default", "ll_register", "ll_build_blocks", "ll_normal_equations", "ll_solve", "ll_inlier_select", "ll_set_blocks", "ll_solve_fused", "ll_transform",
+    "ll_map_build_sharded", "ll_knn", "ll_reg_state_default", "ll_register", "ll_build_blocks", "ll_normal_equations", "ll_solve", "ll_inlier_select", "ll_set_blocks", "ll_solve_fused", "ll_lm_step_parity", "ll_transform",
     "ll_scan_to_pose", "ll_comm_local_handle", "ll_comm_connect", "ll_launch_count", "ll_cellmap_create", "ll_cellmap_release", "ll_cellmap_append",
     "ll_cellmap_assemble", "ll_cellmap_reserve", "ll_cellmap_stats", "ll_voxel_downsample_dev", "ll_transform_dev", "ll_last_features_dev", "ll_mapper_config_default", "ll_mapper_create", "ll_mapper_release",
     "ll_mapper_process_scan", "ll_mapper_pose", "ll_map_rebuild", "ll_debug_solver_cycles", "ll_state_snapshot_bytes", "ll_set_point_layout", "ll_format_pose_log", "ll_reg_state_yaml", "ll_cap_uniform", "ll_map_shard_info", "ll_shard_plan", "ll_align_cfg_default", "ll_scene_align", "ll_frame_to_pose", "ll_features_to_pointcloud2",
@@ -132,6 +132,7 @@
     L.ll_inlier_select.argtypes = [vp, vp, sz, cd, C.POINTER(cd), C.POINTER(ci)]
     L.ll_set_blocks.argtypes = [vp, C.POINTER(RegState), sz, vp, vp, vp, vp]
     L.ll_solve_fused.argtypes = [vp, ci, ci, vp, C.POINTER(cd), C.POINTER(ci), C.POINTER(ci), vp, vp]
+    L.ll_lm_step_parity.argtypes = [vp, vp, sz, cd, vp, vp]
     L.ll_transform.argtypes = [vp, vp, vp, vp, sz, ci, ci, vp]
     L.ll_scan_to_pose.argtypes = [vp, vp, vp, sz, ci, ci, cd, C.POINTER(PipelineCfg), C.POINTER(RegState), C.POINTER(RegResult), C.POINTER(ci), C.POINTER(ci)]
     L.ll_frame_to_pose.argtypes = [vp, vp, ci, vp, vp, ci, ci, vp, C.POINTER(PipelineCfg), C.POINTER(RegState), C.POINTER(RegResult), C.POINTER(ci), C.POINTER(ci)]
diff --git a/loam_livox_b200/csrc/api.cu b/loam_livox_b200/csrc/api.cu
--- a/loam_livox_b200/csrc/api.cu
+++ b/loam_livox_b200/csrc/api.cu
@@ -591,6 +591,20 @@
   if (iterations) { iterations[1] = hs->lm.iteration; iterations[0] = hs->total_lm_iterations - hs->lm.iteration; }
   return LL_OK;
 }
+int ll_lm_step_parity(ll_ctx* ctx, const double* in, size_t n, double bound, double* out_serial, double* out_warp) {
+  if (!ctx || (n > 0 && (!in || !out_serial || !out_warp)) || n > (1u << 24)) return LL_ERR_INVALID;
+  if (n == 0) return LL_OK;
+  cudaSetDevice(ctx->device);
+  cudaStream_t s = ctx->stream;
+  double *d_in = nullptr, *d_s = nullptr, *d_w = nullptr;
+  LL_CUDA(ctx, ctx->scratch.carve([&](Carve& c) { d_in = c.take<double>(n * LL_STEP_IN_DOUBLES); d_s = c.take<double>(n * LL_STEP_OUT_DOUBLES); d_w = c.take<double>(n * LL_STEP_OUT_DOUBLES); }));
+  LL_CUDA(ctx, cudaMemcpyAsync(d_in, in, n * LL_STEP_IN_DOUBLES * sizeof(double), cudaMemcpyHostToDevice, s));
+  LL_TRY(launch_lm_step_parity(ctx, d_in, (int)n, bound, d_s, d_w));
+  LL_CUDA(ctx, cudaMemcpyAsync(out_serial, d_s, n * LL_STEP_OUT_DOUBLES * sizeof(double), cudaMemcpyDeviceToHost, s));
+  LL_CUDA(ctx, cudaMemcpyAsync(out_warp, d_w, n * LL_STEP_OUT_DOUBLES * sizeof(double), cudaMemcpyDeviceToHost, s));
+  LL_CUDA(ctx, cudaStreamSynchronize(s));
+  return LL_OK;
+}
 int ll_inlier_select(ll_ctx* ctx, const double* l1, size_t n, double ratio, double* value, int* n_distinct) {
   if (!ctx || (n > 0 && !l1) || !value || !n_distinct || !(ratio >= 0.0)) return LL_ERR_INVALID;
   for (size_t i = 0; i < n; i++) if (l1[i] < 0.0) { ctx->set_error("L1 norms are never negative"); return LL_ERR_INVALID; }
diff --git a/loam_livox_b200/csrc/kernels.cuh b/loam_livox_b200/csrc/kernels.cuh
--- a/loam_livox_b200/csrc/kernels.cuh
+++ b/loam_livox_b200/csrc/kernels.cuh
@@ -69,12 +69,17 @@
 };
 
 #define LL_SYNC_ROWS 160
+#define K10_FINE_E0 983u
+#define K10_FINE_EXPS 64u
+#define K10_FINE_SHIFT 43
+#define K10_FINE_BINS 512
 struct SolveSync {
   double rows[2][LL_SYNC_ROWS][32];
   double bcast[2][32];
   unsigned hist[6][2048]; unsigned list_cnt; unsigned _pad[63];
   double list[64];
   unsigned gen;
+  alignas(16) unsigned fine[K10_FINE_EXPS][K10_FINE_BINS];
 };
 
 enum SolveMode : int {
@@ -107,6 +112,9 @@
 int solve_capacity(ll_ctx* ctx, int M, int deblur);
 int solve_prepare(ll_ctx* ctx);
 int launch_k10_select(ll_ctx* ctx, const double* d_l1, int n, const double* d_ratio, unsigned long long* table, unsigned table_mask, double* d_value, int* d_n_distinct);
+#define LL_STEP_IN_DOUBLES 48
+#define LL_STEP_OUT_DOUBLES 23
+int launch_lm_step_parity(ll_ctx* ctx, const double* d_in, int n, double bound, double* d_out_serial, double* d_out_warp);
 inline unsigned l1_set_capacity(int M) { unsigned cap = 1024; while (cap < (unsigned)(2 * M)) cap <<= 1; return cap; }
 inline unsigned long long* l1_set_layout(Carve& c, int M) { return c.take<unsigned long long>(l1_set_capacity(M)); }
 int launch_l1_exchange(ll_ctx* ctx, const double* d_l1, int M);
diff --git a/loam_livox_b200/csrc/lm_core.cuh b/loam_livox_b200/csrc/lm_core.cuh
--- a/loam_livox_b200/csrc/lm_core.cuh
+++ b/loam_livox_b200/csrc/lm_core.cuh
@@ -5,10 +5,12 @@
 #define LL_HD __device__
 #define LL_INLINE __forceinline__
 #define LL_NOINLINE __noinline__
+#define LL_SYNCWARP() __syncwarp()
 #else
 #define LL_HD
 #define LL_INLINE inline
 #define LL_NOINLINE
+#define LL_SYNCWARP()
 static inline double rsqrt(double x) { return 1.0 / std::sqrt(x); }
 using std::isfinite;
 #endif
@@ -169,47 +171,147 @@
   for (int c = 0; c < 6; c++) { O.delta[c] = step[c] * I.scaling[c]; O.gd += I.g[c] * O.delta[c]; O.dmax = fmax(O.dmax, fabs(O.delta[c])); }
   d_plus(I.x, O.delta, bound, O.trial);
 }
+#ifdef __CUDACC__
+__device__ __forceinline__ int tri6(int r, int c) { return r * (r + 1) / 2 + c; }
+__device__ LL_NOINLINE void compute_step_warp(const StepIn& I, double bound, StepOut& O) {
+  const unsigned full = 0xffffffffu;
+  const int lane = threadIdx.x & 31, e = lane < 21 ? lane : 20;
+  const int ri = e >= 15 ? 5 : e >= 10 ? 4 : e >= 6 ? 3 : e >= 3 ? 2 : e >= 1 ? 1 : 0, ci = e - tri6(ri, 0);
+  const double inv_radius = 1.0 / I.radius;
+  const double hs = I.H[hidx(ci, ri)] * I.scaling[ci] * I.scaling[ri];
+  double a = hs;
+  if (ri == ci) {
+    const double dg = I.reuse_diagonal ? I.diagonal[ri] : fmin(fmax(hs, 1e-6), 1e32);
+    if (lane == e) O.diagonal[ri] = dg;
+    a = __fma_rn(dg, inv_radius, hs);
+  }
+  double L[6][6], inv[6]; bool ok = true;
+#pragma unroll
+  for (int k = 0; k < 6; k++) {
+    const double piv = __shfl_sync(full, a, tri6(k, k));
+    if (!(piv > 0.0)) ok = false;
+    inv[k] = rsqrt(piv);
+    const double lr = __shfl_sync(full, a, tri6(ri > k ? ri : k, k)) * inv[k], lc = __shfl_sync(full, a, tri6(ci > k ? ci : k, k)) * inv[k];
+#pragma unroll
+    for (int r = k + 1; r < 6; r++) L[r][k] = __shfl_sync(full, a, tri6(r, k)) * inv[k];
+    if (ci > k) a = __fma_rn(-lr, lc, a);
+  }
+  double step[6], rhs[6];
+#pragma unroll
+  for (int i = 0; i < 6; i++) rhs[i] = I.g[i] * I.scaling[i];
+  if (ok) {
+    double y[6];
+#pragma unroll
+    for (int i = 0; i < 6; i++) { double s = rhs[i];
+#pragma unroll
+      for (int k = 0; k < i; k++) s = __fma_rn(-L[i][k], y[k], s); y[i] = s * inv[i]; }
+#pragma unroll
+    for (int i = 5; i >= 0; i--) { double s = y[i];
+#pragma unroll
+      for (int k = i + 1; k < 6; k++) s = __fma_rn(-L[k][i], step[k], s); step[i] = s * inv[i]; }
+#pragma unroll
+    for (int i = 0; i < 6; i++) if (!isfinite(step[i])) ok = false;
+  }
+  int valid = 0; double mcc = 0.0;
+  if (ok) {
+#pragma unroll
+    for (int c = 0; c < 6; c++) step[c] = -step[c];
+    const int li = lane < 6 ? lane : 5;
+    double r = 0.0;
+#pragma unroll
+    for (int j = 0; j < 6; j++) { const int lo = li < j ? li : j, hi = li < j ? j : li; r = __fma_rn(I.H[hidx(lo, hi)] * I.scaling[lo] * I.scaling[hi], step[j], r); }
+    double sg = 0.0, shs = 0.0;
+#pragma unroll
+    for (int i = 0; i < 6; i++) { sg = __fma_rn(step[i], rhs[i], sg); shs = __fma_rn(step[i], __shfl_sync(full, r, i), shs); }
+    mcc = __fma_rn(-0.5, shs, -sg); valid = mcc > 0.0 ? 1 : 0;
+  }
+  if (lane == 0) { O.valid = valid; O.model_cost_change = mcc; O.gd = 0.0; O.dmax = 0.0; }
+  if (!valid) return;
+  double delta[6], gd = 0.0, dmax = 0.0, trial[7];
+#pragma unroll
+  for (int c = 0; c < 6; c++) { delta[c] = step[c] * I.scaling[c]; gd = __fma_rn(I.g[c], delta[c], gd); dmax = fmax(dmax, fabs(delta[c])); }
+  d_plus(I.x, delta, bound, trial);
+  if (lane == 0) { O.gd = gd; O.dmax = dmax; }
+#pragma unroll
+  for (int c = 0; c < 6; c++) if (lane == c) O.delta[c] = delta[c];
+#pragma unroll
+  for (int k = 0; k < 7; k++) if (lane == k) O.trial[k] = trial[k];
+}
+#endif
 LL_HD LL_INLINE double radius_after_success(double radius, double rel) {
   const double c1 = 2.0 * rel - 1.0; radius = radius / fmax(1.0 / 3.0, 1.0 - c1 * c1 * c1); return fmin(1e16, radius);
 }
-LL_HD void lm_hypothesis(const LmState& L, const double* sums, int h, StepIn& I) {
+LL_HD void lm_hypothesis(const LmState& L, const double* sums, int h, StepIn& I, int lane = 0, int stride = 1) {
   if (L.phase == 0 || h == 0) {
-    for (int i = 0; i < 21; i++) I.H[i] = sums[i]; for (int i = 0; i < 6; i++) I.g[i] = sums[21 + i]; for (int k = 0; k < 7; k++) I.x[k] = L.trial[k];
-    if (L.phase == 0) { for (int c = 0; c < 6; c++) I.scaling[c] = 1.0 / (1.0 + sqrt(I.H[hidx(c, c)])); I.radius = 1e4; }
-    else { for (int c = 0; c < 6; c++) I.scaling[c] = L.scaling[c]; I.radius = radius_after_success(L.radius, (L.x_cost - sums[27]) / L.model_cost_change); }
-    for (int c = 0; c < 6; c++) I.diagonal[c] = 0.0; I.reuse_diagonal = 0;
+    for (int i = lane; i < 21; i += stride) I.H[i] = sums[i];
+    for (int k = lane; k < 7; k += stride) I.x[k] = L.trial[k];
+    for (int c = lane; c < 6; c += stride) { I.g[c] = sums[21 + c]; I.scaling[c] = L.phase == 0 ? 1.0 / (1.0 + sqrt(sums[hidx(c, c)])) : L.scaling[c]; I.diagonal[c] = 0.0; }
+    if (lane == 0) { I.radius = L.phase == 0 ? 1e4 : radius_after_success(L.radius, (L.x_cost - sums[27]) / L.model_cost_change); I.reuse_diagonal = 0; }
   } else {
-    for (int i = 0; i < 21; i++) I.H[i] = L.H[i]; for (int i = 0; i < 6; i++) I.g[i] = L.g[i]; for (int k = 0; k < 7; k++) I.x[k] = L.x[k];
-    for (int c = 0; c < 6; c++) { I.scaling[c] = L.scaling[c]; I.diagonal[c] = L.diagonal[c]; }
-    I.radius = L.radius / L.decrease_factor; I.reuse_diagonal = 1;
-  }
-}
+    for (int i = lane; i < 21; i += stride) I.H[i] = L.H[i];
+    for (int k = lane; k < 7; k += stride) I.x[k] = L.x[k];
+    for (int c = lane; c < 6; c += stride) { I.g[c] = L.g[c]; I.scaling[c] = L.scaling[c]; I.diagonal[c] = L.diagonal[c]; }
+    if (lane == 0) { I.radius = L.radius / L.decrease_factor; I.reuse_diagonal = 1; }
+  }
+}
+LL_HD bool lm_iteration_begin(LmState& L, int lane) {
+  const int term = L.iteration >= L.max_iterations ? 0 : (L.last_successful && L.last_gmax <= LM_GTOL) ? 1 : L.radius <= 1e-32 ? 5 : -1;
+  LL_SYNCWARP();
+  if (lane == 0) { if (term >= 0) lm_finish(L, term); else { L.iteration++; L.total_iterations++; } }
+  return term < 0;
+}
+LL_HD void lm_step_input(const LmState& L, StepIn& in, int lane, int stride) {
+  for (int i = lane; i < 21; i += stride) in.H[i] = L.H[i];
+  for (int k = lane; k < 7; k += stride) in.x[k] = L.x[k];
+  for (int c = lane; c < 6; c += stride) { in.g[c] = L.g[c]; in.scaling[c] = L.scaling[c]; in.diagonal[c] = L.diagonal[c]; }
+  if (lane == 0) { in.radius = L.radius; in.reuse_diagonal = L.reuse_diagonal; }
+}
+LL_HD bool lm_iteration_take(LmState& L, const StepOut& so, int lane, int stride) {
+  for (int c = lane; c < 6; c += stride) L.diagonal[c] = so.diagonal[c];
+  if (!so.valid) {
+    const int num_invalid = L.num_invalid + 1;
+    LL_SYNCWARP();
+    if (lane == 0) {
+      L.reuse_diagonal = 1; L.num_invalid = num_invalid;
+      if (num_invalid >= 5) lm_finish(L, 4);
+      else { L.radius = L.radius / L.decrease_factor; L.decrease_factor *= 2.0; L.last_successful = 0; }
+    }
+    return num_invalid >= 5;
+  }
+  for (int c = lane; c < 6; c += stride) L.delta[c] = so.delta[c];
+  for (int k = lane; k < 7; k += stride) L.trial[k] = so.trial[k];
+  if (lane == 0) {
+    L.reuse_diagonal = 1; L.num_invalid = 0;
+    L.model_cost_change = so.model_cost_change; L.gd = so.gd; L.dmax = so.dmax;
+    L.ls_iters = 0; L.prev.value_valid = 0; L.prev.gradient_valid = 0; L.ls_alpha = 1.0;
+    L.phase = 1;
+  }
+  return true;
+}
+#ifdef __CUDACC__
+__device__ __noinline__ void lm_next_iteration_warp(LmState& L, double bound, const StepOut* pre, StepIn& in, StepOut& tmp) {
+  const int lane = threadIdx.x & 31;
+  for (;;) {
+    const bool go = lm_iteration_begin(L, lane);
+    __syncwarp();
+    if (!go) return;
+    const StepOut* so = pre; pre = nullptr;
+    if (!so) { lm_step_input(L, in, lane, 32); __syncwarp(); compute_step_warp(in, bound, tmp); __syncwarp(); so = &tmp; }
+    const bool end = lm_iteration_take(L, *so, lane, 32);
+    __syncwarp();
+    if (end) return;
+  }
+}
+#else
 LL_HD void lm_next_iteration(LmState& L, double bound, const StepOut* pre) {
   for (;;) {
-    if (L.iteration >= L.max_iterations) { lm_finish(L, 0); return; }
-    if (L.last_successful && L.last_gmax <= LM_GTOL) { lm_finish(L, 1); return; }
-    if (L.radius <= 1e-32) { lm_finish(L, 5); return; }
-    L.iteration++; L.total_iterations++;
+    if (!lm_iteration_begin(L, 0)) return;
     StepOut tmp; const StepOut* so = pre; pre = nullptr;
-    if (!so) {
-      StepIn in; for (int i = 0; i < 21; i++) in.H[i] = L.H[i]; for (int i = 0; i < 6; i++) { in.g[i] = L.g[i]; in.scaling[i] = L.scaling[i]; in.diagonal[i] = L.diagonal[i]; }
-      for (int k = 0; k < 7; k++) in.x[k] = L.x[k]; in.radius = L.radius; in.reuse_diagonal = L.reuse_diagonal;
-      compute_step(in, bound, tmp); so = &tmp;
-    }
-    for (int c = 0; c < 6; c++) L.diagonal[c] = so->diagonal[c];
-    L.reuse_diagonal = 1;
-    if (!so->valid) {
-      if (++L.num_invalid >= 5) { lm_finish(L, 4); return; }
-      L.radius = L.radius / L.decrease_factor; L.decrease_factor *= 2.0; L.reuse_diagonal = 1; L.last_successful = 0; continue;
-    }
-    L.num_invalid = 0;
-    L.model_cost_change = so->model_cost_change; L.gd = so->gd; L.dmax = so->dmax;
-    for (int c = 0; c < 6; c++) L.delta[c] = so->delta[c];
-    for (int k = 0; k < 7; k++) L.trial[k] = so->trial[k];
-    L.ls_iters = 0; L.prev.value_valid = 0; L.prev.gradient_valid = 0; L.ls_alpha = 1.0;
-    L.phase = 1; return;
-  }
-}
+    if (!so) { StepIn in; lm_step_input(L, in, 0, 1); compute_step(in, bound, tmp); so = &tmp; }
+    if (lm_iteration_take(L, *so, 0, 1)) return;
+  }
+}
+#endif
 LL_HD void lm_accept_test(LmState& L, const double* sums, double bound, bool defer_gmax) {
   const double cand_cost = sums[27];
   double step_norm = 0; for (int k = 0; k < 7; k++) step_norm += (L.x[k] - L.trial[k]) * (L.x[k] - L.trial[k]); step_norm = sqrt(step_norm);
diff --git a/loam_livox_b200/csrc/solve.cu b/loam_livox_b200/csrc/solve.cu
--- a/loam_livox_b200/csrc/solve.cu
+++ b/loam_livox_b200/csrc/solve.cu
@@ -92,13 +92,10 @@
   E.huber_a = st->huber_a; E.huber_b = st->huber_a * st->huber_a;
 }
 template <bool MB>
-__device__ __forceinline__ void setup_trial(EvalConst& E, const double* x) {
-  for (int k = 0; k < 7; k++) E.x[k] = x[k];
-  E.PJ[0][0] = x[3];  E.PJ[0][1] = x[2];  E.PJ[0][2] = -x[1];
-  E.PJ[1][0] = -x[2]; E.PJ[1][1] = x[3];  E.PJ[1][2] = x[0];
-  E.PJ[2][0] = x[1];  E.PJ[2][1] = -x[0]; E.PJ[2][2] = x[3];
-  E.PJ[3][0] = -x[0]; E.PJ[3][1] = -x[1]; E.PJ[3][2] = -x[2];
-  if (MB) { const double d = x[3], ad = fabs(d);
+__device__ __forceinline__ void setup_trial(EvalConst& E, const double* x, int lane, int stride) {
+  for (int k = lane; k < 7; k += stride) E.x[k] = x[k];
+  for (int m = lane; m < 12; m += stride) { const double v = x[(0x210301032123ull >> (4 * m)) & 15u]; (&E.PJ[0][0])[m] = (0xE8Cu >> m) & 1u ? -v : v; }
+  if (MB && lane == 0) { const double d = x[3], ad = fabs(d);
     if (ad >= 1.0 - 2.220446049250313e-16) { E.sl_lerp = 1; E.sl_theta = 0; E.sl_sin = 1; E.sl_cos = 1; E.sl_dth_dw = 0; }
     else { E.sl_lerp = 0; E.sl_theta = acos(ad); E.sl_sin = sin(E.sl_theta); E.sl_cos = cos(E.sl_theta); E.sl_dth_dw = -(d < 0.0 ? -1.0 : 1.0) / sqrt(1.0 - ad * ad); } }
 }
@@ -206,10 +203,47 @@
 __device__ __forceinline__ void k10_clear(unsigned long long* table, unsigned table_mask, SolveSync* Y) {
   for (unsigned idx = blockIdx.x * SOLVE_THREADS + threadIdx.x; idx <= table_mask; idx += gridDim.x * SOLVE_THREADS) table[idx] = L1_EMPTY;
   for (unsigned idx = blockIdx.x * SOLVE_THREADS + threadIdx.x; idx < K10_PASSES * 2048u + 64u; idx += gridDim.x * SOLVE_THREADS) ((unsigned*)Y->hist)[idx] = 0u;
+  for (unsigned idx = blockIdx.x * SOLVE_THREADS + threadIdx.x; idx < K10_FINE_EXPS * K10_FINE_BINS / 4; idx += gridDim.x * SOLVE_THREADS) ((uint4*)Y->fine)[idx] = make_uint4(0u, 0u, 0u, 0u);
+}
+
+template <int NB>
+__device__ __forceinline__ void k10_find_bin(K10Smem& s_k10, const unsigned* gh, int shift, unsigned dmask, unsigned long long prefix, unsigned long long himask,
+                                             bool first, const double* ratio) {
+  const int tid = threadIdx.x, lane = tid & 31, warp = tid >> 5;
+  constexpr int BPT = NB / SOLVE_THREADS;
+  unsigned h[BPT], run = 0;
+#pragma unroll
+  for (int b = 0; b < BPT; b++) { h[b] = __ldcg(&gh[tid * BPT + b]); run += h[b]; }
+  unsigned incl = run;
+#pragma unroll
+  for (int o = 1; o < 32; o <<= 1) { const unsigned v = __shfl_up_sync(FULL, incl, o); if (lane >= o) incl += v; }
+  if (lane == 31) s_k10.warp_sum[warp] = incl;
+  __syncthreads();
+  if (tid == 0) { unsigned t = 0; for (int w = 0; w < SOLVE_THREADS / 32; w++) { const unsigned c = s_k10.warp_sum[w]; s_k10.warp_sum[w] = t; t += c; } s_k10.warp_sum[SOLVE_THREADS / 32] = t; }
+  __syncthreads();
+  if (first && tid == 0) {
+    const int n = (int)s_k10.warp_sum[SOLVE_THREADS / 32]; s_k10.n_distinct = n;
+    int k = (int)(*ratio * (double)n); if (k > n - 1) k = n - 1; s_k10.k = k;
+    if (n == 0) s_k10.done = 1;
+  }
+  __syncthreads();
+  if (s_k10.done) return;
+  const unsigned excl = s_k10.warp_sum[warp] + incl - run; const unsigned k = (unsigned)s_k10.k;
+  __syncthreads();
+  if (k >= excl && k < excl + run) {
+    unsigned below = excl; int j = 0;
+#pragma unroll
+    for (int b = 0; b < BPT; b++) { if (k >= below + h[b] && j == b) { below += h[b]; j = b + 1; } }
+    const int jj = j < BPT ? j : BPT - 1;
+    s_k10.k = (int)(k - below); s_k10.cnt_bin = (int)h[jj];
+    s_k10.prefix = prefix | ((unsigned long long)(tid * BPT + jj) << shift);
+    s_k10.mask = himask | ((unsigned long long)dmask << shift);
+  }
+  __syncthreads();
 }
 
 __device__ __forceinline__ void k10_select(K10Smem& s_k10, SolveSync* Y, unsigned& gen, const int* type, const double* l1, int M, int tiles_per_cta, int tile, const double* ratio) {
-  const int tid = threadIdx.x, lane = tid & 31, warp = tid >> 5;
+  const int tid = threadIdx.x;
   if (tid == 0) { s_k10.prefix = 0ull; s_k10.mask = 0ull; s_k10.k = -1; s_k10.done = 0; s_k10.result = 0.0; }
   __syncthreads();
   for (int pass = 0; pass < K10_PASSES && !s_k10.done; pass++) {
@@ -221,43 +255,23 @@
       const int i = (blockIdx.x + gridDim.x * k) * tile + tid, li = k * SOLVE_THREADS + tid;
       if (i < M && tid < tile && (type[li] & 0x100)) {
         const unsigned long long key = l1_key(l1[i]);
-        if ((key & himask) == prefix) atomicAdd(&s_k10.hist[(unsigned)(key >> shift) & dmask], 1u);
+        if ((key & himask) == prefix) {
+          atomicAdd(&s_k10.hist[(unsigned)(key >> shift) & dmask], 1u);
+          const unsigned e = (unsigned)(key >> 52) - K10_FINE_E0;
+          if (pass == 0 && e < K10_FINE_EXPS) atomicAdd(&Y->fine[e][(unsigned)(key >> K10_FINE_SHIFT) & (K10_FINE_BINS - 1)], 1u);
+        }
       }
     }
     __syncthreads();
     unsigned* gh = Y->hist[pass];
     for (int b = tid; b < 2048; b += SOLVE_THREADS) { const unsigned c = s_k10.hist[b]; if (c) atomicAdd(&gh[b], c); }
     grid_sync(Y, gen);
-    constexpr int BPT = 2048 / SOLVE_THREADS;
-    unsigned h[BPT], run = 0;
-#pragma unroll
-    for (int b = 0; b < BPT; b++) { h[b] = __ldcg(&gh[tid * BPT + b]); run += h[b]; }
-    unsigned incl = run;
-#pragma unroll
-    for (int o = 1; o < 32; o <<= 1) { const unsigned v = __shfl_up_sync(FULL, incl, o); if (lane >= o) incl += v; }
-    if (lane == 31) s_k10.warp_sum[warp] = incl;
-    __syncthreads();
-    if (tid == 0) { unsigned t = 0; for (int w = 0; w < SOLVE_THREADS / 32; w++) { const unsigned c = s_k10.warp_sum[w]; s_k10.warp_sum[w] = t; t += c; } s_k10.warp_sum[SOLVE_THREADS / 32] = t; }
-    __syncthreads();
-    if (pass == 0 && tid == 0) {
-      const int n = (int)s_k10.warp_sum[SOLVE_THREADS / 32]; s_k10.n_distinct = n;
-      int k = (int)(*ratio * (double)n); if (k > n - 1) k = n - 1; s_k10.k = k;
-      if (n == 0) s_k10.done = 1;
-    }
-    __syncthreads();
+    k10_find_bin<2048>(s_k10, gh, shift, dmask, prefix, himask, pass == 0, ratio);
     if (!s_k10.done) {
-      const unsigned excl = s_k10.warp_sum[warp] + incl - run; const unsigned k = (unsigned)s_k10.k;
-      __syncthreads();
-      if (k >= excl && k < excl + run) {
-        unsigned below = excl; int j = 0;
-#pragma unroll
-        for (int b = 0; b < BPT; b++) { if (k >= below + h[b] && j == b) { below += h[b]; j = b + 1; } }
-        const int jj = j < BPT ? j : BPT - 1;
-        s_k10.k = (int)(k - below); s_k10.cnt_bin = (int)h[jj];
-        s_k10.prefix = prefix | ((unsigned long long)(tid * BPT + jj) << shift);
-        s_k10.mask = himask | ((unsigned long long)dmask << shift);
-      }
-      __syncthreads();
+      if (pass == 0 && s_k10.cnt_bin > 64) {
+        const unsigned e = (unsigned)(s_k10.prefix >> 52) - K10_FINE_E0;
+        if (e < K10_FINE_EXPS) k10_find_bin<K10_FINE_BINS>(s_k10, Y->fine[e], K10_FINE_SHIFT, K10_FINE_BINS - 1, s_k10.prefix, s_k10.mask, false, ratio);
+      }
       if (s_k10.cnt_bin <= 64 || pass == K10_PASSES - 1) {
         const unsigned long long pf = s_k10.prefix, hm = s_k10.mask;
         for (int kk = 0; kk < tiles_per_cta; kk++) {
@@ -290,7 +304,9 @@
   __shared__ double s_sum[32];
   __shared__ LmState s_lm;
   __shared__ double s_gmax;
+  __shared__ StepIn s_in[2];
   __shared__ StepOut s_pre[2];
+  __shared__ StepOut s_tmp;
   __shared__ K10Smem s_k10;
   __shared__ long long s_prof[16];
   RegDevState* st = a.st;
@@ -350,7 +366,7 @@
     if (ph == 1) for (int k = 0; k < 7; k++) x_start[k] = s_lm.x_best[k];
     d_plus(x_start, z, bound, tr);
     if (ph == 0) setup_static(E, st);
-    setup_trial<MB>(E, tr);
+    setup_trial<MB>(E, tr, 0, 1);
     LmState& L = s_lm;
     L.phase = 0; L.iteration = 0; L.max_iterations = (fused && ph == 0) ? a.prerun_iterations : a.max_iterations; L.num_invalid = 0; L.done = 0; L.termination = 0; L.last_successful = 1; L.reuse_diagonal = 0;
     L.ls_iters = 0; L.n_valid = 0; L.total_iterations = 0; L.total_evaluations = 0; L.pending = -1;
@@ -459,29 +475,33 @@
     if (cur_mode == SOLVE_EVALUATE) {
       if (tid == 0) { LmState& L = s_lm; for (int i = 0; i < 21; i++) L.H[i] = s_sum[i]; for (int i = 0; i < 6; i++) L.g[i] = s_sum[21 + i]; L.x_cost = s_sum[27]; L.n_valid = (int)(s_sum[28] + 0.5); L.done = 1; }
     } else {
-      StepIn in; double gx[7], gg[6];
-      if (warp == 1 && lane < 2) lm_hypothesis(s_lm, s_sum, lane, in);
-      if (tid == 64) { for (int k = 0; k < 7; k++) gx[k] = s_lm.trial[k]; for (int c = 0; c < 6; c++) gg[c] = -s_sum[21 + c]; }
+      const bool hyp = warp == 1 || warp == 2; const int h = warp - 1;
+      if (hyp) lm_hypothesis(s_lm, s_sum, h, s_in[h], lane, 32);
       __syncthreads();
       const long long t_h0 = clock64();
-      if (warp == 1 && lane < 2) { compute_step(in, bound, s_pre[lane]); if (master && lane == 0) s_prof[13] += clock64() - t_h0; }
+      if (hyp) { compute_step_warp(s_in[h], bound, s_pre[h]); if (master && tid == 32) s_prof[13] += clock64() - t_h0; }
       else if (tid == 0) { lm_step(s_lm, s_sum, bound, true); if (master) s_prof[14] += clock64() - t_h0; }
-      else if (tid == 64) {
-        double pg[7]; d_plus(gx, gg, bound, pg); double mx = 0; for (int k = 0; k < 7; k++) mx = fmax(mx, fabs(gx[k] - pg[k])); s_gmax = mx;
+      else if (tid == 96) {
+        const double* gx = s_in[0].x; double gg[6], pg[7]; for (int c = 0; c < 6; c++) gg[c] = -s_sum[21 + c];
+        d_plus(gx, gg, bound, pg); double mx = 0; for (int k = 0; k < 7; k++) mx = fmax(mx, fabs(gx[k] - pg[k])); s_gmax = mx;
       }
       __syncthreads();
-      if (tid == 0 && s_lm.pending == 0) s_lm.last_gmax = s_gmax;
-      if (master && tid == 0) s_prof[15] += clock64() - t_h0;
-      if (tid == 0 && s_lm.pending >= 0) lm_next_iteration(s_lm, bound, &s_pre[s_lm.pending]);
-    }
-    if (tid == 0) { if (!*(volatile int*)&s_lm.done) setup_trial<MB>(E, s_lm.trial); }
+      if (warp == 0) {
+        if (lane == 0 && s_lm.pending == 0) s_lm.last_gmax = s_gmax;
+        if (master && lane == 0) s_prof[15] += clock64() - t_h0;
+        __syncwarp();
+        const int pending = s_lm.pending;
+        if (pending >= 0) lm_next_iteration_warp(s_lm, bound, &s_pre[pending], s_in[0], s_tmp);
+        if (!s_lm.done) setup_trial<MB>(E, s_lm.trial, lane, 32);
+      }
+    }
     __syncthreads();
     if (master && tid == 0) { const long long t_e4 = clock64(); s_prof[0] += t_e1 - t_e0; s_prof[1] += t_e2 - t_e1; s_prof[2] += t_e3 - t_e2; s_prof[3] += t_e4 - t_e3; s_prof[5] += 1; }
     if (s_lm.done) break;
   }
   if (tid == 0) {
     LmState& L = s_lm;
-    setup_trial<MB>(E, L.x_best);
+    setup_trial<MB>(E, L.x_best, 0, 1);
     if (master) {
       st->lm = L;
       if (cur_mode != SOLVE_EVALUATE) {
@@ -641,6 +661,36 @@
 }
 
 
+__global__ void __launch_bounds__(128) lm_step_parity_kernel(const double* in, int n, double bound, double* out_serial, double* out_warp) {
+  __shared__ StepIn s_in[4];
+  __shared__ StepOut s_out[4][2];
+  const int lane = threadIdx.x & 31, w = threadIdx.x >> 5, i = blockIdx.x * 4 + w;
+  if (i >= n) return;
+  const double* src = in + (size_t)i * LL_STEP_IN_DOUBLES;
+  StepIn& I = s_in[w];
+  for (int k = lane; k < 47; k += 32) (&I.H[0])[k] = src[k];
+  if (lane == 0) I.reuse_diagonal = src[47] != 0.0 ? 1 : 0;
+  for (int k = lane; k < 2 * (int)(sizeof(StepOut) / 8); k += 32) ((unsigned long long*)&s_out[w][0])[k] = 0x7ff4deadbeef0000ull + (unsigned)(k % (sizeof(StepOut) / 8));
+  __syncwarp();
+  if (lane == 0) compute_step(I, bound, s_out[w][0]);
+  __syncwarp();
+  compute_step_warp(I, bound, s_out[w][1]);
+  __syncwarp();
+  for (int f = 0; f < 2; f++) {
+    const StepOut& O = s_out[w][f];
+    double* dst = (f == 0 ? out_serial : out_warp) + (size_t)i * LL_STEP_OUT_DOUBLES;
+    for (int k = lane; k < 22; k += 32) dst[k] = (&O.delta[0])[k];
+    if (lane == 0) dst[22] = (double)O.valid;
+  }
+}
+int launch_lm_step_parity(ll_ctx* ctx, const double* d_in, int n, double bound, double* d_out_serial, double* d_out_warp) {
+  if (n <= 0) return LL_OK;
+  lm_step_parity_kernel<<<ll_div_up(n, 4), 128, 0, ctx->stream>>>(d_in, n, bound, d_out_serial, d_out_warp);
+  ctx->launches++;
+  LL_CUDA(ctx, cudaGetLastError());
+  return LL_OK;
+}
+
 struct L1ExchangeArgs { const double* l1; int M; int rank, world; char* comm_local; char* comm_peer[8]; };
 __global__ void __launch_bounds__(256) l1_exchange_kernel(L1ExchangeArgs a) {
   const int i = blockIdx.x * blockDim.x + threadIdx.x;
```

Result: no change. 875.8, median of 6 (+1.2%).
